# PSeitz/veloci

Measured on AMD Instinct MI355X. Metric: queries/sec, 3-term AND on 100M-doc index (p50 latency and HBM fraction alongside), higher is better.
Workload: dtype u32 doc ids + f16->f32 scores

## Files before the change

### veloci_amd/csrc/capi.cpp

```cpp
#include <chrono>
#include <thread>
#include <cstdio>
#include <cstdlib>
#include <cstring>

#include "../../include/veloci_amd.h"
#include <functional>
#include <future>

#include <dlfcn.h>
#include <unistd.h>

#include "engine.hpp"
#include "text.hpp"

using namespace vq;
using vqreq::Request;
using vqreq::VelociError;

namespace {
thread_local std::string g_err;

int fail(int code, const std::string& msg) {
    g_err = msg;
// ... 64 lines not shown
        s += ']';
    }
    s += '}';
}

static void why_found_info_json(std::string& s, const Result& R) {
    s += '{';
    bool first = true;
    for (auto& [anchor, fields] : R.why_found_info) {
        if (!first) s += ',';
        first = false;
        s += '"' + std::to_string(anchor) + "\":";
        why_found_terms_json(s, fields);
    }
    s += '}';
}

namespace {
void dump_f32(std::string& s, float f) {
    uint32_t b;
    std::memcpy(&b, &f, 4);
    s += std::to_string(b);
}
template <class T, class F>
void dump_opt(std::string& s, const std::optional<T>& v, F f) {
    if (v) f(s, *v);
    else s += "null";
}
void dump_usize(std::string& s, size_t v) { s += std::to_string(v); }
void dump_bool(std::string& s, bool v) { s += v ? "true" : "false"; }
void dump_str(std::string& s, const std::string& v) { vqjson::escape_to(s, v); }
void dump_boost_part(std::string& s, const vqreq::RequestBoostPart& b) {
    static const char* const names[] = {"Log2", "Log10", "Multiply", "Add", "Replace"};
    s += "{\"path\":";
    dump_str(s, b.path);
    s += ",\"boost_fun\":";
    if (b.boost_fun) s += std::string("\"") + names[int(*b.boost_fun)] + "\"";
    else s += "null";
    s += ",\"param\":";
    dump_opt(s, b.param, dump_f32);
    s += ",\"skip_when_score\":";
    if (b.skip_when_score) {
        s += '[';
        for (size_t i = 0; i < b.skip_when_score->size(); ++i) {
            if (i) s += ',';
            dump_f32(s, (*b.skip_when_score)[i]);
        }
        s += ']';
    } else s += "null";
    s += ",\"expression\":";
    dump_opt(s, b.expression, dump_str);
    s += '}';
}
void dump_boost_list(std::string& s, const std::optional<std::vector<vqreq::RequestBoostPart>>& v) {
    if (!v) {
        s += "null";
        return;
    }
    s += '[';
    for (size_t i = 0; i < v->size(); ++i) {
        if (i) s += ',';
        dump_boost_part(s, (*v)[i]);
    }
    s += ']';
}
void dump_options(std::string& s, const std::optional<vqreq::SearchRequestOptions>& o) {
    if (!o) {
        s += "null";
        return;
    }
    s += "{\"explain\":";
    dump_bool(s, o->explain);
    s += ",\"top\":";
    dump_opt(s, o->top, dump_usize);
    s += ",\"skip\":";
    dump_opt(s, o->skip, dump_usize);
    s += ",\"boost\":";
    dump_boost_list(s, o->boost);
    s += '}';
}
void dump_part(std::string& s, const vqreq::RequestSearchPart& p) {
    s += "{\"path\":";
    dump_str(s, p.path);
    s += ",\"terms\":[";
    for (size_t i = 0; i < p.terms.size(); ++i) {
        if (i) s += ',';
        dump_str(s, p.terms[i]);
    }
    s += "],\"levenshtein_distance\":";
    if (p.levenshtein_distance) s += std::to_string(*p.levenshtein_distance);
    else s += "null";
    s += ",\"starts_with\":";
    dump_bool(s, p.starts_with);
    s += ",\"is_regex\":";
    dump_bool(s, p.is_regex);
    s += ",\"token_value\":";
    if (p.token_value) dump_boost_part(s, *p.token_value);
    else s += "null";
    s += ",\"boost\":";
    dump_opt(s, p.boost, dump_f32);
    s += ",\"ignore_case\":";
    dump_opt(s, p.ignore_case, dump_bool);
    s += ",\"snippet\":";
    dump_opt(s, p.snippet, dump_bool);
    s += ",\"snippet_info\":";
    dump_bool(s, p.has_snippet_info);
    s += ",\"top\":";
    dump_opt(s, p.top, dump_usize);
    s += ",\"skip\":";
    dump_opt(s, p.skip, dump_usize);
    s += ",\"options\":";
    dump_options(s, p.options);
    s += '}';
}
void dump_search_request(std::string& s, const vqreq::SearchRequest& r) {
    if (r.kind == vqreq::SearchRequest::Search) {
        s += "{\"search\":";
        dump_part(s, r.part);
        s += '}';
        return;
    }
    s += r.kind == vqreq::SearchRequest::Or ? "{\"or\":{\"queries\":[" : "{\"and\":{\"queries\":[";
    for (size_t i = 0; i < r.tree.queries.size(); ++i) {
        if (i) s += ',';
        dump_search_request(s, r.tree.queries[i]);
    }
    s += "],\"options\":";
    dump_options(s, r.tree.options);
    s += "}}";
}
void dump_parts(std::string& s, const std::optional<std::vector<vqreq::RequestSearchPart>>& v) {
    if (!v) {
        s += "null";
        return;
    }
    s += '[';
    for (size_t i = 0; i < v->size(); ++i) {
        if (i) s += ',';
        dump_part(s, (*v)[i]);
    }
    s += ']';
}
}

extern "C" {

const char* vq_last_error(void) { return g_err.c_str(); }
const char* vq_version(void) { return "veloci_amd 0.3 (gfx950)"; }
uint32_t vq_debug_div100_mismatches(void) { return vq::debug_div100_mismatches(); }
uint32_t vq_debug_probe_occupancy(uint32_t shape, uint32_t nd, uint32_t na, uint32_t arr_slot, uint32_t cand_cap, uint32_t* lds_bytes) {
    const size_t lds = vq::scan_probe_lds_bytes(cand_cap, nd, na, arr_slot);
    if (lds_bytes) *lds_bytes = uint32_t(lds);
    return vq::debug_probe_occupancy(shape, lds);
}
uint64_t vq_index_speculative_reruns(const vq_index* index) { return index ? index->idx->or_reruns.load() : 0; }
int vq_debug_facet_select(const uint32_t* hist, uint32_t num_values, uint32_t top, uint32_t misalign, uint32_t* out_values, uint32_t* out_counts) {
    if (!hist || !out_values || !out_counts) return -1;
    return vq::debug_facet_select(hist, num_values, top, misalign, out_values, out_counts);
}

vq_index_builder* vq_index_builder_new(uint32_t num_anchors, uint32_t doc_lo, uint32_t doc_hi) {
    auto* b = new vq_index_builder();
    b->b.num_anchors = num_anchors;
    b->b.doc_lo = doc_lo;
    b->b.doc_hi = doc_hi;
    return b;
}
void vq_index_builder_free(vq_index_builder* b) { delete b; }

int vq_index_add_fst(vq_index_builder* b, const char* path, uint32_t num_terms, const uint8_t* term_bytes, const uint64_t* term_offsets) {
    return guard([&] {
        if (!b || !path || (num_terms && (!term_bytes || !term_offsets))) throw VelociError(VQ_ERR_INVALID_ARGUMENT, "vq_index_add_fst: null argument");
        HostFst f;
        f.terms.reserve(num_terms);
        for (uint32_t i = 0; i < num_terms; ++i) {
            f.terms.emplace_back(reinterpret_cast<const char*>(term_bytes) + term_offsets[i], size_t(term_offsets[i + 1] - term_offsets[i]));
            if (i && !(f.terms[i - 1] < f.terms[i])) throw VelociError(VQ_ERR_INVALID_ARGUMENT, std::string("terms must be bytewise sorted and unique: ") + path);
        }
        b->b.fst[path] = std::move(f);
    });
}

int vq_index_add_token_to_anchor_score(vq_index_builder* b, const char* path, uint32_t num_tokens, const uint64_t* offsets, const uint32_t* anchors,
                                       const uint32_t* scores, const uint64_t* global_lens) {
    return guard([&] {
        if (!b || !path || !offsets) throw VelociError(VQ_ERR_INVALID_ARGUMENT, "vq_index_add_token_to_anchor_score: null argument");
        HostPostings p;
        p.offsets.assign(offsets, offsets + num_tokens + 1);
        const uint64_t n = offsets[num_tokens];
        if (n && (!anchors || !scores)) throw VelociError(VQ_ERR_INVALID_ARGUMENT, "vq_index_add_token_to_anchor_score: null arrays");
        p.anchors.resize(n);
        p.scores.resize(n);
        const size_t piece = size_t(1) << 24;
        parallel_for((n + piece - 1) / piece, host_threads(), [&](size_t i) {
            const size_t off = i * piece, m = std::min<size_t>(piece, n - off);
            std::memcpy(p.anchors.data() + off, anchors + off, m * 4);
            std::memcpy(p.scores.data() + off, scores + off, m * 4);
        });
        parallel_for(num_tokens, host_threads(), [&](size_t t) {
            for (uint64_t i = offsets[t] + 1; i < offsets[t + 1]; ++i)
                if (!(anchors[i - 1] < anchors[i])) throw VelociError(VQ_ERR_INVALID_ARGUMENT, std::string("posting lists must be ascending and unique: ") + path);
        });
        if (global_lens) p.global_lens.assign(global_lens, global_lens + num_tokens);
        b->b.postings[path] = std::move(p);
    });
}

int vq_index_add_key_value_store(vq_index_builder* b, const char* path, uint32_t key_base, uint32_t num_keys, const uint64_t* offsets,
                                 const uint32_t* values) {
    return guard([&] {
        if (!b || !path || !offsets) throw VelociError(VQ_ERR_INVALID_ARGUMENT, "vq_index_add_key_value_store: null argument");
        HostKV k;
        k.key_base = key_base;
        k.offsets.assign(offsets, offsets + num_keys + 1);
        const uint64_t n = offsets[num_keys];
        if (n && !values) throw VelociError(VQ_ERR_INVALID_ARGUMENT, "vq_index_add_key_value_store: null values");
        k.values.assign(values, values + n);
        b->b.kv[path] = std::move(k);
    });
}

int vq_index_add_phrase_pair_to_anchor(vq_index_builder* b, const char* path, uint64_t num_pairs, const uint32_t* t1, const uint32_t* t2,
                                       const uint64_t* offsets, const uint32_t* anchors) {
    return guard([&] {
        if (!b || !path || !offsets) throw VelociError(VQ_ERR_INVALID_ARGUMENT, "vq_index_add_phrase_pair_to_anchor: null argument");
        HostPhrase p;
        p.t1.assign(t1, t1 + num_pairs);
        p.t2.assign(t2, t2 + num_pairs);
        p.offsets.assign(offsets, offsets + num_pairs + 1);
        p.anchors.assign(anchors, anchors + offsets[num_pairs]);
        b->b.phrase[path] = std::move(p);
    });
}

int vq_index_add_boost(vq_index_builder* b, const char* path, uint32_t key_base, uint32_t num_keys, const uint8_t* present, const uint32_t* value_bits) {
    return guard([&] {
        if (!b || !path || (num_keys && !value_bits)) throw VelociError(VQ_ERR_INVALID_ARGUMENT, "vq_index_add_boost: null argument");
        HostBoost h;
        h.key_base = key_base;
        if (present) h.present.assign(present, present + num_keys);
        h.bits.assign(value_bits, value_bits + num_keys);
        b->b.boost[path] = std::move(h);
    });
}

int vq_index_set_column_meta(vq_index_builder* b, const char* field, int is_anchor_identity_column, int tokenize) {
    return guard([&] {
        if (!b || !field) throw VelociError(VQ_ERR_INVALID_ARGUMENT, "vq_index_set_column_meta: null argument");
        ColumnMeta m;
        m.is_anchor_identity_column = is_anchor_identity_column != 0;
        m.tokenize = tokenize != 0;
        b->b.columns[field] = m;
    });
}

int vq_index_build(vq_index_builder* b, int device, vq_index** out) {
    return guard([&] {
        if (!b || !out) throw VelociError(VQ_ERR_INVALID_ARGUMENT, "vq_index_build: null argument");
        *out = nullptr;
        auto idx = build_index(b->b, device);
        auto* h = new vq_index();
        h->idx = std::move(idx);
        *out = h;
    });
}
void vq_index_free(vq_index* i) { delete i; }

int vq_index_set_stream(vq_index* i, void* hip_stream) {
    return guard([&] {
        if (!i) throw VelociError(VQ_ERR_INVALID_ARGUMENT, "vq_index_set_stream: null index");
        std::vector<std::unique_lock<std::mutex>> quiet;
        for (auto& w : i->idx->ws) quiet.emplace_back(w.mu);
        i->idx->stream = hip_stream ? static_cast<hipStream_t>(hip_stream) : i->idx->own_stream;
        i->idx->fin_stream = hip_stream ? static_cast<hipStream_t>(hip_stream) : i->idx->own_fin_stream;
    });
}
int vq_index_set_streams(vq_index* i, void* scan_stream, void* finish_stream) {
    return guard([&] {
        if (!i) throw VelociError(VQ_ERR_INVALID_ARGUMENT, "vq_index_set_streams: null index");
        if (!scan_stream || !finish_stream) throw VelociError(VQ_ERR_INVALID_ARGUMENT, "vq_index_set_streams: null stream (vq_index_set_stream(index, NULL) restores the index's own)");
        std::vector<std::unique_lock<std::mutex>> quiet;
        for (auto& w : i->idx->ws) quiet.emplace_back(w.mu);
        i->idx->stream = static_cast<hipStream_t>(scan_stream);
        i->idx->fin_stream = static_cast<hipStream_t>(finish_stream);
    });
}
int vq_index_set_allreduce(vq_index* i, vq_allreduce_u64_fn fn, void* ctx) {
    return guard([&] {
        if (!i) throw VelociError(VQ_ERR_INVALID_ARGUMENT, "vq_index_set_allreduce: null index");
        std::vector<std::unique_lock<std::mutex>> quiet;
        for (auto& w : i->idx->ws) quiet.emplace_back(w.mu);
        i->idx->allreduce_fn = fn;
        i->idx->allreduce_ctx = ctx;
    });
}
uint64_t vq_index_device_bytes(const vq_index* i) { return i ? i->idx->device_bytes : 0; }

int vq_request_parse(const char* json, size_t len, vq_request** out) {
    return guard([&] {
        if (!json || !out) throw VelociError(VQ_ERR_INVALID_ARGUMENT, "vq_request_parse: null argument");
        *out = nullptr;
        auto* r = new vq_request();
        try {
            r->req = vqreq::request_from_json_text(json, len);
        } catch (...) {
            delete r;
// ... 957 lines not shown
```

### veloci_amd/csrc/compile.cpp

```cpp
#include <algorithm>
#include <cmath>
#include <cstdlib>
#include <cstring>
#include <regex>
#include <set>

#include "engine.hpp"
#include "text.hpp"

namespace vq {
std::atomic<uint64_t> g_compile_ns[16];

using namespace vqreq;

namespace {

bool ends_with(const std::string& s, const char* suf) {
    size_t n = std::strlen(suf);
    return s.size() >= n && std::memcmp(s.data() + s.size() - n, suf, n) == 0;
}

[[noreturn]] void unsupported(const std::string& what) {
    throw VelociError(ERR_UNSUPPORTED, "unsupported on the MI355X query path: " + what);
}
// ... 532 lines not shown
        for (uint32_t id : l.hits_ids) {
            const uint32_t *b, *e;
            if (t2a.host_row(id, &b, &e)) all.insert(all.end(), b, e);
        }
        std::sort(all.begin(), all.end());
        if (!with_multiplicity) all.erase(std::unique(all.begin(), all.end()), all.end());
        return layered_inline(all);
    }
    std::vector<uint32_t> layered_inline(const std::vector<uint32_t>& sorted_ids) {
        std::vector<std::vector<uint32_t>> layers;
        for (size_t i = 0; i < sorted_ids.size();) {
            size_t j = i;
            while (j < sorted_ids.size() && sorted_ids[j] == sorted_ids[i]) ++j;
            const size_t mult = j - i;
            if (layers.size() < mult) layers.resize(mult);
            for (size_t m = 0; m < mult; ++m) layers[m].push_back(sorted_ids[i]);
            i = j;
        }
        std::vector<uint32_t> out;
        for (auto& l : layers) out.push_back(add_inline_list(std::move(l)));
        return out;
    }

    static size_t union_min() {
        static const size_t v = std::getenv("VQ_UNION_MIN") ? size_t(std::atoi(std::getenv("VQ_UNION_MIN"))) : 4;
        return v;
    }
    static bool has_wide_and(const SearchRequest& r) {
        if (r.kind == SearchRequest::Search) return false;
        if (r.kind == SearchRequest::And && r.tree.queries.size() >= 3) return true;
        for (auto& q : r.tree.queries)
            if (has_wide_and(q)) return true;
        return false;
    }

    void push_op(std::vector<DOp>& ops, const DOp& op, uint32_t& sp) {
        if (ops.size() >= size_t(kMaxOps)) unsupported("query tree with more than " + std::to_string(kMaxOps) + " nodes");
        ops.push_back(op);
        if (op.kind != OP_LEAF) sp -= op.nchild;
        ++sp;
        max_depth = std::max(max_depth, sp);
        if (sp > uint32_t(kStackDepth)) unsupported("query tree deeper than the evaluation stack");
    }

    std::string leaf_union_key(const Leaf& l) {
        const PostingStore& ps = posting_store(l);
        size_t nonempty = 0;
        for (auto& [tid, score] : l.hits_scores)
            if (tid < ps.num_tokens && ps.global_len[tid]) ++nonempty;
        if (!(nonempty > union_min() || (nonempty > 1 && req.search_req && has_wide_and(*req.search_req)))) return std::string();
        return "u|" + l.path + "|" + (l.key.empty() ? l.part->key() : l.key);
    }

    NodeInfo compile_leaf_scores(const SearchRequest& r, Leaf& l, std::vector<DOp>& ops, uint32_t& sp) {
        std::vector<Leaf*> one{&l};
        return compile_leaf_lists(r.part.terms[0], one, ops, sp);
    }

    NodeInfo compile_leaf_lists(const std::string& label, const std::vector<Leaf*>& members, std::vector<DOp>& ops, uint32_t& sp) {
        PhaseTimer pt(3);
        NodeInfo info;
        DOp op{};
        op.kind = OP_LEAF;
        op.list_begin = uint16_t(cq.lists.size());
        info.label = label;
        struct Entry {
            const PostingStore* ps;
            uint32_t tid;
            float score;
        };
        std::vector<Entry> entries;
        entries.reserve(4);
        info.cover.reserve(4);
        for (Leaf* l : members) {
            const PostingStore& ps = posting_store(*l);
            for (auto& [tid, score] : l->hits_scores)
                if (tid < ps.num_tokens) entries.push_back({&ps, tid, score});
        }
        size_t nonempty = 0;
        for (auto& e : entries)
            if (e.ps->global_len[e.tid]) ++nonempty;
        uint32_t count = 0;
        if (nonempty > union_min() || (nonempty > 1 && req.search_req && has_wide_and(*req.search_req))) {
            std::string ukey;
            if (members.size() == 1) ukey = leaf_union_key(*members[0]);
            else {
                ukey = "u|fused";
                for (Leaf* l : members) ukey += "|" + l->path + "|" + (l->key.empty() ? l->part->key() : l->key);
            }
            const UnionJob* done = nullptr;
            if (unions) {
                auto it = unions->find(ukey);
                if (it != unions->end()) done = &it->second;
            }
            info.glen = 0;
            if (!done) {
                UnionJob job;
                job.key = ukey;
                for (auto& e : entries)
                    if (e.ps->global_len[e.tid]) {
                        job.terms.push_back(UnionJob::Term{e.ps, e.tid, e.score});
                        job.input_postings += e.ps->len[e.tid];
                    }
                cq.union_requests.push_back(std::move(job));
                info.len_known = true;
            } else {
                if (done->len) {
                    HList h;
                    h.d_docs = done->d_docs;
                    h.d_scores = reinterpret_cast<const uint16_t*>(done->d_vals);
                    h.len = done->len;
                    h.global_len = done->global_len;
                    h.flags = LIST_HAS_SCORES | LIST_F32;
                    h.term_score = 1.0f;
                    h.max_value = done->max_value;
                    uint32_t li = add_list(h);
                    info.cover.push_back(li);
                    info.cover_len += h.len;
                    count = 1;
                }
                cq.algorithmic_bytes += 6ull * done->input_postings + 8ull * done->len;
                info.glen = done->global_len;
                info.len_known = !req.filter && idx.can_sum_over_shards();
            }
            op.list_count = uint16_t(count);
            push_op(ops, op, sp);
            info.emitted = true;
            return info;
        }
        uint32_t with_entries = 0;
        for (auto& e : entries) {
            const PostingStore& ps = *e.ps;
            if (ps.global_len[e.tid]) ++with_entries;
            if (ps.len[e.tid] == 0) continue;
            HList h;
            h.d_docs = ps.docs.as<uint32_t>() + ps.start[e.tid];
            h.d_scores = ps.scores.as<uint16_t>() + ps.start[e.tid];
            h.len = ps.len[e.tid];
            h.global_len = ps.global_len[e.tid];
            h.flags = LIST_HAS_SCORES;
            h.term_score = e.score;
            h.max_raw = ps.max_raw[e.tid];
            if (!ps.bm_start.empty() && ps.bm_start[e.tid] >= 0) {
                h.flags |= LIST_BITMAP;
                h.d_bitmap = ps.bitmaps.as<uint32_t>() + ps.bm_start[e.tid];
                h.d_rank_dir = ps.rank_dir.as<uint32_t>() + ps.rd_start[e.tid];
            }
            if (!ps.td_start.empty() && ps.td_start[e.tid] >= 0) h.d_tile_dir = ps.tile_dir.as<uint32_t>() + ps.td_start[e.tid];
            if (!ps.pk_start.empty() && ps.pk_start[e.tid] >= 0) {
                h.d_cov32 = ps.cov32.as<uint32_t>() + uint64_t(ps.pk_start[e.tid]) * 8;
                h.d_gdir = ps.gdir.as<uint32_t>() + ps.gd_start[e.tid];
                if (ps.ak_start[e.tid] >= 0) h.d_arr16 = ps.arr16.as<uint16_t>() + uint64_t(ps.ak_start[e.tid]) * 8;
                h.tile_most = ps.tile_most[e.tid];
            }
            uint32_t li = add_list(h);
            info.cover.push_back(li);
            info.cover_len += h.len;
            cq.algorithmic_bytes += 6ull * h.len;
            ++count;
        }
        op.list_count = uint16_t(count);
        info.len_known = with_entries <= 1 && !req.filter;
        info.glen = 0;
        for (auto& e : entries) info.glen += e.ps->global_len[e.tid];
        push_op(ops, op, sp);
        info.emitted = true;
        return info;
    }

    void fill_boost_params(DColBoost& cb, const RequestBoostPart& b) {
        cb.fun = b.boost_fun ? int32_t(*b.boost_fun) : BF_NONE;
        cb.param = b.param.value_or(0.0f);
        if (b.skip_when_score) {
            if (b.skip_when_score->size() > size_t(kMaxSkipWhen)) unsupported("more than 4 skip_when_score values");
            cb.nskip = uint32_t(b.skip_when_score->size());
            for (size_t i = 0; i < b.skip_when_score->size(); ++i) cb.skip[i] = (*b.skip_when_score)[i];
        }
        cb.expr_op = EX_NONE;
        if (b.expression) parse_expression(*b.expression, cb);
    }

    std::vector<uint32_t> boost_1n_text_ids(const RequestSearchPart& part, Leaf& l) {
        std::vector<uint32_t> ids;
        auto cit = idx.columns.find(part.path);
        const bool tokenized = cit != idx.columns.end() && cit->second.tokenize;
        if (tokenized) {
            const KVStore& t2t = kv_store(l.path + TOKENS_TO_TEXT_ID);
            for (auto& h : l.hits_scores) {
                const uint32_t *rb, *re;
                if (t2t.host_row(h.first, &rb, &re)) ids.insert(ids.end(), rb, re);
                else ids.push_back(h.first);
            }
            sort_unique_u32(ids);
        } else ids = l.hits_ids;
        return ids;
    }
    std::vector<std::pair<uint32_t, float>> resolve_boost_1n(const RequestSearchPart& part, Leaf& l, const RequestBoostPart& b) {
        PhaseTimer pt(1);
        std::vector<uint32_t> value_ids;
        {
            PhaseTimer gather(6);
            const std::vector<uint32_t> ids = boost_1n_text_ids(part, l);
            const KVStore& to_parent = kv_store(l.path + VALUE_ID_TO_PARENT);
            for (uint32_t id : ids) {
                const uint32_t *rb, *re;
                if (to_parent.host_row(id, &rb, &re)) value_ids.insert(value_ids.end(), rb, re);
            }
        }
        {
            PhaseTimer sort(7);
            sort_unique_u32(value_ids);
        }
        PhaseTimer pairs_timer(8);
        auto bit = idx.boost.find(b.path + BOOST_VALID_TO_VALUE);
        if (bit == idx.boost.end()) throw VelociError(ERR_INDEX_NOT_FOUND, "Did not found path in indices " + b.path + BOOST_VALID_TO_VALUE);
        const KVStore& to_anchor = kv_store(b.path + VALUE_ID_TO_ANCHOR);
        std::vector<std::pair<uint32_t, float>> pairs;
        pairs.reserve(value_ids.size());
        for (uint32_t vid : value_ids) {
            float v;
            if (!bit->second.host_value(vid, &v)) continue;
            const uint32_t *rb, *re;
            if (to_anchor.host_row(vid, &rb, &re)) pairs.push_back({*rb, v});
        }
        return pairs;
    }

    void emit_boost_1n(const RequestSearchPart& part, Leaf& l, const RequestBoostPart& b, std::vector<DOp>& ops, uint32_t& sp) {
        PhaseTimer pt(2);
        const std::string cache_key = (l.key.empty() ? part.key() : l.key) + "|" + b.path;
        auto emit_layer = [&](const HList& h) {
            const uint32_t li = add_list(h);
            cq.algorithmic_bytes += 8ull * h.len;
            DColBoost cb{};
            fill_boost_params(cb, b);
            cb.nskip = 0;
            cq.leaf_cols.push_back(cb);
            DOp op{};
            op.kind = OP_BOOST1N;
            op.nchild = 1;
            op.list_begin = uint16_t(li);
            op.list_count = 1;
            op.child_slot[0] = uint8_t(cq.leaf_cols.size() - 1);
            push_op(ops, op, sp);
        };
        static const bool device_on = std::getenv("VQ_BOOST1N_DEVICE") != nullptr;
        if (boost_cache && device_on) {
            const std::string to_parent = l.path + VALUE_ID_TO_PARENT, to_anchor = b.path + VALUE_ID_TO_ANCHOR, col = b.path + BOOST_VALID_TO_VALUE;
            auto kp = idx.kv.find(to_parent), ka = idx.kv.find(to_anchor);
            const bool staged = kp != idx.kv.end() && ka != idx.kv.end() && kp->second.value_csr && ka->second.value_csr && idx.boost.count(col);
            if (staged && !boost_cache->device) {
                Boost1nJob job;
                job.key = cache_key;
                job.to_parent_path = to_parent;
                job.to_anchor_path = to_anchor;
                job.boost_path = col;
                job.text_ids = boost_1n_text_ids(part, l);
                cq.boost1n_requests.push_back(std::move(job));
                return;
            }
            if (staged) {
                auto it = boost_cache->device->find(cache_key);
                if (it != boost_cache->device->end() && it->second.done) {
                    const Boost1nJob& job = it->second;
                    if (!job.ascending) unsupported("1:n field boost whose value ids are not in anchor order (" + b.path + ")");
                    if (!job.several) {
                        HList h;
                        h.d_docs = job.d_docs;
                        h.d_scores = reinterpret_cast<const uint16_t*>(job.d_vals);
                        h.len = job.len;
                        h.global_len = job.total;
                        h.flags = LIST_HAS_SCORES | LIST_F32;
                        h.term_score = 1.0f;
                        emit_layer(h);
                        return;
                    }
                }
            }
        }
        std::shared_ptr<Boost1nEntry> entry = boost_cache ? boost_cache->entry(cache_key) : std::make_shared<Boost1nEntry>();
        auto make_layers = [&](const std::vector<std::vector<std::pair<uint32_t, float>>>& layers) {
            auto out = std::make_shared<std::vector<Boost1nEntry::Layer>>();
            for (auto& layer : layers) {
                Boost1nEntry::Layer L;
                L.global_len = layer.size();
                L.docs.reserve(layer.size());
                L.vals.reserve(layer.size());
                for (auto& pr : layer)
                    if (pr.first >= idx.doc_lo && pr.first < idx.doc_hi) {
                        L.docs.push_back(pr.first);
                        L.vals.push_back(pr.second);
                    }
                out->push_back(std::move(L));
            }
            return out;
        };
        std::call_once(entry->resolved, [&] {
            entry->pairs = resolve_boost_1n(part, l, b);
            PhaseTimer order_check(9);
            const auto& pairs = entry->pairs;
            for (size_t i = 1; i < pairs.size(); ++i) {
                if (pairs[i].first < pairs[i - 1].first) entry->ascending = false;
                entry->several = entry->several || pairs[i].first == pairs[i - 1].first;
            }
            if (!entry->ascending) return;
            if (!entry->several) entry->layers = make_layers({pairs});
// ... 1157 lines not shown
                        for (uint32_t e = 0; e < cq.lists.size(); ++e)
                            if (cq.lists[e].d_docs == h.d_docs && cq.lists[e].inline_idx < 0 && cq.lists[e].len == h.len) {
                                li = e;
                                break;
                            }
                        if (li == UINT32_MAX) {
                            li = add_list(h);
                            cq.algorithmic_bytes += 4ull * h.len;
                        }
                        cq.loc_idx.push_back(uint16_t(li));
                        ++count;
                    }
                lf.list_count = uint16_t(count);
                cq.locf.push_back(lf);
            }

        if (req.facets)
            for (auto& fr : *req.facets) {
                std::vector<std::string> steps = get_steps_to_anchor(fr.field);
                std::string store_path;
                if (steps.size() == 1) store_path = steps.front() + PARENT_TO_VALUE_ID;
                else if (idx.kv.count(steps.back() + ANCHOR_TO_TEXT_ID)) store_path = steps.back() + ANCHOR_TO_TEXT_ID;
                const KVStore& kv = store_path.empty() ? idx.composed_facet(steps) : kv_store(store_path);
                if (!kv.facet_csr) unsupported("facet source " + store_path + " is not staged as an anchor-keyed CSR");
                auto dit = idx.dict.find(steps.back());
                if (dit == idx.dict.end()) throw VelociError(ERR_FST_NOT_FOUND, "fst not found loaded in indices " + steps.back() + " ");
                DFacet f{};
                f.offsets = kv.csr_off.as<uint64_t>();
                f.values = kv.csr_values.as<uint32_t>();
                f.direct = kv.csr_direct.p ? kv.csr_direct.as<uint32_t>() : nullptr;
                f.key_base = kv.csr_key_base;
                f.num_keys = kv.csr_num_keys;
                f.num_values = std::max<uint32_t>(uint32_t(dit->second.terms.size()), kv.csr_num_keys ? kv.csr_max_value + 1 : 0);
                const uint64_t want = fr.top ? std::min<uint64_t>(*fr.top, f.num_values) : f.num_values;
                f.top = want > uint64_t(kMaxTopK) ? 0u : uint32_t(want);
                cq.facets.push_back(f);
                FacetOut fo;
                fo.field = fr.field;
                fo.dict_path = steps.back();
                fo.top = f.top;
                fo.host_top = want > uint64_t(kMaxTopK) ? uint32_t(want) : 0u;
                fo.num_values = f.num_values;
                cq.facet_out.push_back(fo);
                cq.algorithmic_bytes += 4ull * f.num_values;
            }
        cq.algorithmic_bytes += 8ull * cq.top_k;

        if (label_wanted) {
            if (maybe_reqs.empty() && count_reqs.empty()) unsupported("OR over an operand whose term label is only known at run time (set_op.rs:143,439)");
            if (!idx.can_sum_over_shards())
                unsupported("OR over an AND whose label follows run-time result sizes, on a sharded index without vq_index_set_allreduce");
            count_reqs.insert(count_reqs.end(), maybe_reqs.begin(), maybe_reqs.end());
        }
        if (2 * count_reqs.size() + 1 > 256) unsupported("more than 127 AND operands whose sizes must be measured first");
        build_presence_program();
        if (!count_reqs.empty())
            for (auto& l : cq.lists) l.flags |= LIST_COVER;
        {
            const size_t n = cq.ops.size();
            auto is_leaf1 = [&](const DOp& o) {
                return o.kind == OP_LEAF && o.list_count == 1 && (cq.lists[o.list_begin].flags & LIST_HAS_SCORES) && !(cq.lists[o.list_begin].flags & LIST_F32);
            };
            if (n == 1 && is_leaf1(cq.ops[0])) cq.simple_n = 1;
            else if (n >= 3 && n <= 5 && cq.ops[n - 1].kind != OP_LEAF && cq.ops[n - 1].nchild == n - 1) {
                bool ok = true;
                for (size_t i = 0; i + 1 < n; ++i) ok = ok && is_leaf1(cq.ops[i]);
                if (ok) cq.simple_n = uint32_t(n - 1);
            }
            if (cq.simple_n > 1 && cq.ops[n - 1].kind == OP_OR && cq.ops[n - 1].nslots == cq.simple_n) {
                DOp& root = cq.ops[n - 1];
                std::vector<std::pair<uint8_t, DOp>> leaves;
                for (uint32_t k = 0; k < cq.simple_n; ++k) leaves.push_back({root.child_slot[k], cq.ops[k]});
                std::stable_sort(leaves.begin(), leaves.end(), [](auto& x, auto& y) { return x.first < y.first; });
                for (uint32_t k = 0; k < cq.simple_n; ++k) {
                    cq.ops[k] = leaves[k].second;
                    root.child_slot[k] = leaves[k].first;
                }
            }
        }

        {
            static const bool force_generic = std::getenv("VQ_FORCE_GENERIC") != nullptr;
            const bool pure = cq.simple_n && count_reqs.empty() && cq.fops.empty() && cq.groups.empty() && cq.tboosts.empty() && cq.cols.empty() && cq.locf.empty() &&
                              cq.facets.empty() && uint64_t(idx.doc_hi) - idx.doc_lo >= 65536;
            if (pure && !force_generic) {
                uint32_t f = 1u << 17;
                static const bool no_probe = std::getenv("VQ_NO_PROBE") != nullptr;
                static const uint64_t probe_min_docs = std::getenv("VQ_PROBE_MIN_DOCS") ? uint64_t(std::atoll(std::getenv("VQ_PROBE_MIN_DOCS"))) : 40'000'000ull;
                bool probe = !no_probe && cq.simple_n >= 2 && cq.ops[cq.simple_n].kind == OP_AND && uint64_t(idx.doc_hi) - idx.doc_lo >= probe_min_docs;
                uint32_t arr_mask = 0;
                if (probe) {
                    static const bool no_arr = std::getenv("VQ_PROBE_NO_ARR") != nullptr;
                    uint32_t covers = 0;
                    for (uint32_t k = 0; k < cq.simple_n; ++k) {
                        const HList& l = cq.lists[cq.ops[k].list_begin];
                        if (l.flags & LIST_COVER) {
                            ++covers;
                            probe = probe && l.d_cov32;
                        } else {
                            const bool arr = l.d_arr16 && !no_arr && (!(l.flags & LIST_BITMAP) || uint64_t(l.len) * 16 < uint64_t(idx.doc_hi) - idx.doc_lo);
                            if (arr) arr_mask |= 1u << k;
                            probe = probe && (arr || (l.flags & LIST_BITMAP));
                        }
                    }
                    probe = probe && covers == 1;
                }
                static const bool no_probe_or = std::getenv("VQ_NO_PROBE_OR") != nullptr;
                uint32_t or_cover = UINT32_MAX;
                if (!probe && !no_probe && !no_probe_or && !req.exact_routes_only && cq.top_k >= 1 && cq.simple_n >= 2 && cq.simple_n <= 3 && cq.ops[cq.simple_n].kind == OP_OR &&
                    cq.ops[cq.simple_n].nslots == cq.simple_n && !idx.sharded() && !(idx.comm && idx.comm->nranks > 1) && uint64_t(idx.doc_hi) - idx.doc_lo >= probe_min_docs) {
                    for (uint32_t k = 0; k < cq.simple_n; ++k) {
                        const HList& l = cq.lists[cq.ops[k].list_begin];
                        if (l.d_cov32 && (or_cover == UINT32_MAX || l.len < cq.lists[cq.ops[or_cover].list_begin].len)) or_cover = k;
                    }
                    double sum = 0.0, cnt = 0.0;
                    for (uint32_t k = 0; k < cq.simple_n && or_cover != UINT32_MAX; ++k) {
                        if (k == or_cover) continue;
                        const HList& l = cq.lists[cq.ops[k].list_begin];
                        if (!(l.flags & LIST_BITMAP) || (l.flags & LIST_F32) || l.max_raw >= 0x7C00 || !(l.term_score >= 0.0f)) {
                            or_cover = UINT32_MAX;
                            break;
                        }
                        const uint16_t h = l.max_raw;
                        const int e = (h >> 10) & 31, m = h & 1023;
                        const double a = e ? std::ldexp(1.0 + m / 1024.0, e - 15) : std::ldexp(m / 1024.0, -14);
                        const double v = double(l.term_score) * (a / 100.0);
                        if (v >= 0.00001 * (1.0 - 1e-5)) cnt += 1.0;
                        sum += v;
                    }
                    if (or_cover != UINT32_MAX) {
                        const HList& c = cq.lists[cq.ops[or_cover].list_begin];
                        if (!(c.term_score > 0.0f) || c.max_raw >= 0x7C00) or_cover = UINT32_MAX;
                        else {
                            const double b = sum * cnt * cnt * (1.0 + 1e-5);
                            cq.or_skip_bound = b < 3.0e38 ? float(b) : std::numeric_limits<float>::infinity();
                            if (cq.or_skip_bound < float(b)) cq.or_skip_bound = std::nextafter(cq.or_skip_bound, std::numeric_limits<float>::infinity());
                            probe = true;
                        }
                    }
                }
                const bool or_probe = or_cover != UINT32_MAX && probe;
                bool seq = false;
                for (uint32_t k = 0; k < cq.simple_n && !probe; ++k) {
                    const HList& l = cq.lists[cq.ops[k].list_begin];
                    if ((l.flags & LIST_COVER) && (l.flags & LIST_BITMAP)) seq = true;
                }
                if (seq) f |= 1u << 16;
                if (probe) {
                    f |= 1u << 25 | arr_mask << 12 | (or_probe ? 1u << 27 : 0u);
                    cq.probe = DProbe{};
                    for (uint32_t k = 0; k < cq.simple_n; ++k) {
                        const HList& l = cq.lists[cq.ops[k].list_begin];
                        cq.probe.leaf[k] = DProbeLeaf{l.d_cov32, l.d_arr16, l.d_gdir};
                        if ((arr_mask >> k) & 1u) cq.probe_arr_gran = std::max(cq.probe_arr_gran, l.tile_most);
                    }
                }
                static const bool ring = std::getenv("VQ_RING") != nullptr && std::atoi(std::getenv("VQ_RING")) != 0;
                if (probe && ring && !arr_mask && !or_probe && cq.top_k >= 1 && cq.top_k <= kPoolMaxK) f |= 1u << 26;
                for (uint32_t k = 0; k < cq.simple_n; ++k) {
                    const HList& l = cq.lists[cq.ops[k].list_begin];
                    const bool cover = or_probe ? k == or_cover : (l.flags & LIST_COVER) != 0;
                    if (cover) f |= 1u << (8 + k);
                    if ((l.flags & LIST_BITMAP) && (seq || !cover) && !((arr_mask >> k) & 1u)) f |= 1u << k;
                    if (uint64_t(l.len) * 8192 >= 200 * (uint64_t(idx.doc_hi) - idx.doc_lo)) f |= 1u << (20 + k);
                }
                static const bool no_union_cov = std::getenv("VQ_NO_UNION_COV") != nullptr;
                if (cq.simple_n == 1 && !no_union_cov) {
                    const HList& l = cq.lists[cq.ops[0].list_begin];
                    if (l.d_cov32 && l.d_gdir && l.d_tile_dir && l.term_score > 0.0f && !(l.flags & LIST_F32) && l.inline_idx < 0) {
                        f |= 1u << 28;
                        cq.probe = DProbe{};
                        cq.probe.leaf[0] = DProbeLeaf{l.d_cov32, l.d_arr16, l.d_gdir};
                    }
                }
                cq.simple_flags = f;
            }
        }

        {
            static const bool off = std::getenv("VQ_FORCE_GENERIC") != nullptr || std::getenv("VQ_NO_LEAF_F32") != nullptr;
            if (!off && !cq.simple_flags && count_reqs.empty() && cq.ops.size() == 1 && cq.ops[0].kind == OP_LEAF && cq.ops[0].list_count == 1 &&
                (cq.lists[cq.ops[0].list_begin].flags & LIST_F32) && cq.fops.empty() && cq.groups.empty() && cq.tboosts.empty() && cq.cols.empty() && cq.locf.empty() &&
                cq.facets.empty())
                cq.simple_flags = 1u << 19;
        }
        if (!cq.simple_flags) detect_rich_simple();
        if (!cq.simple_flags) detect_wide();
        if (!cq.simple_flags || ((cq.simple_flags >> 24) & 1u)) compute_prune_table();
        if (!cq.simple_flags && count_reqs.empty()) {
            bool dense_cover = false;
            for (auto& l : cq.lists) dense_cover = dense_cover || ((l.flags & LIST_COVER) && (l.flags & LIST_BITMAP));
            if (dense_cover) {
                cq.seq_tiles = 1;
                for (auto& l : cq.lists)
                    if (l.flags & LIST_BITMAP) l.flags &= ~uint32_t(LIST_COVER);
            }
        }

        const uint32_t L = std::max<uint32_t>(uint32_t(cq.lists.size()), 1);
        const uint64_t range = uint64_t(idx.doc_hi) - idx.doc_lo;
        static const uint32_t ww_max = [] {
            const char* e = std::getenv("VQ_TILE_WORDS_MAX");
            uint32_t v = e ? uint32_t(std::atoi(e)) : 256u;
            uint32_t p2 = 64;
            while (p2 < v && p2 < 2048) p2 <<= 1;
            return p2;
        }();
        static const size_t var_budget = [] {
            const char* e = std::getenv("VQ_TILE_LDS_KB");
            return size_t(e ? std::atoi(e) : 12) * 1024;
        }();
        static const uint64_t span_env = [] {
            const char* e = std::getenv("VQ_SPAN_POSTINGS");
            return uint64_t(e ? std::atoll(e) : 0);
        }();
        const bool and_like = ((cq.simple_flags >> 18) & 1u) || (cq.simple_flags && cq.simple_n > 1 && cq.ops.back().kind == OP_AND);
        const bool wide_like = (cq.simple_flags >> 24) & 1u;
        const bool probe_like = (cq.simple_flags >> 25) & 1u;
        const uint64_t probe_span = std::min<uint64_t>(std::max<uint64_t>(range / 96, 131072), 1048576);
        const bool or_like = cq.simple_flags && !((cq.simple_flags >> 18) & 1u) && !wide_like && !probe_like && cq.simple_n > 1 && cq.ops.back().kind == OP_OR;
        const uint64_t span_postings = span_env ? span_env : (probe_like ? probe_span : and_like ? 131072 : wide_like ? 589824 : (or_like && range >= 50'000'000ull) ? 524288 : 262144);
        uint32_t ww = ww_max;
        const size_t TL = size_t(L) + cq.n_temps;
        while (ww > 64 && (size_t(ww) + TL * ww + size_t(L) * ww / 2) * 4 > var_budget) ww >>= 1;
        if ((size_t(ww) + TL * ww + size_t(L) * ww / 2) * 4 > 96 * 1024) unsupported("too many lists for the LDS tile");
        const uint64_t cover_len = std::max<uint64_t>(root.cover_len, 1);
        if (cover_len * (uint64_t(ww) << 5) / std::max<uint64_t>(range, 1) < 64) {
            const uint64_t want = std::max<uint64_t>(range / cover_len, 2048);
            while (ww > 64 && (uint64_t(ww) << 5) / 2 >= want) ww >>= 1;
        }
        if (cq.simple_flags) ww = 256;
        cq.tile_words = ww;
        cq.stack_depth = std::max<uint32_t>(max_depth, 1);
        uint64_t spans = (cq.total_len + span_postings - 1) / span_postings;
        static const uint64_t facet_span = [] {
            const char* e = std::getenv("VQ_FACET_SPAN_POSTINGS");
            return uint64_t(e ? std::atoll(e) : 4096);
        }();
        if (!cq.facets.empty()) spans = (cq.total_len + facet_span - 1) / facet_span;
        const uint64_t tiles = std::max<uint64_t>((range + (uint64_t(ww) << 5) - 1) / (uint64_t(ww) << 5), 1);
        {
            uint64_t cover_len = 0;
            for (auto& l : cq.lists)
                if (l.flags & LIST_COVER) cover_len += l.len;
            const uint64_t visited = std::max<uint64_t>(std::min<uint64_t>(cover_len, tiles), 1);
            if (!cq.simple_flags && cq.total_len / visited < 1024) spans = std::max<uint64_t>(spans, visited / 16);
            if (((cq.simple_flags >> 18) & 1u) && cq.total_len / visited < 1024) spans = std::max<uint64_t>(spans, visited / 64);
        }
        if ((cq.simple_flags >> 26) & 1u) {
            static const uint64_t ring_tiles = [] {
                const char* e = std::getenv("VQ_RING_SPAN_TILES");
                return uint64_t(e ? std::max(1, std::atoi(e)) : 64);
            }();
            const uint64_t ptiles = std::max<uint64_t>((range + (1u << kProbeTileShift) - 1) >> kProbeTileShift, 1);
            spans = (ptiles + ring_tiles - 1) / ring_tiles;
        }
        spans = std::min<uint64_t>(spans, tiles);
        spans = std::min<uint64_t>(std::max<uint64_t>(spans, 1), 4096);
        cq.n_spans = uint32_t(spans);
        if ((cq.simple_flags >> 19) & 1u) {
            const uint64_t len = cq.lists[cq.ops[0].list_begin].len;
            cq.n_spans = uint32_t(std::min<uint64_t>(std::max<uint64_t>(len / (cq.facets.empty() ? 16384 : 4096), 1), 4096));
        }
        cq.max_spans = uint32_t(std::min<uint64_t>(std::max<uint64_t>(tiles, 1), 4096));
        if ((cq.simple_flags >> 19) & 1u) cq.max_spans = uint32_t(std::min<uint64_t>(std::max<uint64_t>(cq.lists[cq.ops[0].list_begin].len / 64, 1), 4096));
        compute_layout_bytes(root.cover_len);
    }

    void compute_layout_bytes(uint64_t cover_len) {
        const uint64_t range = uint64_t(idx.doc_hi) - idx.doc_lo;
        const bool simple = cq.simple_flags != 0;
        const bool wide = (cq.simple_flags >> 24) & 1u;
        const uint64_t tile_docs = wide ? 8192 : ((cq.simple_flags >> 25) & 1u) ? (1u << kProbeTileShift) : simple ? 16384 : uint64_t(cq.tile_words) << 5;
        const uint64_t tiles = std::max<uint64_t>((range + tile_docs - 1) / tile_docs, 1);
        const bool seq = wide ? cq.wide.seq != 0 : simple ? ((cq.simple_flags >> 16) & 1u) : cq.seq_tiles != 0;
        const uint64_t visited = seq ? tiles : std::min<uint64_t>(std::max<uint64_t>(cover_len, 1), tiles);
        auto bitmap_cost = [&]() { return visited * (tile_docs / 8 + 4); };
        uint64_t b = 8ull * cq.top_k;
        if ((cq.simple_flags >> 19) & 1u) b += 8ull * cq.lists[cq.ops[0].list_begin].len;
        else if (simple && !((cq.simple_flags >> 18) & 1u) && cq.simple_n == 1 && std::getenv("VQ_NO_UNION") == nullptr)
            b += (((cq.simple_flags >> 28) & 1u) ? 4ull : 6ull) * cq.lists[cq.ops[0].list_begin].len;
        else if (wide) {
            for (uint32_t k = 0; k < cq.wide.n_leaves; ++k) b += ((cq.wide.bitmap_mask >> k) & 1u) ? bitmap_cost() : 4ull * cq.lists[cq.wide.leaf_list[k]].len;
        } else if ((cq.simple_flags >> 25) & 1u) {
            for (uint32_t k = 0; k < cq.simple_n; ++k) {
                const uint64_t len = cq.lists[cq.ops[k].list_begin].len;
                b += ((cq.simple_flags >> k) & 1u) ? visited * (tile_docs / 8 + 4 * (tile_docs >> kRankShift)) : ((cq.simple_flags >> (12 + k)) & 1u) ? 2ull * len : 4ull * len;
            }
        } else if (simple) {
            std::vector<bool> seen(cq.lists.size(), false);
            const bool rich = (cq.simple_flags >> 18) & 1u;
            for (uint32_t k = 0; k < cq.simple_n; ++k) {
                const uint32_t li = rich ? cq.simple2.leaf_list[k] : cq.ops[k].list_begin;
                seen[li] = true;
                b += ((cq.simple_flags >> k) & 1u) ? bitmap_cost() : 4ull * cq.lists[li].len;
            }
            for (uint32_t li = 0; li < cq.lists.size(); ++li)
                if (!seen[li]) b += 4ull * cq.lists[li].len;
        } else {
            for (auto& l : cq.lists) {
                const bool as_bitmap = (l.flags & LIST_BITMAP) && !(l.flags & LIST_COVER);
                b += as_bitmap ? bitmap_cost() : 4ull * l.len;
            }
        }
        for (auto& f : cq.facets) b += 4ull * f.num_values;
        cq.layout_bytes = b;
    }
};

}

float default_score_for_distance_host(uint8_t distance, bool prefix_matches) { return default_score_for_distance(distance, prefix_matches); }
size_t debug_sort_unique(uint32_t* ids, size_t n) {
    std::vector<uint32_t> v(ids, ids + n);
    sort_unique_u32(v);
    std::copy(v.begin(), v.end(), ids);
    return v.size();
}

std::vector<SuggestEntry> suggest_part(const Index& idx, const RequestSearchPart& part, const FuzzyTable* fuzzy) {
    Request dummy;
    Compiler c(idx, dummy, fuzzy);
    Leaf l;
    l.part = &part;
    l.get_scores = true;
    l.return_term = true;
    l.return_term_lowercase = true;
    c.lookup_terms(idx, l, true, false);
    if (part.token_value) c.apply_token_value(*part.token_value, l);
    std::vector<SuggestEntry> out;
    std::map<uint32_t, const std::string*> text;
    for (auto& t : l.terms) text[t.first] = &t.second;
    for (auto& h : l.hits_scores) out.push_back(SuggestEntry{*text.at(h.first), h.second, h.first});
    return out;
}


namespace {
template <class IsHit, class Append>
std::string snippet_of_tokens(size_t n, IsHit is_hit, Append append_text, const vqreq::SnippetInfo& opt, bool* any) {
    const int64_t around = opt.num_words_around_snippet * 2;
    std::string out;
    int64_t first_hit = -1, last_hit = -1, group_first = -1, group_last = -1;
    uint64_t windows = 0;
    auto close_group = [&]() {
        if (group_first < 0) return;
        if (windows < opt.max_snippets) {
            if (windows) out += opt.snippet_connector;
            const size_t lo = size_t(std::max<int64_t>(group_first - around, 0)), hi = size_t(std::min<int64_t>(group_last + around + 1, int64_t(n)));
            for (size_t i = lo; i < hi; ++i) {
                if (is_hit(i)) {
                    out += opt.snippet_start_tag;
                    append_text(out, i);
                    out += opt.snippet_end_tag;
                } else append_text(out, i);
            }
        }
        ++windows;
    };
    for (size_t i = 0; i < n; ++i) {
        if (!is_hit(i)) continue;
        if (first_hit < 0) first_hit = int64_t(i);
        if (group_first < 0 || int64_t(i) - group_last >= around) {
            close_group();
            group_first = int64_t(i);
        }
        group_last = last_hit = int64_t(i);
    }
    close_group();
    *any = first_hit >= 0;
    if (!*any) return out;
    if (first_hit > around) out.insert(0, opt.snippet_connector);
    if (last_hit < int64_t(n) - around) out += opt.snippet_connector;
    return out;
}
std::string snippet_of_text(const Dictionary& dict, const uint32_t* toks, size_t n, const std::vector<uint32_t>& wanted_sorted, const vqreq::SnippetInfo& opt, bool* any) {
    return snippet_of_tokens(
        n, [&](size_t i) { return std::binary_search(wanted_sorted.begin(), wanted_sorted.end(), toks[i]); },
        [&](std::string& out, size_t i) {
            if (toks[i] < dict.terms.size()) out += dict.terms[toks[i]];
        },
        opt, any);
}
void check_snippet_window(const vqreq::SnippetInfo& opt) {
    if (opt.num_words_around_snippet < 0 || opt.num_words_around_snippet > 0x3FFFFFFF)
        throw VelociError(ERR_INVALID_REQUEST, "InvalidRequest: \"snippet_info.num_words_around_snippet out of range\" ");
}
}

std::optional<std::string> highlight_text(const std::string& text, const std::vector<std::string>& terms, const vqreq::SnippetInfo& opt, bool tokenized) {
    check_snippet_window(opt);
    std::vector<std::string> set = terms;
    std::sort(set.begin(), set.end());
    set.erase(std::unique(set.begin(), set.end()), set.end());
    if (set.size() == 1 && set[0] == text) return opt.snippet_start_tag + text + opt.snippet_end_tag;
    if (!tokenized) return std::nullopt;
    const std::vector<vqtext::TokenSpan> tokens = vqtext::tokenize_grouped(text);
    std::vector<char> hit(tokens.size(), 0);
    for (size_t i = 0; i < tokens.size(); ++i) hit[i] = std::binary_search(set.begin(), set.end(), text.substr(tokens[i].begin, tokens[i].end - tokens[i].begin));
    bool any = false;
    std::string out = snippet_of_tokens(
        tokens.size(), [&](size_t i) { return hit[i] != 0; }, [&](std::string& o, size_t i) { o.append(text, tokens[i].begin, tokens[i].end - tokens[i].begin); }, opt, &any);
    if (!any || opt.max_snippets == 0) return std::nullopt;
    return out;
}

std::vector<SuggestEntry> highlight_part(const Index& idx, const RequestSearchPart& part, const FuzzyTable* fuzzy) {
    static const vqreq::SnippetInfo kDefault;
    const vqreq::SnippetInfo& opt = part.has_snippet_info ? part.snippet_info : kDefault;
    check_snippet_window(opt);
    RequestSearchPart lookup = part;
    lookup.snippet.reset();
    lookup.has_snippet_info = false;
    Request dummy;
    Compiler c(idx, dummy, fuzzy);
    Leaf l;
    l.part = &lookup;
    l.get_scores = true;
    c.lookup_terms(idx, l, true, false);
    if (lookup.token_value) c.apply_token_value(*lookup.token_value, l);

    struct TextHit {
        uint32_t text;
        float score;
        uint32_t token, order;
    };
    std::vector<TextHit> hits;
    std::vector<std::pair<uint32_t, float>> ranked;
    const std::string& path = l.path;
    auto cit = idx.columns.find(path.substr(0, path.size() - std::strlen(TEXTINDEX)));
    const bool tokenized = cit != idx.columns.end() && cit->second.tokenize;
    const bool add_snippets = part.snippet.value_or(false);
    std::map<uint32_t, std::string> snippets;
    for (auto& h : l.hits_scores) ranked.push_back(h);
    if (tokenized) {
        auto kit = idx.kv.find(path + TOKENS_TO_TEXT_ID);
        if (kit == idx.kv.end()) throw VelociError(ERR_INDEX_NOT_FOUND, "Did not found path in indices " + path + TOKENS_TO_TEXT_ID);
        uint32_t order = 0;
        for (auto& h : l.hits_scores) {
            const uint32_t *b, *e;
// ... 238 lines not shown
```

### veloci_amd/csrc/device_types.hpp

```cpp
#pragma once
#include <hip/hip_runtime.h>
#include <stdint.h>

namespace vq {

constexpr int kBlock = 64;
constexpr int kCandCap = 2048;
constexpr int kMaxTopK = 1024;
constexpr int kStackDepth = 16;
constexpr int kMaxChildren = 16;
constexpr int kMaxLists = 64;
constexpr int kMaxOps = 160;
constexpr int kMaxSkipWhen = 4;
constexpr uint32_t kTileDirShift = 14;
constexpr uint32_t kProbeTileShift = 15;
constexpr uint32_t kRankShift = 9;

enum ListFlags : uint32_t {
    LIST_HAS_SCORES = 1u,
    LIST_COVER = 2u,
    LIST_BITMAP = 4u,
    LIST_F32 = 8u,
};

struct DList {
    const uint32_t* docs;
    const uint16_t* scores;
    uint32_t len;
    uint32_t flags;
    float term_score;
    uint16_t max_raw;
    uint16_t pad;
    const uint32_t* bitmap;
    const uint32_t* rank_dir;
    const uint32_t* tile_dir;
};

enum OpKind : uint8_t { OP_LEAF = 0, OP_AND = 1, OP_OR = 2, OP_BOOST1N = 3, OP_LEAFMAX = 4 };

struct DOp {
    uint8_t kind;
    uint8_t nchild;
    uint8_t nslots;
    uint8_t pad;
    uint16_t list_begin;
    uint16_t list_count;
    uint8_t child_slot[kMaxChildren];
    uint8_t and_order[kMaxChildren];
};

enum PresKind : uint8_t { PRES_AND = 0, PRES_OR = 1, PRES_ZERO = 2, PRES_COUNT = 3 };
constexpr uint16_t kSlotTemp = 0x8000;
constexpr uint16_t kSlotRoot = 0xFFFF;
struct DPresOp {
    uint8_t kind;
    uint8_t pad;
    uint16_t out;
    uint16_t n_in;
    uint16_t in_begin;
};

struct DGroup {
    uint16_t list_begin, list_count;
    float mult;
};

struct DTermBoost {
    uint16_t list;
    uint16_t pad;
    float mult;
};

enum BoostFun : int32_t { BF_NONE = -1, BF_LOG2 = 0, BF_LOG10 = 1, BF_MULTIPLY = 2, BF_ADD = 3, BF_REPLACE = 4 };
enum ExprOp : int32_t { EX_NONE = -1, EX_DIV = 0, EX_MUL = 1, EX_ADD = 2, EX_SUB = 3 };

struct DColBoost {
    const float* values;
    const uint32_t* present;
    uint32_t key_base, num_keys;
    int32_t fun;
    float param;
    uint32_t nskip;
    float skip[kMaxSkipWhen];
    int32_t expr_op;
    int32_t expr_lkind, expr_rkind;
    float expr_lval, expr_rval;
    uint32_t pad;
};

constexpr uint16_t kLocPrecomputed = 0xFFFF;
struct DLocField {
    uint16_t list_begin, list_count;
};

struct DFacet {
    const uint64_t* offsets;
    const uint32_t* values;
    const uint32_t* direct;
    uint32_t key_base, num_keys;
    uint32_t hist_off;
    uint32_t num_values;
    uint32_t top;
    uint32_t out_off;
};

struct DSimple2 {
    uint8_t ngroups, root_kind, root_nslots, n_side;
    uint8_t g_kind[4], g_mask[4], g_nslots[4];
    uint8_t g_order[4][4];
    uint8_t g_slot[4][4];
    uint8_t r_order[4];
    uint8_t r_slot[4];
    uint8_t n_grp, n_tb, n_loc, has_filter;
    uint8_t filter_mask, f32_mask, pad2, pad3;
    uint8_t grp_mask[4];
    uint8_t tb_side[4];
    uint8_t loc_leaf[2], loc_side[2];
    uint16_t leaf_list[4];
    uint16_t side_list[4];
    float grp_mult[4];
    float tb_mult[4];
    float ub[16];
    uint8_t prune, pad4, pad5, pad6;
};

constexpr int kWideMax = 16;
struct DWide {
    uint8_t n_leaves, n_groups, root_kind, root_nslots;
    uint8_t seq, pad0, pad1, pad2;
    uint16_t bitmap_mask, cover_mask, prefetch_mask, f32_mask;
    uint16_t leaf_list[kWideMax];
    uint8_t leaf_slot[kWideMax];
    uint8_t g_kind[kWideMax], g_begin[kWideMax], g_count[kWideMax];
    uint8_t leaf_and_order[kWideMax];
    uint8_t leaf_slot_order[kWideMax];
    uint8_t r_and_order[kWideMax];
    uint8_t r_slot[kWideMax];
    uint8_t r_slot_order[kWideMax];
};

struct QHeader {
    uint32_t n_lists, n_ops, n_fops, n_groups, n_tboost, n_col, n_locf, n_facets;
    uint32_t off_lists, off_ops, off_fops, off_groups, off_tboost, off_col, off_locf, off_facets;
    uint32_t top_k;
    uint32_t tile_words;
    uint32_t n_spans;
    uint32_t keys_base;
    uint32_t doc_lo, doc_hi;
    uint32_t part_keys_off;
    uint32_t blob_bytes;
    uint32_t desc_bytes;
    uint32_t n_pres, off_pres, off_pres_in, n_temps;
    uint32_t off_loc_idx;
    uint32_t off_simple2;
    uint32_t off_pool;
    uint32_t prune_n;
    uint64_t prune_mask;
    unsigned long long gthr;
    unsigned long long key_upper;
    uint32_t seq_tiles;
    uint32_t stat_off;
    uint32_t prune_gbits[16];
    uint32_t n_counts;
    uint32_t bitmap_base;
    uint32_t simple_n;
    uint32_t simple_flags;
};

// ... 24 lines not shown
```

### veloci_amd/csrc/engine.hpp

```cpp
#pragma once
#include <hip/hip_runtime.h>

#include <atomic>
#include <cmath>
#include <chrono>
#include <cstdint>
#include <map>
#include <limits>
#include <memory>
#include <thread>
#include <functional>
#include <condition_variable>
#include <mutex>
#include <string>
#include <unordered_map>
#include <vector>

#include "device_types.hpp"
#include "kernels.hpp"
#include "request.hpp"
#include "hostpool.hpp"

namespace vq {

// ... 121 lines not shown
};

struct Dictionary {
    std::vector<std::string> terms;
    std::unordered_map<std::string, std::vector<uint32_t>> lower_map;
    uint32_t char_bytes = 2;
    bool low_exact = true;
    DevBuf d_off;
    DevBuf d_raw;
    DevBuf d_low;
};

struct Index;
struct PostingStore;
struct FuzzyProbe {
    std::string key;
    std::string path;
    std::vector<uint32_t> query;
    uint32_t max_d = 0;
    bool transposition = false, prefix = false, ci = true;
    std::vector<uint32_t> matches;
    std::vector<float> scores;
    std::string lower_term;
    uint32_t lev = 0;
    bool check_prefix = false;
    int status = 0;
    std::string error;
};
using FuzzyTable = std::map<std::string, FuzzyProbe>;
std::string fuzzy_key(const vqreq::RequestSearchPart& p);
bool needs_dictionary_scan(const vqreq::RequestSearchPart& p);
void collect_fuzzy_probes(const Index& idx, const vqreq::Request& req, FuzzyTable& table);
struct Workspace;
void run_fuzzy_probes(const Index& idx, Workspace& ws, FuzzyTable& table, hipStream_t st);
void score_fuzzy_probe(const Index& idx, FuzzyProbe& probe);
float default_score_for_distance_host(uint8_t distance, bool prefix_matches);
size_t debug_sort_unique(uint32_t* ids, size_t n);
struct SuggestEntry {
    std::string text;
    float score;
    uint32_t term_id;
};
std::vector<SuggestEntry> suggest_part(const Index& idx, const vqreq::RequestSearchPart& part, const FuzzyTable* fuzzy);
void collect_suggest_probes(const Index& idx, const vqreq::Request& req, FuzzyTable& table);
std::optional<std::string> highlight_text(const std::string& text, const std::vector<std::string>& terms, const vqreq::SnippetInfo& opt, bool tokenized);
vqreq::Request page_request_after(const vqreq::Request& request, float score, uint32_t id);
std::vector<SuggestEntry> highlight_part(const Index& idx, const vqreq::RequestSearchPart& part, const FuzzyTable* fuzzy);
std::vector<SuggestEntry> run_highlight(const Index& idx, vqreq::RequestSearchPart part);
std::vector<SuggestEntry> run_suggest(const Index& idx, const vqreq::Request& req);

struct UnionJob {
    std::string key;
    struct Term {
        const PostingStore* store;
        uint32_t token;
        float score;
    };
    std::vector<Term> terms;
    const uint32_t* d_docs = nullptr;
    const float* d_vals = nullptr;
    float max_value = std::numeric_limits<float>::infinity();
    uint32_t len = 0;
    uint64_t global_len = 0;
    uint64_t input_postings = 0;
};
using UnionTable = std::map<std::string, UnionJob>;
struct RangeJob {
    std::string key;
    std::string store_path;
    std::vector<uint32_t> tokens;
    std::string union_key;
    std::shared_ptr<const std::vector<uint32_t>> anchors;
    std::vector<uint64_t> counts;
};
using RangeTable = std::map<std::string, RangeJob>;
struct Boost1nEntry {
    struct Layer {
        std::vector<uint32_t> docs;
        std::vector<float> vals;
        uint64_t global_len = 0;
    };
    std::once_flag resolved, layered;
    std::vector<std::pair<uint32_t, float>> pairs;
    bool ascending = true, several = false;
    std::vector<uint32_t> anchors;
    std::shared_ptr<const std::vector<Layer>> layers;
};
struct Boost1nCache {
    static constexpr size_t kShards = 64;
    struct Shard {
        std::mutex mu;
        std::unordered_map<std::string, std::shared_ptr<Boost1nEntry>> map;
    } shard[kShards];
    std::shared_ptr<Boost1nEntry> entry(const std::string& key) {
        Shard& sh = shard[std::hash<std::string>{}(key) % kShards];
        std::lock_guard<std::mutex> g(sh.mu);
        auto& slot = sh.map[key];
        if (!slot) slot = std::make_shared<Boost1nEntry>();
        return slot;
    }
    const std::map<std::string, struct Boost1nJob>* device = nullptr;
};
struct LocalityJob {
    std::string key;
    std::string t2t_path, t2a_path;
    std::vector<uint32_t> tokens;
    const uint32_t* d_docs = nullptr;
    const float* d_vals = nullptr;
    uint32_t len = 0;
};
using LocalityTable = std::map<std::string, LocalityJob>;
struct Boost1nJob {
    std::string key;
    std::string to_parent_path, to_anchor_path, boost_path;
    std::vector<uint32_t> text_ids;
    const uint32_t* d_docs = nullptr;
    const float* d_vals = nullptr;
    uint32_t len = 0;
    uint32_t total = 0;
    bool ascending = true;
    bool several = false;
    bool done = false;
};
using Boost1nTable = std::map<std::string, Boost1nJob>;
constexpr int kStatusNeedsUnion = -1;
constexpr int kStatusNeedsCounts = -2;
constexpr int kStatusNeedsRanges = -3;

struct QueryCounts {
    bool has_filter = false;
    uint64_t filter_count = 0;
    std::map<uint32_t, std::pair<uint64_t, uint64_t>> nodes;
};

struct PostingStore {
    uint32_t num_tokens = 0;
    std::vector<uint64_t> start;
    std::vector<uint32_t> len;
    std::vector<uint64_t> global_len;
    std::vector<uint16_t> max_raw;
    DevBuf docs;
    DevBuf scores;
    uint64_t total_padded = 0;
    std::vector<int64_t> bm_start;
    std::vector<int64_t> rd_start;
    DevBuf bitmaps;
    DevBuf rank_dir;
    std::vector<int64_t> td_start;
    DevBuf tile_dir;
    std::vector<int64_t> pk_start;
    std::vector<int64_t> ak_start;
    std::vector<int64_t> gd_start;
    std::vector<uint32_t> tile_most;
    DevBuf cov32, arr16, gdir;
};

struct KVStore {
    uint32_t key_base = 0, num_keys = 0;
    std::vector<uint64_t> host_off;
    std::vector<uint32_t> host_values;
    bool list_rows = false;
    bool rows_sorted_unique = true;
    bool rows_equal_postings = false;
    std::vector<uint64_t> start;
    std::vector<uint32_t> len;
    DevBuf values;
    DevBuf d_row_start, d_row_len;
    bool text_csr = false;
    DevBuf d_text_vals;
    bool value_csr = false;
    DevBuf d_csr_off;
    bool facet_csr = false;
    uint32_t csr_key_base = 0, csr_num_keys = 0;
    uint32_t csr_max_value = 0;
    DevBuf csr_direct;
    DevBuf csr_off;
    DevBuf csr_values;

    bool host_row(uint64_t key, const uint32_t** b, const uint32_t** e) const {
        if (key < key_base) return false;
        uint64_t r = key - key_base;
        if (r >= num_keys || host_off[r] == host_off[r + 1]) return false;
        *b = host_values.data() + host_off[r];
        *e = host_values.data() + host_off[r + 1];
        return true;
    }
};

struct PhraseStore {
    std::vector<std::pair<uint32_t, uint32_t>> keys;
    std::vector<uint64_t> start;
    std::vector<uint32_t> len;
    DevBuf anchors;
};

struct BoostColumn {
    uint32_t key_base = 0, num_keys = 0;
    bool has_present = false;
    float vmin = 0.0f, vmax = 0.0f;
    bool any_value = false, has_nan = false;
    DevBuf values;
    DevBuf present;
    std::vector<uint32_t> host_bits;
    std::vector<uint8_t> host_present;
    bool host_value(uint64_t key, float* out) const {
        if (key < key_base || key - key_base >= host_bits.size()) return false;
        const size_t r = size_t(key - key_base);
        if (!host_present.empty() && !host_present[r]) return false;
        std::memcpy(out, &host_bits[r], 4);
        return true;
    }
};

struct PinnedBuf {
    void* p = nullptr;
    size_t bytes = 0;
    PinnedBuf() = default;
    PinnedBuf(const PinnedBuf&) = delete;
    PinnedBuf& operator=(const PinnedBuf&) = delete;
    ~PinnedBuf();
    void ensure(size_t n);
    template <class T>
    T* as() const { return reinterpret_cast<T*>(p); }
};

constexpr int kWorkspaces = 4;

enum KernelId : int {
    K_DICT_SCAN = 0, K_UNION_COUNT, K_UNION_WRITE, K_UNION_DENSE_SCATTER, K_UNION_DENSE_COUNT, K_UNION_DENSE_WRITE, K_RANGE_HITS, K_COUNT_PREPASS, K_SCAN_LEAF_F32, K_SCAN_RICH, K_SCAN_RING, K_SCAN_PROBE, K_SCAN_AND, K_SCAN_SIMPLE, K_SCAN_UNION,
    K_SCAN_WIDE, K_TILE_SCAN, K_MERGE_SPANS, K_FINALIZE, K_FACET_SELECT, K_LOCALITY, K_BOOST1N, K_COUNT_
};
extern const char* const kKernelNames[K_COUNT_];

struct TimedLaunch {
    int kernel;
    uint32_t ev_begin, ev_end;
    uint64_t layout_bytes, algorithmic_bytes, queries;
};

struct Workspace {
    std::mutex mu;
    std::atomic<bool> pinned{false};
    std::vector<hipEvent_t> ev_pool;
    uint32_t ev_used = 0;
    std::vector<TimedLaunch> timed;
    hipEvent_t ev_done = nullptr;
    PinnedBuf h_up, h_down;
    DevBuf d_up;
    DevBuf d_span_keys;
    DevBuf d_partial;
    DevBuf d_down;
    DevBuf d_union_docs[2], d_union_vals[2], d_union_max, d_union_meta;
    DevBuf d_union_slab, d_union_dense_docs, d_union_dense_vals, d_union_dense_meta;
    DevBuf d_loc_a, d_loc_b, d_loc_pairs_a, d_loc_pairs_b, d_loc_meta, d_loc_tmp, d_loc_docs, d_loc_vals;
    DevBuf d_b1n_a, d_b1n_b, d_b1n_meta, d_b1n_tmp, d_b1n_docs, d_b1n_vals;
    DevBuf d_probe_desc, d_probe_counts, d_probe_ids;
};

struct KernelProfile {
    double ms = 0;
    uint64_t launches = 0;
    uint64_t layout_bytes = 0;
    uint64_t algorithmic_bytes = 0;
    uint64_t gathered_bytes = 0;
    uint64_t queries = 0;
};
struct Profile {
    bool enabled = false;
    KernelProfile k[K_COUNT_];
    uint64_t batches = 0;
};
struct LaunchTimer {
    Workspace* ws = nullptr;
    hipStream_t st = nullptr;
    size_t slot = 0;
    LaunchTimer(bool on, Workspace& w, hipStream_t s, int kernel, uint64_t layout_bytes = 0, uint64_t algorithmic_bytes = 0, uint64_t queries = 0);
    ~LaunchTimer();
    LaunchTimer(const LaunchTimer&) = delete;
    LaunchTimer& operator=(const LaunchTimer&) = delete;
};


struct ShardComm {
    int nranks = 1, rank = 0;
    void* nccl = nullptr;
    int (*allgather)(void* ctx, const void* local, void* gathered, size_t bytes_per_rank, void* stream) = nullptr;
    int (*allreduce_u32)(void* ctx, void* inout, size_t count, void* stream) = nullptr;
    void* ctx = nullptr;
    hipStream_t stream = nullptr;
    hipEvent_t ev_scan[2] = {nullptr, nullptr}, ev_xchg[2] = {nullptr, nullptr}, ev_fin[2] = {nullptr, nullptr};
    void* unmerged = nullptr;
    int live = 0;
    DevBuf gathered[2];
    DevBuf red;
    bool busy[2] = {false, false};
    std::string failed;
    std::mutex mu;
    ~ShardComm();
};

struct Index {
    int device = 0;
    int (*allreduce_fn)(void*, uint64_t*, size_t) = nullptr;
    void* allreduce_ctx = nullptr;
    bool sharded() const { return doc_lo != 0 || doc_hi != num_anchors; }
    bool can_sum_over_shards() const { return !sharded() || allreduce_fn != nullptr; }
    void sum_over_shards(std::vector<uint64_t>& v) const {
        if (!sharded() || v.empty()) return;
        if (!allreduce_fn || allreduce_fn(allreduce_ctx, v.data(), v.size()) != 0) throw vqreq::VelociError(vqreq::ERR_DEVICE, "all-reduce over the shards failed");
    }
    mutable std::atomic<uint64_t> or_reruns{0};
    mutable std::unique_ptr<HostPool> pool;
    mutable std::mutex pool_mu;
    uint32_t num_anchors = 0, doc_lo = 0, doc_hi = 0;
    uint32_t bitmap_base = 0;
    uint64_t bitmap_words = 0;
    std::map<std::string, Dictionary> dict;
    std::map<std::string, PostingStore> postings;
    std::map<std::string, KVStore> kv;
    std::map<std::string, PhraseStore> phrase;
    std::map<std::string, BoostColumn> boost;
    std::map<std::string, ColumnMeta> columns;
    uint64_t device_bytes = 0;
    mutable std::mutex composed_mu;
    mutable std::map<std::string, std::unique_ptr<KVStore>> composed_facets;
    const KVStore& composed_facet(const std::vector<std::string>& steps) const;
    hipStream_t own_stream = nullptr, own_fin_stream = nullptr;
    hipStream_t pre_stream = nullptr;
    hipStream_t stream = nullptr;
    hipStream_t fin_stream = nullptr;
    mutable std::mutex profile_mutex;
    mutable Profile profile;
    mutable Workspace ws[kWorkspaces];
    mutable std::atomic<uint32_t> next_ws{0};
    mutable DevBuf arena;
    static constexpr size_t kArenaBytes = 64ull << 20;
    mutable std::unique_ptr<ShardComm> comm;
    ~Index();
    bool is_anchor_identity(const std::string& textindex_path) const;
};

std::unique_ptr<Index> build_index(const IndexBuilder& b, int device);

struct HList {
    const uint32_t* d_docs = nullptr;
    const uint16_t* d_scores = nullptr;
    uint32_t len = 0;
    uint32_t flags = 0;
    float term_score = 0.f;
    uint16_t max_raw = 0x7C00;
    float max_value = std::numeric_limits<float>::infinity();
    uint64_t global_len = 0;
    const uint32_t* d_bitmap = nullptr;
    const uint32_t* d_rank_dir = nullptr;
    const uint32_t* d_tile_dir = nullptr;
    const uint32_t* d_cov32 = nullptr;
    const uint16_t* d_arr16 = nullptr;
    const uint32_t* d_gdir = nullptr;
    uint32_t tile_most = 0;
    int inline_idx = -1;
    int inline_val_idx = -1;
};

struct FacetOut {
    std::string field;
    std::string dict_path;
    uint32_t top = 10;
    uint32_t num_values = 0;
    uint32_t host_top = 0;
};

struct ExplainRec {
    enum Kind : uint8_t { Boost, MaxTokenToTextId, TermToAnchor, LevenshteinScore, OrSumOverDistinctTerms } kind = Boost;
    float a = 0.0f, b = 0.0f, c = 0.0f;
    uint32_t term_id = 0;
    std::string text;
};
using ExplainRecs = std::vector<ExplainRec>;
struct ExplainNode {
    uint32_t kind = 0;
    int op = -1;
    std::vector<int> children;
    std::vector<uint16_t> order;
    uint32_t list_begin = 0, list_count = 0;
    std::vector<uint32_t> list_term;
    std::map<uint32_t, ExplainRecs> term_records;
};
using WhyFoundPlan = std::map<std::string, std::vector<uint32_t>>;
struct ExplainPlan {
    std::vector<ExplainNode> nodes;
    int root = -1;
    std::vector<ExList> lists;
    std::vector<ExOp> ops;
    std::vector<uint16_t> aux;
    std::vector<DColBoost> cols;
};

struct CompiledQuery {
    size_t blob_bytes = 0, desc_bytes = 0;
    int status = 0;
    std::shared_ptr<const ExplainPlan> explain_plan;
    std::shared_ptr<const WhyFoundPlan> why_found_plan;
    std::string error;
    std::vector<RangeJob> range_requests;
    std::vector<UnionJob> union_requests;
    std::vector<LocalityJob> locality_requests;
    std::vector<Boost1nJob> boost1n_requests;
    std::vector<uint32_t> count_nodes;
    uint32_t n_counts = 0;
    std::vector<HList> lists;
    std::vector<std::vector<uint32_t>> inline_lists;
    std::vector<std::vector<float>> inline_vals;
    std::vector<DColBoost> leaf_cols;
    uint32_t seq_tiles = 0;
    uint32_t prune_n = 0;
    uint64_t prune_mask = 0;
    uint32_t prune_gbits[16] = {};
    uint32_t n_top_cols = 0;
    std::vector<DOp> ops, fops;
    std::vector<DPresOp> pres;
    std::vector<uint16_t> pres_in;
    uint32_t n_temps = 0;
    uint32_t simple_n = 0;
    uint32_t simple_flags = 0;
    std::vector<DGroup> groups;
    std::vector<DTermBoost> tboosts;
    std::vector<DColBoost> cols;
    std::vector<DLocField> locf;
    std::vector<uint16_t> loc_idx;
    DSimple2 simple2{};
    DWide wide{};
    DProbe probe{};
    uint32_t probe_arr_gran = 0;
    std::vector<DFacet> facets;
    std::vector<FacetOut> facet_out;
    std::map<std::string, std::vector<std::string>> why_found_terms;
    uint32_t top = 10, skip = 0, top_k = 10;
    uint64_t total_len = 0;
    uint64_t algorithmic_bytes = 0;
    uint64_t layout_bytes = 0;
    uint64_t key_upper = ~0ull;
    float or_skip_bound = std::numeric_limits<float>::quiet_NaN();
    bool deep = false;
    uint32_t tile_words = 0, n_spans = 1, stack_depth = 1;
    uint32_t max_spans = 1;
};

CompiledQuery compile_query(const Index& idx, const vqreq::Request& req, const FuzzyTable* fuzzy = nullptr, const UnionTable* unions = nullptr,
                            const QueryCounts* counts = nullptr, const RangeTable* ranges = nullptr, Boost1nCache* boost_cache = nullptr,
                            const LocalityTable* localities = nullptr);
void run_locality_jobs(const Index& idx, Workspace& ws, LocalityTable& table, hipStream_t st);
void run_boost1n_jobs(const Index& idx, Workspace& ws, Boost1nTable& table, hipStream_t st);
void run_range_jobs(const Index& idx, Workspace& ws, RangeTable& table, const UnionTable& unions, hipStream_t st);
void run_union_jobs(const Index& idx, Workspace& ws, UnionTable& table, hipStream_t st);
struct Result;
void complete_explain_requests(const Index& idx, std::vector<std::unique_ptr<Result>>& results, std::vector<int>& status, std::vector<std::string>& errors);
void complete_why_found_requests(const Index& idx, std::vector<std::unique_ptr<Result>>& results, std::vector<int>& status, std::vector<std::string>& errors);
bool request_wants_explain(const vqreq::Request& req);
std::string explain_records_json(const ExplainRecs& records);
void complete_deep_requests(const Index& idx, const vqreq::Request* const* reqs, size_t n, std::vector<std::unique_ptr<Result>>& results,
                            std::vector<int>& status, std::vector<std::string>& errors);

struct ResultFacet {
    std::string field;
    std::vector<std::pair<std::string, uint64_t>> entries;
};
struct Result {
    uint64_t num_hits = 0;
    uint64_t execution_time_ns = 0;
    std::vector<uint32_t> ids;
    std::vector<float> scores;
    std::vector<ResultFacet> facets;
    bool has_facets = false;
    std::map<std::string, std::vector<std::string>> why_found_terms;
    std::shared_ptr<const ExplainPlan> explain_plan;
    std::shared_ptr<const WhyFoundPlan> why_found_plan;
    std::map<uint32_t, std::map<std::string, std::vector<std::string>>> why_found_info;
    bool has_explain = false;
    std::vector<std::pair<bool, ExplainRecs>> explain;
    bool deep = false;
    bool rerun_exact = false;
    mutable std::string json;
};

struct PartialBatch {
    const Index* index = nullptr;
    Workspace* ws = nullptr;
    std::unique_lock<std::mutex> lock;
    bool pinned_ws = false;
    std::vector<CompiledQuery> queries;
    std::vector<uint32_t> slot;
    std::vector<uint8_t> qclass;
    std::vector<FacetJob> facet_jobs;
    uint32_t nq_dev = 0;
    PartialLayout layout{};
    const uint8_t* d_blobs = nullptr;
    const uint32_t* d_blob_off = nullptr;
    const uint32_t* d_span_base = nullptr;
    const FacetJob* d_facet_jobs = nullptr;
    uint8_t* d_partial = nullptr;
    uint32_t total_spans = 0;
    uint32_t n_facet_jobs = 0;
    uint32_t total_facet_out = 0;
    bool profiled = false;
    bool launched = false, finished = false;
    bool merge_launched = false;
    std::chrono::steady_clock::time_point t0;
    void release_workspace();
    std::vector<const vqreq::Request*> reqs;
    ~PartialBatch();
};

std::unique_ptr<PartialBatch> run_partial(const Index& idx, const vqreq::Request* const* reqs, size_t n, int slot = -1, int64_t arena_offset = -1);
void finish_batch(const Index& idx, PartialBatch& pb, const void* gathered_device, uint32_t num_shards, std::vector<std::unique_ptr<Result>>& out,
                  std::vector<int>& status, std::vector<std::string>& errors, size_t shard_stride = 0);
void finish_launch(const Index& idx, PartialBatch& pb, const void* gathered_device, uint32_t num_shards, size_t shard_stride = 0);

}
```

### veloci_amd/csrc/exec.cpp

```cpp
#include <algorithm>
#include <cstdio>
#include <cstdlib>
#include <cstring>
#include <thread>

#include "engine.hpp"

#include "text.hpp"

namespace vq {

using namespace vqreq;

void DevBuf::ensure(size_t n) {
    if (n <= bytes) return;
    size_t want = std::max(n, bytes + bytes / 2);
    alloc(want);
}
PinnedBuf::~PinnedBuf() {
    if (p) (void)hipHostFree(p);
}
void PinnedBuf::ensure(size_t n) {
    if (n <= bytes) return;
    if (p) (void)hipHostFree(p);
// ... 1183 lines not shown
                    for (auto& kv : c.nodes) {
                        flat.push_back(kv.second.first);
                        flat.push_back(kv.second.second);
                    }
                }
                idx.sum_over_shards(flat);
                size_t k = 0;
                for (auto& c : counts) {
                    c.filter_count = flat[k++];
                    for (auto& kv : c.nodes) {
                        kv.second.first = flat[k++];
                        kv.second.second = flat[k++];
                    }
                }
            }
            for (size_t k = 0; k < need.size(); ++k) {
                CompiledQuery& q = pb->queries[need[k]];
                q = compile_query(idx, *reqs[need[k]], fuzzy.empty() ? nullptr : &fuzzy, unions.empty() ? nullptr : &unions, &counts[k], rangesp, &boost_cache,
                                  localities.empty() ? nullptr : &localities);
                if (q.status < 0) {
                    q.status = ERR_UNSUPPORTED;
                    q.error = "unsupported on the MI355X query path: query still needs a pre-pass after the count pre-pass (internal)";
                }
            }
        }
    }
    const double t_compiled = now_ms();
    uint32_t nq = 0;
    uint64_t total_keys = 0, total_hist = 0, total_span_keys = 0, total_spans = 0, blob_bytes = 0;
    uint32_t max_lists = 1, max_ww = 32;
    size_t lds_bytes = 0;
    uint32_t stack_depth = 1;
    std::vector<uint32_t> keys_base, part_keys_off, span_base;
    std::vector<std::vector<uint32_t>> hist_offs, fac_out_offs;
    std::vector<FacetJob> jobs;
    uint32_t fac_out_total = 0;
    {
        static const uint64_t target1 = [] {
            const char* e = std::getenv("VQ_SPAN_TARGET");
            return uint64_t(e ? std::atoll(e) : 2048);
        }();
        const uint64_t target = std::min<uint64_t>(target1 + 64 * uint64_t(n - 1), std::max<uint64_t>(target1, 5120));
        uint64_t have = 0;
        for (size_t i = 0; i < n; ++i)
            if (pb->queries[i].status == 0) have += pb->queries[i].n_spans;
        if (have && have * 3 <= target * 2) {
            const uint64_t f = (target + have - 1) / have;
            for (size_t i = 0; i < n; ++i) {
                CompiledQuery& cq = pb->queries[i];
                if (cq.status == 0) cq.n_spans = uint32_t(std::max<uint64_t>(cq.n_spans, std::min<uint64_t>(uint64_t(cq.n_spans) * f, cq.max_spans)));
            }
        }
        static const bool weighted = std::getenv("VQ_NO_WEIGHTED_SPANS") == nullptr;
        uint64_t total_postings = 0;
        for (size_t i = 0; i < n; ++i)
            if (pb->queries[i].status == 0) total_postings += pb->queries[i].total_len;
        if (weighted && n > 1 && total_postings) {
            const uint64_t per_span = std::max<uint64_t>(total_postings / target, 4096);
            for (size_t i = 0; i < n; ++i) {
                CompiledQuery& cq = pb->queries[i];
                if (cq.status != 0) continue;
                const uint64_t want = std::min<uint64_t>((cq.total_len + per_span - 1) / per_span, cq.max_spans);
                cq.n_spans = uint32_t(std::max<uint64_t>(cq.n_spans, want));
            }
        }
    }
    for (size_t i = 0; i < n; ++i) {
        CompiledQuery& cq = pb->queries[i];
        if (cq.status != 0) continue;
        pb->slot[i] = nq++;
        keys_base.push_back(uint32_t(total_span_keys));
        part_keys_off.push_back(uint32_t(total_keys));
        span_base.push_back(uint32_t(total_spans));
        total_span_keys += uint64_t(cq.n_spans) * cq.top_k;
        total_keys += cq.top_k;
        total_spans += cq.n_spans;
        std::vector<uint32_t> ho, fo;
        for (auto& f : cq.facets) {
            ho.push_back(uint32_t(total_hist));
            fo.push_back(fac_out_total);
            jobs.push_back(FacetJob{uint32_t(total_hist), f.num_values, f.top, fac_out_total});
            total_hist += f.num_values;
            fac_out_total += f.top;
        }
        hist_offs.push_back(std::move(ho));
        fac_out_offs.push_back(std::move(fo));
        if (!cq.blob_bytes) size_blob(cq, idx);
        blob_bytes += cq.blob_bytes;
        max_lists = std::max<uint32_t>(max_lists, uint32_t(cq.lists.size()));
        max_ww = std::max(max_ww, cq.tile_words);
        stack_depth = std::max(stack_depth, cq.stack_depth);
    }
    if (total_span_keys > 0xFFFFFFFFull || total_hist > 0xFFFFFFFFull || total_spans > 0x7FFFFFFFull)
        throw VelociError(ERR_UNSUPPORTED, "batch too large for 32-bit workspace offsets: split the batch");
    span_base.push_back(uint32_t(total_spans));
    pb->nq_dev = nq;
    pb->total_spans = uint32_t(total_spans);
    pb->n_facet_jobs = uint32_t(jobs.size());
    pb->total_facet_out = fac_out_total;
    pb->facet_jobs = jobs;
    const double t_layout = now_ms();

    PartialLayout& lay = pb->layout;
    lay.nq = nq;
    lay.total_keys = total_keys;
    lay.total_hist = total_hist;
    lay.off_hits = 0;
    lay.off_stats = align_up(size_t(nq) * 8, 16);
    lay.off_keys = lay.off_stats + align_up(size_t(nq) * 8, 16);
    lay.off_hist = align_up(lay.off_keys + size_t(total_keys) * 8, 256);
    lay.bytes = align_up(lay.off_hist + size_t(total_hist) * 4, 256);

    const size_t up_blob_off = align_up(blob_bytes, 256);
    const size_t tbl = align_up(size_t(nq + 1) * 4, 256);
    const size_t up_span_base = up_blob_off + tbl;
    const size_t up_qmap_g = up_span_base + tbl;
    const size_t up_span_s = up_qmap_g + tbl;
    const size_t up_qmap_s = up_span_s + tbl;
    const size_t up_span_d = up_qmap_s + tbl;
    const size_t up_qmap_d = up_span_d + tbl;
    const size_t up_span_w = up_qmap_d + tbl;
    const size_t up_qmap_w = up_span_w + tbl;
    const size_t up_span_r = up_qmap_w + tbl;
    const size_t up_qmap_r = up_span_r + tbl;
    const size_t up_span_f = up_qmap_r + tbl;
    const size_t up_qmap_f = up_span_f + tbl;
    const size_t up_span_x = up_qmap_f + tbl;
    const size_t up_qmap_x = up_span_x + tbl;
    const size_t tbl_p = align_up(size_t(nq + 1 + kProbeShapes) * 4, 256);
    const size_t up_span_p = up_qmap_x + tbl;
    const size_t up_qmap_p = up_span_p + tbl_p;
    const size_t up_qmap_n = up_qmap_p + tbl_p;
    const size_t up_work_n = up_qmap_n + tbl;
    size_t ring_items_max = 0;
    for (size_t i = 0; i < n; ++i)
        if (pb->queries[i].status == 0 && ((pb->queries[i].simple_flags >> 26) & 1u)) ring_items_max += pb->queries[i].n_spans;
    const size_t up_items_n = up_work_n + 256;
    const size_t up_jobs = up_items_n + align_up(ring_items_max * 4, 256);
    const size_t up_bytes = up_jobs + align_up(jobs.size() * sizeof(FacetJob), 256) + 256;
    ws.h_up.ensure(up_bytes);
    ws.d_up.ensure(up_bytes);
    uint8_t* hup = ws.h_up.as<uint8_t>();
    uint8_t* dup = ws.d_up.as<uint8_t>();
    bool union_has_or = false;
    uint32_t scatter_wide = 0, scatter_simple = 0;
    uint32_t n_simple = 0, n_generic = 0, n_dense = 0, n_wide = 0, n_rich = 0, spans_simple = 0, spans_generic = 0, spans_dense = 0, spans_wide = 0, spans_rich = 0;
    uint32_t scatter_rich = 0;
    bool facets_rich = false;
    uint32_t n_leaf = 0, spans_leaf = 0;
    uint32_t n_xwide = 0, spans_xwide = 0, leaves_xwide = 0, scatter_xwide = 0;
    struct ProbeClass {
        uint32_t first = 0, n = 0, spans = 0;
        uint32_t na_seen = 0, arr_slot = 0;
    } pcls[kProbeShapes];
    auto probe_class = [](const CompiledQuery& cq) -> uint32_t {
        if ((cq.simple_flags >> 27) & 1u) return kProbeOr;
        const uint32_t nd = cq.simple_n - 1, na = uint32_t(__builtin_popcount((cq.simple_flags >> 12) & 0xFu));
        return nd <= 1 ? kProbeAnd1 : nd == 2 ? kProbeAnd2A0 + na : kProbeAnd3A0 + na;
    };
    auto on_probe = [](const CompiledQuery& cq) {
        return cq.status == 0 && ((cq.simple_flags >> 25) & 1u) && !((cq.simple_flags >> 26) & 1u) && !((cq.simple_flags >> 19) & 1u) && !((cq.simple_flags >> 24) & 1u) &&
               !((cq.simple_flags >> 18) & 1u);
    };
    bool any_probe = false;
    uint32_t n_ring = 0, items_ring = 0, nd_ring = 1, ring_spans_each = 0;
    uint64_t cls_layout[K_COUNT_] = {}, cls_algo[K_COUNT_] = {}, cls_q[K_COUNT_] = {};
    {
        size_t off = 0;
        uint32_t* hbo = reinterpret_cast<uint32_t*>(hup + up_blob_off);
        uint32_t qi = 0;
        for (size_t i = 0; i < n; ++i) {
            CompiledQuery& cq = pb->queries[i];
            if (cq.status != 0) continue;
            hbo[qi] = uint32_t(off);
            const size_t packed = pack_blob(cq, idx, hup + off, dup + off, keys_base[qi], part_keys_off[qi], hist_offs[qi], fac_out_offs[qi], nullptr,
                                            pb->profiled ? uint32_t((lay.off_stats - lay.off_hits) / 8 + qi) : 0u);
            if (packed != cq.blob_bytes) throw VelociError(ERR_DEVICE, "query blob changed size between compilation and packing (internal)");
            off += packed;
            ++qi;
        }
        hbo[nq] = uint32_t(off);
        uint32_t* sg = reinterpret_cast<uint32_t*>(hup + up_span_base);
        uint32_t* mg = reinterpret_cast<uint32_t*>(hup + up_qmap_g);
        uint32_t* ss = reinterpret_cast<uint32_t*>(hup + up_span_s);
        uint32_t* ms = reinterpret_cast<uint32_t*>(hup + up_qmap_s);
        uint32_t* sd = reinterpret_cast<uint32_t*>(hup + up_span_d);
        uint32_t* md = reinterpret_cast<uint32_t*>(hup + up_qmap_d);
        uint32_t* sw = reinterpret_cast<uint32_t*>(hup + up_span_w);
        uint32_t* mw = reinterpret_cast<uint32_t*>(hup + up_qmap_w);
        uint32_t* sr = reinterpret_cast<uint32_t*>(hup + up_span_r);
        uint32_t* mr = reinterpret_cast<uint32_t*>(hup + up_qmap_r);
        uint32_t* sf = reinterpret_cast<uint32_t*>(hup + up_span_f);
        uint32_t* mf = reinterpret_cast<uint32_t*>(hup + up_qmap_f);
        uint32_t accf = 0, accx = 0;
        uint32_t* sx = reinterpret_cast<uint32_t*>(hup + up_span_x);
        uint32_t* mx = reinterpret_cast<uint32_t*>(hup + up_qmap_x);
        uint32_t accg = 0, accs = 0, accd = 0, accw = 0, accr = 0;
        uint32_t* sp = reinterpret_cast<uint32_t*>(hup + up_span_p);
        uint32_t* mp = reinterpret_cast<uint32_t*>(hup + up_qmap_p);
        {
            uint32_t cnt[kProbeShapes] = {};
            for (size_t i = 0; i < n; ++i)
                if (on_probe(pb->queries[i])) ++cnt[probe_class(pb->queries[i])];
            uint32_t at = 0;
            for (uint32_t c = 0; c < kProbeShapes; ++c) {
                pcls[c].first = at;
                at += cnt[c] + 1;
            }
        }
        uint32_t* mn = reinterpret_cast<uint32_t*>(hup + up_qmap_n);
        uint32_t ring_max_spans = 0;
        std::vector<uint32_t> ring_ns;
        bool ring_uniform = true;
        std::memset(hup + up_work_n, 0, 256);
        qi = 0;
        for (size_t i = 0; i < n; ++i) {
            const CompiledQuery& cq = pb->queries[i];
            if (cq.status != 0) continue;
            static const bool union_enabled = std::getenv("VQ_NO_UNION") == nullptr;
            static const bool union_or = std::getenv("VQ_UNION_OR") != nullptr;
            const bool rich = (cq.simple_flags >> 18) & 1u;
            const bool dense = !rich && union_enabled && cq.simple_flags && (cq.simple_n == 1 || (union_or && cq.ops.back().kind == OP_OR));
            int kclass;
            if ((cq.simple_flags >> 19) & 1u) {
                kclass = K_SCAN_LEAF_F32;
                sf[n_leaf] = accf;
                mf[n_leaf++] = qi;
                accf += cq.n_spans;
            } else if ((cq.simple_flags >> 24) & 1u) {
                kclass = K_SCAN_WIDE;
                leaves_xwide = std::max<uint32_t>(leaves_xwide, cq.wide.n_leaves);
                scatter_xwide = std::max<uint32_t>(scatter_xwide, cq.wide.n_leaves - uint32_t(__builtin_popcount(cq.wide.bitmap_mask)));
                sx[n_xwide] = accx;
                mx[n_xwide++] = qi;
                accx += cq.n_spans;
            } else if (rich) {
                kclass = K_SCAN_RICH;
                facets_rich = facets_rich || !cq.facets.empty();
                scatter_rich = std::max<uint32_t>(scatter_rich, cq.simple_n - uint32_t(__builtin_popcount(cq.simple_flags & 0xFu)) + cq.simple2.n_side);
                sr[n_rich] = accr;
                mr[n_rich++] = qi;
                accr += cq.n_spans;
            } else if (dense) {
                kclass = K_SCAN_UNION;
                union_has_or = union_has_or || cq.simple_n > 1;
                sd[n_dense] = accd;
                md[n_dense++] = qi;
                accd += cq.n_spans;
            } else if ((cq.simple_flags >> 26) & 1u) {
                kclass = K_SCAN_RING;
                nd_ring = std::max<uint32_t>(nd_ring, cq.simple_n - 1);
                ring_uniform = ring_uniform && (n_ring == 0 || cq.n_spans == ring_max_spans);
                ring_max_spans = std::max(ring_max_spans, cq.n_spans);
                mn[n_ring++] = qi;
                ring_ns.push_back(cq.n_spans);
                items_ring += cq.n_spans;
            } else if ((cq.simple_flags >> 25) & 1u) {
                kclass = K_SCAN_PROBE;
                if (!on_probe(cq)) throw VelociError(ERR_DEVICE, "probe query outside the probe tables (internal)");
                ProbeClass& pc = pcls[probe_class(cq)];
                pc.na_seen |= 1u << uint32_t(__builtin_popcount((cq.simple_flags >> 12) & 0xFu));
                pc.arr_slot = std::max(pc.arr_slot, cq.probe_arr_gran * 4u);
                sp[pc.first + pc.n] = pc.spans;
                mp[pc.first + pc.n++] = qi;
                pc.spans += cq.n_spans;
                any_probe = true;
            } else if (cq.simple_flags && cq.simple_n > 1 && cq.ops.back().kind == OP_AND) {
                kclass = K_SCAN_AND;
                scatter_wide = std::max<uint32_t>(scatter_wide, cq.simple_n - uint32_t(__builtin_popcount(cq.simple_flags & 0xFu)));
                sw[n_wide] = accw;
                mw[n_wide++] = qi;
                accw += cq.n_spans;
            } else if (cq.simple_flags) {
                kclass = K_SCAN_SIMPLE;
                scatter_simple = std::max<uint32_t>(scatter_simple, cq.simple_n - uint32_t(__builtin_popcount(cq.simple_flags & 0xFu)));
                ss[n_simple] = accs;
                ms[n_simple++] = qi;
                accs += cq.n_spans;
            } else {
                kclass = K_TILE_SCAN;
                sg[n_generic] = accg;
                mg[n_generic++] = qi;
                accg += cq.n_spans;
            }
            pb->qclass.push_back(uint8_t(kclass));
            cls_layout[kclass] += cq.layout_bytes;
            cls_algo[kclass] += cq.algorithmic_bytes;
            cls_q[kclass] += 1;
            ++qi;
        }
        sg[n_generic] = accg;
        ss[n_simple] = accs;
        sw[n_wide] = accw;
        spans_wide = accw;
        sr[n_rich] = accr;
        spans_rich = accr;
        sf[n_leaf] = accf;
        spans_leaf = accf;
        sx[n_xwide] = accx;
        spans_xwide = accx;
        for (const ProbeClass& pc : pcls) sp[pc.first + pc.n] = pc.spans;
        if (n_ring) {
            if (ring_uniform) ring_spans_each = ring_max_spans;
            else {
                uint32_t* it = reinterpret_cast<uint32_t*>(hup + up_items_n);
                uint32_t k = 0;
                for (uint32_t r = 0; r < ring_max_spans; ++r)
                    for (uint32_t j = 0; j < n_ring; ++j)
                        if (r < ring_ns[j]) it[k++] = (j << 12) | r;
            }
        }
        sd[n_dense] = accd;
        spans_generic = accg;
        spans_simple = accs;
        spans_dense = accd;
        if (!jobs.empty()) std::memcpy(hup + up_jobs, jobs.data(), jobs.size() * sizeof(FacetJob));
    }
    pb->d_blobs = dup;
    pb->d_blob_off = reinterpret_cast<const uint32_t*>(dup + up_blob_off);
    pb->d_span_base = reinterpret_cast<const uint32_t*>(dup + up_span_base);
    pb->d_facet_jobs = reinterpret_cast<const FacetJob*>(dup + up_jobs);
    if (nq == 0) return pb;

    const double t_packed = now_ms();
    VQ_HIP(hipMemcpyAsync(dup, hup, up_bytes, hipMemcpyHostToDevice, st));
    ws.d_span_keys.ensure(size_t(total_span_keys) * 8 + 16);
    if (arena_offset >= 0) {
        if (size_t(arena_offset) % 256 || size_t(arena_offset) + lay.bytes > Index::kArenaBytes)
            throw VelociError(ERR_UNSUPPORTED, "partial arena: the step's partials do not fit (" + std::to_string(size_t(arena_offset) + lay.bytes) + " bytes)");
        idx.arena.ensure(Index::kArenaBytes);
        pb->d_partial = idx.arena.as<uint8_t>() + arena_offset;
    } else {
        ws.d_partial.ensure(lay.bytes);
        pb->d_partial = ws.d_partial.as<uint8_t>();
    }
    VQ_HIP(hipMemsetAsync(pb->d_partial, 0, lay.bytes, st));

    uint32_t max_top_k = 1;
    for (size_t i = 0; i < n; ++i)
        if (pb->queries[i].status == 0) max_top_k = std::max(max_top_k, pb->queries[i].top_k);
    uint32_t desc_cap = 0;
    for (size_t i = 0; i < n; ++i)
        if (pb->queries[i].status == 0) {
            desc_cap = std::max(desc_cap, uint32_t(pb->queries[i].desc_bytes));
        }
    desc_cap = uint32_t(align_up(desc_cap, 16));
    bool facets_generic = false;
    static const bool no_facet_cache = std::getenv("VQ_NO_FACET_CACHE") != nullptr;
    for (size_t i = 0; i < n; ++i)
        if (pb->queries[i].status == 0 && !pb->queries[i].simple_flags && !pb->queries[i].facets.empty()) facets_generic = !no_facet_cache;
    if (facets_generic) desc_cap += 2 * 1024 * 4;
    static const uint32_t cand_min = [] {
        const char* e = std::getenv("VQ_CAND_CAP");
        return uint32_t(e ? std::max(32, std::atoi(e)) : 32);
    }();
    uint32_t cand_cap = cand_min;
    while (cand_cap < 2 * max_top_k) cand_cap <<= 1;
    const uint32_t list_table = (std::max<uint32_t>(max_lists, 2) + 1u) & ~1u;
    static const bool tile_queue = std::getenv("VQ_NO_QUEUE") == nullptr;
    for (size_t i = 0; i < n; ++i)
        if (pb->queries[i].status == 0 && !pb->queries[i].simple_flags)
            lds_bytes = std::max(lds_bytes, tile_scan_lds_bytes(uint32_t(pb->queries[i].lists.size()) + pb->queries[i].n_temps, uint32_t(pb->queries[i].lists.size()), pb->queries[i].tile_words, stack_depth, cand_cap, desc_cap, tile_queue && !pb->queries[i].simple_n, list_table));
    if (lds_bytes > 160 * 1024) throw VelociError(ERR_UNSUPPORTED, "LDS tile larger than 160 KiB");
    const bool prof = pb->profiled;
    auto hits_ptr = reinterpret_cast<unsigned long long*>(pb->d_partial + lay.off_hits);
    auto hist_ptr = reinterpret_cast<uint32_t*>(pb->d_partial + lay.off_hist);
    auto keys_ptr = ws.d_span_keys.as<unsigned long long>();
    auto tab = [&](size_t o) { return reinterpret_cast<const uint32_t*>(dup + o); };
    if (spans_leaf) {
        LaunchTimer t(prof, ws, st, K_SCAN_LEAF_F32, cls_layout[K_SCAN_LEAF_F32], cls_algo[K_SCAN_LEAF_F32], cls_q[K_SCAN_LEAF_F32]);
        launch_scan_leaf_f32(st, spans_leaf, pb->d_blobs, pb->d_blob_off, tab(up_span_f), tab(up_qmap_f), n_leaf, cand_cap, keys_ptr, hits_ptr, hist_ptr);
    }
    VQ_HIP(hipGetLastError());
    if (spans_rich) {
        LaunchTimer t(prof, ws, st, K_SCAN_RICH, cls_layout[K_SCAN_RICH], cls_algo[K_SCAN_RICH], cls_q[K_SCAN_RICH]);
        launch_scan_simple(st, true, scatter_rich, spans_rich, pb->d_blobs, pb->d_blob_off, tab(up_span_r), tab(up_qmap_r), n_rich, cand_cap, keys_ptr, hits_ptr, hist_ptr, facets_rich);
    }
    VQ_HIP(hipGetLastError());
    if (items_ring) {
        static const uint32_t cus = [] {
            int dev = 0, v = 0;
            if (hipGetDevice(&dev) != hipSuccess || hipDeviceGetAttribute(&v, hipDeviceAttributeMultiprocessorCount, dev) != hipSuccess || v <= 0) v = 256;
            return uint32_t(v);
        }();
        LaunchTimer t(prof, ws, st, K_SCAN_RING, cls_layout[K_SCAN_RING], cls_algo[K_SCAN_RING], cls_q[K_SCAN_RING]);
        launch_scan_ring(st, nd_ring, cus, pb->d_blobs, pb->d_blob_off, tab(up_qmap_n), n_ring, ring_spans_each, tab(up_items_n), items_ring,
                         reinterpret_cast<uint32_t*>(dup + up_work_n), keys_ptr, hits_ptr);
    }
    VQ_HIP(hipGetLastError());
    if (any_probe) {
        LaunchTimer t(prof, ws, st, K_SCAN_PROBE, cls_layout[K_SCAN_PROBE], cls_algo[K_SCAN_PROBE], cls_q[K_SCAN_PROBE]);
        static const bool trace = std::getenv("VQ_PROBE_TRACE") != nullptr;
        for (uint32_t c = 0; c < kProbeShapes; ++c)
            if (pcls[c].spans && trace)
                std::fprintf(stderr, "probe launch: shape %u, %u queries, %u spans, array slot %u words (fullest tile: %u granules), NA seen 0x%x\n", c, pcls[c].n, pcls[c].spans,
                             pcls[c].arr_slot, pcls[c].arr_slot / 4, pcls[c].na_seen);
        for (uint32_t c = 0; c < kProbeShapes; ++c)
            if (pcls[c].spans)
                launch_scan_probe_shape(st, c, pcls[c].na_seen, pcls[c].arr_slot, pcls[c].spans, pb->d_blobs, pb->d_blob_off, tab(up_span_p) + pcls[c].first, tab(up_qmap_p) + pcls[c].first,
                                        pcls[c].n, cand_cap, keys_ptr, hits_ptr);
    }
    VQ_HIP(hipGetLastError());
    if (spans_wide) {
        LaunchTimer t(prof, ws, st, K_SCAN_AND, cls_layout[K_SCAN_AND], cls_algo[K_SCAN_AND], cls_q[K_SCAN_AND]);
        launch_scan_simple(st, false, scatter_wide, spans_wide, pb->d_blobs, pb->d_blob_off, tab(up_span_w), tab(up_qmap_w), n_wide, cand_cap, keys_ptr, hits_ptr, hist_ptr);
    }
    VQ_HIP(hipGetLastError());
    if (spans_simple) {
        LaunchTimer t(prof, ws, st, K_SCAN_SIMPLE, cls_layout[K_SCAN_SIMPLE], cls_algo[K_SCAN_SIMPLE], cls_q[K_SCAN_SIMPLE]);
        launch_scan_simple(st, false, scatter_simple, spans_simple, pb->d_blobs, pb->d_blob_off, tab(up_span_s), tab(up_qmap_s), n_simple, cand_cap, keys_ptr, hits_ptr, hist_ptr);
    }
    VQ_HIP(hipGetLastError());
    if (spans_dense) {
        LaunchTimer t(prof, ws, st, K_SCAN_UNION, cls_layout[K_SCAN_UNION], cls_algo[K_SCAN_UNION], cls_q[K_SCAN_UNION]);
        launch_scan_union(st, union_has_or, spans_dense, pb->d_blobs, pb->d_blob_off, tab(up_span_d), tab(up_qmap_d), n_dense, cand_cap, keys_ptr, hits_ptr);
    }
    VQ_HIP(hipGetLastError());
    if (spans_xwide) {
        LaunchTimer t(prof, ws, st, K_SCAN_WIDE, cls_layout[K_SCAN_WIDE], cls_algo[K_SCAN_WIDE], cls_q[K_SCAN_WIDE]);
        launch_scan_wide(st, leaves_xwide, scatter_xwide, spans_xwide, pb->d_blobs, pb->d_blob_off, tab(up_span_x), tab(up_qmap_x), n_xwide, cand_cap, keys_ptr, hits_ptr);
    }
    VQ_HIP(hipGetLastError());
    if (spans_generic) {
        LaunchTimer t(prof, ws, st, K_TILE_SCAN, cls_layout[K_TILE_SCAN], cls_algo[K_TILE_SCAN], cls_q[K_TILE_SCAN]);
        launch_tile_scan(st, spans_generic, lds_bytes, pb->d_blobs, pb->d_blob_off, pb->d_span_base, tab(up_qmap_g), n_generic, stack_depth, cand_cap, desc_cap, keys_ptr,
                         hits_ptr, hist_ptr, tile_queue, list_table, facets_generic);
    }
    VQ_HIP(hipGetLastError());
    {
        LaunchTimer t(prof, ws, st, K_MERGE_SPANS, total_span_keys * 8 + total_keys * 8, total_span_keys * 8 + total_keys * 8, nq);
        launch_merge_spans(st, nq, pb->d_blobs, pb->d_blob_off, keys_ptr, reinterpret_cast<unsigned long long*>(pb->d_partial + lay.off_keys));
    }
    VQ_HIP(hipGetLastError());
    VQ_HIP(hipEventRecord(ws.ev_done, st));
    pb->launched = true;
    if (timing_enabled())
        std::fprintf(stderr, "[vq timing] n=%zu compile %.3f ms (dictionary scans %.3f [%zu probes], pass 1 %.3f, unions %.3f [%zu jobs], pass 2 %.3f), range jobs %.3f [%zu], spans generic/simple/and/rich/union %u/%u/%u/%u/%u, pack+launch %.3f ms\n", n,
                     t_compiled - t_start, t_probes - t_start, fuzzy.size(), t_pass1 - t_probes, t_unions - t_pass1, unions.size(), t_compiled - t_ranges,
                     t_ranges - t_unions, ranges.size(), spans_generic, spans_simple, spans_wide, spans_rich, spans_dense + spans_leaf, now_ms() - t_compiled);
    if (timing_enabled())
        std::fprintf(stderr, "[vq timing] pack+launch: span sizing + layout %.3f, blobs + tables %.3f, upload + launches %.3f ms\n", t_layout - t_compiled, t_packed - t_layout, now_ms() - t_packed);
    if (timing_enabled()) {
        uint64_t v[16];
        for (int k = 0; k < 16; ++k) v[k] = g_compile_ns[k].exchange(0);
        if (std::getenv("VQ_TIMING_SUB")) {
            std::fprintf(stderr, "[vq timing] inside 1:n resolve (thread-ms; 6 value-id gather, 7 sort, 8 pairs, 9 order check + layers):");
            for (int k = 6; k < 10; ++k) std::fprintf(stderr, " [%d] %.3f", k, v[k] * 1e-6);
            std::fprintf(stderr, "\n");
        }
        std::fprintf(stderr, "[vq timing] compile thread-ms: total %.3f = dictionary lookups %.3f + 1:n resolve %.3f + 1:n layers %.3f + leaf lists %.3f + rest %.3f; longest request %.3f\n", v[5] * 1e-6,
                     v[0] * 1e-6, v[1] * 1e-6, (v[2] - v[1]) * 1e-6, v[3] * 1e-6, (double(v[5]) - double(v[0]) - double(v[2]) - double(v[3])) * 1e-6, v[4] * 1e-6);
    }
    return pb;
}

std::vector<SuggestEntry> run_suggest(const Index& idx, const vqreq::Request& req) {
    if (!req.suggest) throw VelociError(ERR_INVALID_REQUEST, "only suggest allowed in suggest function");
    VQ_HIP(hipSetDevice(idx.device));
    FuzzyTable fuzzy;
    collect_suggest_probes(idx, req, fuzzy);
    if (!fuzzy.empty()) {
        Workspace& ws = idx.ws[idx.next_ws.fetch_add(1) % kWorkspaces];
        std::unique_lock<std::mutex> lock(ws.mu);
        ws.timed.clear();
        ws.ev_used = 0;
        run_fuzzy_probes(idx, ws, fuzzy, idx.pre_stream ? idx.pre_stream : idx.stream);
    }
    std::vector<SuggestEntry> out;
    for (auto& part : *req.suggest) {
        auto one = suggest_part(idx, part, fuzzy.empty() ? nullptr : &fuzzy);
        out.insert(out.end(), one.begin(), one.end());
    }
    std::stable_sort(out.begin(), out.end(), [](const SuggestEntry& a, const SuggestEntry& b) { return a.text > b.text; });
    std::vector<SuggestEntry> merged;
    for (auto& e : out) {
        if (!merged.empty() && merged.back().text == e.text) {
            if (e.score > merged.back().score) merged.back().score = e.score;
        } else merged.push_back(e);
    }
    std::stable_sort(merged.begin(), merged.end(), [](const SuggestEntry& a, const SuggestEntry& b) { return a.score > b.score; });
    const size_t skip = std::min(req.skip.value_or(0), merged.size());
    merged.erase(merged.begin(), merged.begin() + skip);
    if (req.top && merged.size() > *req.top) merged.resize(*req.top);
    return merged;
}

std::vector<SuggestEntry> run_highlight(const Index& idx, vqreq::RequestSearchPart part) {
    for (auto& t : part.terms) t = vqtext::normalize_text(t);
    VQ_HIP(hipSetDevice(idx.device));
    vqreq::Request probe_req;
    probe_req.suggest = std::vector<vqreq::RequestSearchPart>{part};
    FuzzyTable fuzzy;
    collect_suggest_probes(idx, probe_req, fuzzy);
    if (!fuzzy.empty()) {
        Workspace& ws = idx.ws[idx.next_ws.fetch_add(1) % kWorkspaces];
        std::unique_lock<std::mutex> lock(ws.mu);
        ws.timed.clear();
        ws.ev_used = 0;
        run_fuzzy_probes(idx, ws, fuzzy, idx.pre_stream ? idx.pre_stream : idx.stream);
    }
    std::vector<SuggestEntry> out = highlight_part(idx, part, fuzzy.empty() ? nullptr : &fuzzy);
    std::stable_sort(out.begin(), out.end(), [](const SuggestEntry& a, const SuggestEntry& b) { return a.score > b.score; });
    const size_t skip = std::min(part.skip.value_or(0), out.size());
    out.erase(out.begin(), out.begin() + skip);
    if (part.top && out.size() > *part.top) out.resize(*part.top);
    return out;
}

vqreq::Request page_request_after(const vqreq::Request& R, float score, uint32_t id) {
    vqreq::Request page = R;
    page.top = size_t(kMaxTopK);
    page.skip = 0;
    page.facets.reset();
    uint32_t bits;
    std::memcpy(&bits, &score, 4);
    page.key_upper = (uint64_t(order_f32(bits)) << 32) | id;
    return page;
}

void complete_deep_requests(const Index& idx, const vqreq::Request* const* reqs, size_t n, std::vector<std::unique_ptr<Result>>& results,
                            std::vector<int>& status, std::vector<std::string>& errors) {
    constexpr uint64_t kMaxDeep = 65536;
    for (size_t i = 0; i < n; ++i) {
        if (status[i] != 0 || !results[i] || !results[i]->deep) continue;
        const vqreq::Request& R = *reqs[i];
        Result& out = *results[i];
        out.deep = false;
        const uint64_t top = R.top.value_or(10), skip = R.skip.value_or(0);
        const uint64_t want = top + skip < top ? ~0ull : top + skip;
        std::vector<uint32_t> ids = std::move(out.ids);
        std::vector<float> scores = std::move(out.scores);
        out.ids.clear();
        out.scores.clear();
        if (skip >= out.num_hits) continue;
        const uint64_t reach = std::min<uint64_t>(want, out.num_hits);
        if (reach > kMaxDeep) {
            status[i] = ERR_UNSUPPORTED;
            errors[i] = "unsupported on the MI355X query path: top + skip reaches more than " + std::to_string(kMaxDeep) + " ranked hits";
            results[i].reset();
            continue;
        }
        vqreq::Request page = R;
        page.top = size_t(kMaxTopK);
        page.skip = 0;
        page.facets.reset();
        bool failed = false;
        while (ids.size() < reach && ids.size() % size_t(kMaxTopK) == 0 && !ids.empty()) {
            uint32_t bits;
            std::memcpy(&bits, &scores.back(), 4);
            page.key_upper = (uint64_t(order_f32(bits)) << 32) | ids.back();
            const vqreq::Request* arr[1] = {&page};
            std::vector<std::unique_ptr<Result>> r;
// ... 437 lines not shown
```

### veloci_amd/csrc/index.cpp

```cpp
#include <algorithm>
#include <atomic>
#include <chrono>
#include <cstring>
#include <exception>
#include <mutex>
#include <thread>
#include <sys/mman.h>

#include "engine.hpp"
#include "text.hpp"

namespace vq {

const char* const TOKENS_TO_TEXT_ID = ".tokens_to_text_id";
const char* const TO_ANCHOR_ID_SCORE = ".to_anchor_id_score";
const char* const PHRASE_PAIR_TO_ANCHOR = ".phrase_pair_to_anchor";
const char* const VALUE_ID_TO_PARENT = ".value_id_to_parent";
const char* const PARENT_TO_VALUE_ID = ".parent_to_value_id";
const char* const TEXT_ID_TO_ANCHOR = ".text_id_to_anchor";
const char* const ANCHOR_TO_TEXT_ID = ".anchor_to_text_id";
const char* const BOOST_VALID_TO_VALUE = ".boost_valid_to_value";
const char* const TOKEN_VALUES = ".token_values";
const char* const VALUE_ID_TO_ANCHOR = ".value_id_to_anchor";
const char* const TEXTINDEX = ".textindex";
// ... 139 lines not shown

    for (auto& [path, f] : b.fst) {
        Dictionary d;
        d.terms = f.terms;
        d.lower_map.reserve(d.terms.size());
        for (uint32_t i = 0; i < d.terms.size(); ++i) d.lower_map[vqtext::to_lower_utf8(d.terms[i])].push_back(i);
        {
            std::vector<uint32_t> off(d.terms.size() + 1, 0u);
            std::vector<uint32_t> raw, low;
            for (uint32_t i = 0; i < d.terms.size(); ++i) {
                for (uint32_t cp : vqtext::decode_utf8(d.terms[i])) {
                    if (cp > 0xFFFFu) d.char_bytes = 4;
                    if (cp == 0x130u) d.low_exact = false;
                    raw.push_back(cp);
                    low.push_back(vqtext::lower_cp(cp));
                }
                off[i + 1] = uint32_t(raw.size());
            }
            auto image = [&](DevBuf& dst, const std::vector<uint32_t>& cps) {
                if (d.char_bytes == 4) {
                    dst.alloc(cps.size() * 4 + 16);
                    dst.upload(cps.data(), cps.size() * 4);
                } else {
                    const std::vector<uint16_t> narrow(cps.begin(), cps.end());
                    dst.alloc(narrow.size() * 2 + 16);
                    dst.upload(narrow.data(), narrow.size() * 2);
                }
            };
            d.d_off.alloc(off.size() * 4 + 16);
            d.d_off.upload(off.data(), off.size() * 4);
            image(d.d_raw, raw);
            image(d.d_low, low);
            idx->device_bytes += d.d_off.bytes + d.d_raw.bytes + d.d_low.bytes;
        }
        idx->dict.emplace(path, std::move(d));
    }

    const size_t nthreads = host_threads();
    auto upload = [&](DevBuf& dst, const void* src, size_t n) {
        const size_t piece = size_t(256) << 20;
        parallel_for((n + piece - 1) / piece, nthreads, [&](size_t i) {
            VQ_HIP(hipSetDevice(device));
            const size_t off = i * piece;
            VQ_HIP(hipMemcpy(dst.as<uint8_t>() + off, static_cast<const uint8_t*>(src) + off, std::min(piece, n - off), hipMemcpyHostToDevice));
        });
    };
    for (const auto& kv : b.postings) {
        const std::string& path = kv.first;
        const HostPostings& p = kv.second;
        PostingStore ps;
        ps.num_tokens = uint32_t(p.offsets.size() - 1);
        ps.start.resize(ps.num_tokens);
        ps.len.resize(ps.num_tokens);
        ps.global_len.resize(ps.num_tokens);
        ps.max_raw.assign(ps.num_tokens, 0);
        std::vector<uint64_t> src_at(ps.num_tokens);
        uint64_t total = 0;
        for (uint32_t t = 0; t < ps.num_tokens; ++t) {
            const uint32_t* rb = p.anchors.data() + p.offsets[t];
            const uint32_t* re = p.anchors.data() + p.offsets[t + 1];
            const uint32_t *sb, *se;
            shard_subrange(rb, re, lo, hi, &sb, &se);
            src_at[t] = uint64_t(sb - p.anchors.data());
            ps.start[t] = total;
            ps.len[t] = uint32_t(se - sb);
            ps.global_len[t] = p.global_lens.empty() ? uint64_t(re - rb) : p.global_lens[t];
            total += (uint64_t(ps.len[t]) + 3u) & ~uint64_t(3);
        }
        uninit_vector<uint32_t> docs(total);
        uninit_vector<uint16_t> scores(total);
        parallel_for(ps.num_tokens, nthreads, [&](size_t t) {
            const uint64_t s0 = ps.start[t], n = ps.len[t], padded = (n + 3u) & ~uint64_t(3);
            std::memcpy(docs.data() + s0, p.anchors.data() + src_at[t], n * 4);
            const uint32_t* sc = p.scores.data() + src_at[t];
            uint16_t most = 0;
            for (uint64_t i = 0; i < n; ++i) {
                const uint16_t h = f32_to_f16_rne(float(sc[i]));
                scores[s0 + i] = h;
                most = std::max(most, h);
            }
            for (uint64_t i = n; i < padded; ++i) {
                docs[s0 + i] = 0xFFFFFFFFu;
                scores[s0 + i] = 0;
            }
            ps.max_raw[t] = most;
        });
        ps.total_padded = total;
        ps.bm_start.assign(ps.num_tokens, -1);
        ps.rd_start.assign(ps.num_tokens, -1);
        {
            const uint64_t range = uint64_t(hi) - lo;
            const uint64_t words = idx->bitmap_words, blocks = words >> (kRankShift - 5);
            std::vector<uint32_t> dense;
            for (uint32_t t = 0; t < ps.num_tokens; ++t)
                if (range >= 65536 && uint64_t(ps.len[t]) * 64 >= range) dense.push_back(t);
            if (!dense.empty()) {
                uninit_vector<uint32_t> bits(words * dense.size());
                uninit_vector<uint32_t> rdir((blocks + 1) * dense.size());
                parallel_for(dense.size(), nthreads, [&](size_t k) {
                    const uint32_t t = dense[k];
                    uint32_t* bw = bits.data() + words * k;
                    uint32_t* rd = rdir.data() + (blocks + 1) * k;
                    std::memset(bw, 0, words * 4);
                    std::memset(rd, 0, (blocks + 1) * 4);
                    const uint32_t* d = docs.data() + ps.start[t];
                    for (uint32_t i = 0; i < ps.len[t]; ++i) {
                        const uint32_t rel = d[i] - idx->bitmap_base;
                        bw[rel >> 5] |= 1u << (rel & 31u);
                        rd[(rel >> kRankShift) + 1] += 1;
                    }
                    for (uint64_t bl = 1; bl <= blocks; ++bl) rd[bl] += rd[bl - 1];
                    ps.bm_start[t] = int64_t(words * k);
                    ps.rd_start[t] = int64_t((blocks + 1) * k);
                });
                ps.bitmaps.alloc(bits.size() * 4 + 16);
                upload(ps.bitmaps, bits.data(), bits.size() * 4);
                ps.rank_dir.alloc(rdir.size() * 4 + 16);
                upload(ps.rank_dir, rdir.data(), rdir.size() * 4);
                idx->device_bytes += ps.bitmaps.bytes + ps.rank_dir.bytes;
            }
        }
        ps.td_start.assign(ps.num_tokens, -1);
        std::vector<uint32_t> tiled;
        {
            const uint64_t range = uint64_t(hi) - lo;
            const uint64_t tiles = (idx->bitmap_words >> (kTileDirShift - 5)) + 3;
            for (uint32_t t = 0; t < ps.num_tokens; ++t) {
                if (range < 65536 || uint64_t(ps.len[t]) * 4096 < range) continue;
                ps.td_start[t] = int64_t(tiled.size() * (tiles + 1));
                tiled.push_back(t);
            }
            std::vector<uint32_t> tdir(tiled.size() * (tiles + 1));
            parallel_for(tiled.size(), nthreads, [&](size_t j) {
                const uint32_t t = tiled[j];
                const uint32_t* d = docs.data() + ps.start[t];
                uint32_t* out = tdir.data() + j * (tiles + 1);
                uint32_t i = 0;
                for (uint64_t k = 0; k <= tiles; ++k) {
                    const uint64_t bound = uint64_t(idx->bitmap_base) + (k << kTileDirShift);
                    while (i < ps.len[t] && d[i] < bound) ++i;
                    out[k] = i;
                }
            });
            if (!tdir.empty()) {
                ps.tile_dir.alloc(tdir.size() * 4 + 16);
                ps.tile_dir.upload(tdir.data(), tdir.size() * 4);
                idx->device_bytes += ps.tile_dir.bytes;
            }
        }
        ps.pk_start.assign(ps.num_tokens, -1);
        ps.ak_start.assign(ps.num_tokens, -1);
        ps.gd_start.assign(ps.num_tokens, -1);
        ps.tile_most.assign(ps.num_tokens, 0);
        {
            const uint64_t ptiles = (idx->bitmap_words >> (kProbeTileShift - 5)) + 2;
            uint64_t cov_gran = 0, arr_gran = 0;
            std::vector<uint32_t> gd(tiled.size() * (ptiles + 1));
            std::vector<uint64_t> gran_of(tiled.size());
            std::vector<uint32_t> most_of(tiled.size());
            parallel_for(tiled.size(), nthreads, [&](size_t j) {
                const uint32_t t = tiled[j];
                const uint32_t* d = docs.data() + ps.start[t];
                uint32_t* g = gd.data() + j * (ptiles + 1);
                uint64_t gran = 0;
                uint32_t i = 0, most = 0;
                for (uint64_t k = 0; k <= ptiles; ++k) {
                    g[k] = uint32_t(gran);
                    const uint64_t thi = uint64_t(idx->bitmap_base) + ((k + 1) << kProbeTileShift);
                    const uint32_t i0 = i;
                    while (i < ps.len[t] && d[i] < thi) ++i;
                    const uint32_t n8 = (i - i0 + 7u) / 8u;
                    most = std::max(most, n8);
                    gran += n8;
                }
                gran_of[j] = gran;
                most_of[j] = most;
            });
            for (size_t j = 0; j < tiled.size(); ++j) {
                const uint32_t t = tiled[j];
                ps.gd_start[t] = int64_t(j * (ptiles + 1));
                if (gran_of[j] >= (1ull << 28)) throw VelociError(vqreq::ERR_INVALID_ARGUMENT, "posting list too long for its tile-packed image");
                ps.pk_start[t] = int64_t(cov_gran);
                ps.tile_most[t] = most_of[j];
                cov_gran += gran_of[j];
                if (most_of[j] <= 256) {
                    ps.ak_start[t] = int64_t(arr_gran);
                    arr_gran += gran_of[j];
                }
            }
            if (cov_gran) {
                ps.cov32.alloc(cov_gran * 32 + 4096);
                ps.arr16.alloc(arr_gran * 16 + 4096);
                ps.gdir.alloc(gd.size() * 4 + 16);
                ps.gdir.upload(gd.data(), gd.size() * 4);
                idx->device_bytes += ps.cov32.bytes + ps.arr16.bytes + ps.gdir.bytes;
                uninit_vector<uint32_t> cov(cov_gran * 8);
                uninit_vector<uint16_t> arr(arr_gran * 8);
                parallel_for(tiled.size(), nthreads, [&](size_t j) {
                    const uint32_t t = tiled[j];
                    const bool as_array = ps.ak_start[t] >= 0;
                    const uint32_t* d = docs.data() + ps.start[t];
                    const uint16_t* sc = scores.data() + ps.start[t];
                    uint32_t* c = cov.data() + uint64_t(ps.pk_start[t]) * 8;
                    uint16_t* a = as_array ? arr.data() + uint64_t(ps.ak_start[t]) * 8 : nullptr;
                    uint64_t w = 0;
                    uint32_t i = 0;
                    for (uint64_t k = 0; k <= ptiles; ++k) {
                        const uint64_t tlo = uint64_t(idx->bitmap_base) + (k << kProbeTileShift), thi = tlo + (1u << kProbeTileShift);
                        for (; i < ps.len[t] && d[i] < thi; ++i, ++w) {
                            const uint32_t rel = uint32_t(d[i] - tlo);
                            c[w] = rel << 16 | sc[i];
                            if (a) a[w] = uint16_t(rel);
                        }
                        for (; w % 8; ++w) {
                            c[w] = 0xFFFFFFFFu;
                            if (a) a[w] = 0xFFFFu;
                        }
                    }
                });
                upload(ps.cov32, cov.data(), cov.size() * 4);
                upload(ps.arr16, arr.data(), arr.size() * 2);
            }
        }
        ps.docs.alloc(docs.size() * 4 + 16);
        upload(ps.docs, docs.data(), docs.size() * 4);
        ps.scores.alloc(scores.size() * 2 + 16);
        upload(ps.scores, scores.data(), scores.size() * 2);
        idx->device_bytes += ps.docs.bytes + ps.scores.bytes;
        idx->postings.emplace(path, std::move(ps));
    }

    for (auto& [path, k] : b.kv) {
        KVStore s;
        s.key_base = k.key_base;
        s.num_keys = uint32_t(k.offsets.size() - 1);
        s.host_off = k.offsets;
        s.host_values = k.values;
        bool identity_t2t = false;
        if (ends_with(path, TOKENS_TO_TEXT_ID)) {
            std::string ti = path.substr(0, path.size() - std::strlen(TOKENS_TO_TEXT_ID));
            identity_t2t = idx->is_anchor_identity(ti);
        }
        s.list_rows = ends_with(path, TEXT_ID_TO_ANCHOR) || identity_t2t;
        if (identity_t2t) {
            std::string pp = path.substr(0, path.size() - std::strlen(TOKENS_TO_TEXT_ID)) + TO_ANCHOR_ID_SCORE;
            auto bit = b.postings.find(pp);
            if (bit != b.postings.end() && bit->second.offsets.size() == k.offsets.size() && k.key_base == 0) {
                const auto& po = bit->second;
                bool same = po.offsets == k.offsets && po.anchors.size() == k.values.size() &&
                            std::memcmp(po.anchors.data(), k.values.data(), k.values.size() * 4) == 0;
                s.rows_equal_postings = same;
            }
        }
        if (s.list_rows) {
            s.start.resize(s.num_keys);
            s.len.resize(s.num_keys);
            std::vector<uint32_t> vals;
            vals.reserve(k.values.size() + 4);
            std::vector<uint32_t> tmp;
            for (uint32_t r = 0; r < s.num_keys; ++r) {
                const uint32_t* rb = k.values.data() + k.offsets[r];
                const uint32_t* re = k.values.data() + k.offsets[r + 1];
                if (!std::is_sorted(rb, re) || std::adjacent_find(rb, re) != re) {
                    tmp.assign(rb, re);
                    std::sort(tmp.begin(), tmp.end());
                    tmp.erase(std::unique(tmp.begin(), tmp.end()), tmp.end());
                    rb = tmp.data();
                    re = tmp.data() + tmp.size();
                    s.rows_sorted_unique = false;
                }
                const uint32_t *sb, *se;
                shard_subrange(rb, re, lo, hi, &sb, &se);
                s.start[r] = vals.size();
                s.len[r] = uint32_t(se - sb);
                append_padded(vals, sb, se);
            }
            s.values.alloc(vals.size() * 4 + 16);
            s.values.upload(vals.data(), vals.size() * 4);
            idx->device_bytes += s.values.bytes;
            if (ends_with(path, TEXT_ID_TO_ANCHOR)) {
                s.d_row_start.alloc(s.start.size() * 8 + 16);
                s.d_row_start.upload(s.start.data(), s.start.size() * 8);
                s.d_row_len.alloc(s.len.size() * 4 + 16);
                s.d_row_len.upload(s.len.data(), s.len.size() * 4);
                idx->device_bytes += s.d_row_start.bytes + s.d_row_len.bytes;
            }
        }
        if (ends_with(path, TOKENS_TO_TEXT_ID) && !identity_t2t) {
            s.text_csr = true;
            s.d_text_vals.alloc(k.values.size() * 4 + 16);
            s.d_text_vals.upload(k.values.data(), k.values.size() * 4);
            idx->device_bytes += s.d_text_vals.bytes;
        }
        if (ends_with(path, VALUE_ID_TO_PARENT) || ends_with(path, VALUE_ID_TO_ANCHOR)) {
            s.value_csr = true;
            s.d_text_vals.alloc(k.values.size() * 4 + 16);
            s.d_text_vals.upload(k.values.data(), k.values.size() * 4);
            s.d_csr_off.alloc(k.offsets.size() * 8 + 16);
            s.d_csr_off.upload(k.offsets.data(), k.offsets.size() * 8);
            idx->device_bytes += s.d_text_vals.bytes + s.d_csr_off.bytes;
        }
        s.facet_csr = ends_with(path, ANCHOR_TO_TEXT_ID) || (ends_with(path, PARENT_TO_VALUE_ID) && path.find("[]") == std::string::npos);
        if (s.facet_csr) {
            const uint64_t kb = k.key_base, ke = uint64_t(k.key_base) + s.num_keys;
            const uint64_t nb = std::min<uint64_t>(std::max<uint64_t>(kb, lo), ke);
            const uint64_t ne = std::max<uint64_t>(nb, std::min<uint64_t>(ke, hi));
            std::vector<uint64_t> off(ne - nb + 1);
            const uint64_t first = k.offsets[nb - kb];
            for (uint64_t r = nb; r <= ne; ++r) off[r - nb] = k.offsets[r - kb] - first;
            s.csr_off.alloc(off.size() * 8);
            s.csr_off.upload(off.data(), off.size() * 8);
            const uint64_t nvals = k.offsets[ne - kb] - first;
            s.csr_values.alloc(nvals * 4 + 16);
            s.csr_values.upload(k.values.data() + first, nvals * 4);
            idx->device_bytes += s.csr_off.bytes + s.csr_values.bytes;
            s.csr_key_base = uint32_t(nb);
            s.csr_num_keys = uint32_t(ne - nb);
            for (uint64_t e = first; e < first + nvals; ++e) s.csr_max_value = std::max(s.csr_max_value, k.values[e]);
            bool single = true;
            for (size_t r = 0; r + 1 < off.size() && single; ++r) single = off[r + 1] - off[r] <= 1;
            if (single && s.csr_num_keys) {
                std::vector<uint32_t> direct(s.csr_num_keys, 0xFFFFFFFFu);
                for (size_t r = 0; r + 1 < off.size(); ++r)
                    if (off[r + 1] > off[r]) direct[r] = k.values[first + off[r]];
                s.csr_direct.alloc(direct.size() * 4 + 16);
                s.csr_direct.upload(direct.data(), direct.size() * 4);
                idx->device_bytes += s.csr_direct.bytes;
            }
        }
        idx->kv.emplace(path, std::move(s));
    }

    for (auto& [path, p] : b.phrase) {
        PhraseStore s;
        const size_t n = p.t1.size();
        s.keys.reserve(n);
        s.start.resize(n);
        s.len.resize(n);
        std::vector<uint32_t> vals;
        for (size_t i = 0; i < n; ++i) {
            s.keys.push_back({p.t1[i], p.t2[i]});
            const uint32_t* rb = p.anchors.data() + p.offsets[i];
            const uint32_t* re = p.anchors.data() + p.offsets[i + 1];
            const uint32_t *sb, *se;
            shard_subrange(rb, re, lo, hi, &sb, &se);
            s.start[i] = vals.size();
            s.len[i] = uint32_t(se - sb);
            append_padded(vals, sb, se);
        }
        if (!std::is_sorted(s.keys.begin(), s.keys.end())) throw VelociError(vqreq::ERR_INVALID_ARGUMENT, "phrase pair keys must be sorted by (t1, t2): " + path);
        s.anchors.alloc(vals.size() * 4 + 16);
        s.anchors.upload(vals.data(), vals.size() * 4);
        idx->device_bytes += s.anchors.bytes;
        idx->phrase.emplace(path, std::move(s));
    }

    for (auto& [path, bc] : b.boost) {
        BoostColumn c;
        c.key_base = bc.key_base;
        c.num_keys = uint32_t(bc.bits.size());
        for (size_t i = 0; i < bc.bits.size(); ++i) {
            if (!bc.present.empty() && !bc.present[i]) continue;
            float v;
            std::memcpy(&v, &bc.bits[i], 4);
            if (v != v) {
                c.has_nan = true;
                continue;
            }
            c.vmin = c.any_value ? std::min(c.vmin, v) : v;
            c.vmax = c.any_value ? std::max(c.vmax, v) : v;
// ... 69 lines not shown
```

### veloci_amd/csrc/kernels.hpp

```cpp
#pragma once
#include <hip/hip_runtime.h>
#include <stddef.h>
#include <stdint.h>

#include "device_types.hpp"

namespace vq {

struct DictProbe {
    uint32_t m, max_d, flags, lm;
    uint16_t query[64];
    uint16_t lquery[64];
};
struct DictProbeW {
    uint32_t m, max_d, flags, lm;
    uint32_t q_off;
    uint32_t lq_off;
    uint32_t pad[2];
};
constexpr uint32_t kDictMaxPattern = 1u << 20;
struct DictMatch {
    uint32_t probe, term;
    uint32_t info;
};

struct UList {
    const uint32_t* docs;
    const void* scores;
    uint32_t len;
    float term_score;
    uint32_t flags, pad;
};
struct RangeJobD {
    uint32_t list_begin, n_lists, anchor_begin, n_anchors, block_begin, pad;
};
struct UTask {
    uint32_t list_begin, n_lists;
    uint32_t span_begin, n_spans;
    uint32_t pivot, pad;
};

struct FacetJob {
    uint32_t hist_off, num_values, top, out_off;
};

size_t tile_scan_lds_bytes(uint32_t n_bitmaps, uint32_t n_lists, uint32_t tile_words, uint32_t stack_depth, uint32_t cand_cap, uint32_t desc_cap, bool queue, uint32_t ml);

void launch_tile_scan(hipStream_t st, uint32_t total_spans, size_t lds_bytes, const uint8_t* blobs, const uint32_t* blob_off, const uint32_t* span_base,
                      const uint32_t* qmap, uint32_t nq, uint32_t stack_depth, uint32_t cand_cap, uint32_t desc_cap, unsigned long long* span_keys, unsigned long long* num_hits, uint32_t* hist, bool queue, uint32_t ml,
                      bool facet_cache = false);
void launch_scan_leaf_f32(hipStream_t st, uint32_t total_spans, const uint8_t* blobs, const uint32_t* blob_off, const uint32_t* span_base, const uint32_t* qmap,
                          uint32_t nq, uint32_t cand_cap, unsigned long long* span_keys, unsigned long long* num_hits, uint32_t* hist);
size_t scan_simple_lds_bytes(uint32_t cand_cap, uint32_t nv, uint32_t n_scatter, bool facet_cache);
uint32_t debug_div100_mismatches();
int debug_facet_select(const uint32_t* hist_host, uint32_t num_values, uint32_t top, uint32_t misalign, uint32_t* out_vals_host, uint32_t* out_counts_host);
void launch_scan_simple(hipStream_t st, bool wide, uint32_t n_scatter, uint32_t total_spans, const uint8_t* blobs, const uint32_t* blob_off, const uint32_t* span_base,
                        const uint32_t* qmap, uint32_t nq, uint32_t cand_cap, unsigned long long* span_keys, unsigned long long* num_hits, uint32_t* hist, bool facet_cache = false);
enum : uint32_t { kProbeAnd1 = 0, kProbeAnd2A0, kProbeAnd2A1, kProbeAnd2A2, kProbeAnd3A0, kProbeAnd3A1, kProbeAnd3A2, kProbeAnd3A3, kProbeOr, kProbeShapes };
size_t scan_probe_lds_bytes(uint32_t cand_cap, uint32_t nd, uint32_t na, uint32_t arr_slot);
uint32_t debug_probe_occupancy(uint32_t shape, size_t lds_bytes);
void launch_scan_probe_shape(hipStream_t st, uint32_t shape, uint32_t na_seen, uint32_t arr_slot, uint32_t total_spans, const uint8_t* blobs, const uint32_t* blob_off,
                             const uint32_t* span_base, const uint32_t* qmap, uint32_t nq, uint32_t cand_cap, unsigned long long* span_keys, unsigned long long* num_hits);
uint32_t scan_ring_consumers(uint32_t max_nd);
uint32_t scan_ring_slots(uint32_t maxnd, uint32_t consumers);
size_t scan_ring_lds_bytes(uint32_t maxnd, uint32_t consumers, uint32_t slots);
void launch_scan_ring(hipStream_t st, uint32_t max_nd, uint32_t grid, const uint8_t* blobs, const uint32_t* blob_off, const uint32_t* qmap, uint32_t nq, uint32_t spans_each,
                      const uint32_t* items, uint32_t total_items, uint32_t* work, unsigned long long* span_keys, unsigned long long* num_hits);
size_t scan_wide_lds_bytes(uint32_t cand_cap, uint32_t n_leaves, uint32_t n_scatter);
void launch_scan_wide(hipStream_t st, uint32_t max_leaves, uint32_t max_scatter, uint32_t total_spans, const uint8_t* blobs, const uint32_t* blob_off, const uint32_t* span_base,
                      const uint32_t* qmap, uint32_t nq, uint32_t cand_cap, unsigned long long* span_keys, unsigned long long* num_hits);
void launch_merge_spans(hipStream_t st, uint32_t nq, const uint8_t* blobs, const uint32_t* blob_off, const unsigned long long* span_keys,
                        unsigned long long* part_keys);
void launch_finalize(hipStream_t st, uint32_t nq, const uint8_t* blobs, const uint32_t* blob_off, const uint8_t* gathered, uint32_t num_shards,
                     size_t shard_stride, const PartialLayout& lay, uint32_t* res_ids, float* res_scores, uint32_t* res_n, unsigned long long* res_hits);
void launch_facet_select(hipStream_t st, uint32_t n_jobs, const FacetJob* jobs, const uint32_t* hist, uint32_t* out_vals, uint32_t* out_counts,
                         uint32_t* out_n);

void launch_range_hits(hipStream_t st, uint32_t n_blocks, uint32_t n_jobs, const UList* ulists, const RangeJobD* jobs, const uint32_t* anchors, unsigned long long* counts);
void launch_union(hipStream_t st, bool write, uint32_t total_spans, const UList* ulists, const UTask* tasks, const uint32_t* span_task, uint32_t* span_cnt,
                  const uint64_t* span_off, uint32_t* out_docs, float* out_vals, uint32_t* task_min);
constexpr uint32_t kDenseBlockDocs = 2048;
struct UDenseList {
    const uint32_t* docs;
    const uint16_t* scores;
    uint64_t first;
    float term_score;
    uint32_t job;
};
struct UDenseJob {
    uint64_t slab_off;
    uint64_t out_off;
    uint32_t block_begin, n_blocks;
    uint32_t result, pad;
};
struct UDenseResult {
    uint32_t len, max_key;
};
void launch_union_dense_scatter(hipStream_t st, const UDenseList* lists, uint32_t n_lists, uint64_t total_postings, const UDenseJob* jobs, uint32_t* slab, uint32_t lo_doc,
                                uint32_t range);
void launch_union_dense_count(hipStream_t st, const UDenseJob* jobs, uint32_t n_jobs, uint32_t n_blocks, const uint32_t* slab, uint32_t* block_cnt, uint32_t* block_max,
                              UDenseResult* results);
void launch_union_dense_write(hipStream_t st, const UDenseJob* jobs, uint32_t n_jobs, uint32_t n_blocks, const uint32_t* slab, const uint32_t* block_off, uint32_t lo_doc,
                              uint32_t* out_docs, float* out_vals);
void launch_scan_union(hipStream_t st, bool with_or, uint32_t total_spans, const uint8_t* blobs, const uint32_t* blob_off, const uint32_t* span_base, const uint32_t* qmap,
                       uint32_t nq, uint32_t cand_cap, unsigned long long* span_keys, unsigned long long* num_hits);
void launch_dict_scan(hipStream_t st, const DictProbe* d_probes, uint32_t probe_base, uint32_t n_probes, const uint32_t* off, const uint16_t* chars, const uint16_t* low_chars,
                      uint32_t num_terms, uint32_t* out_count, uint32_t out_cap, DictMatch* out);
void launch_dict_scan_wide(hipStream_t st, uint32_t char_bytes, const DictProbeW* d_probes, const uint32_t* pool, uint32_t probe_base, uint32_t n_probes, const uint32_t* off,
                           const void* chars, const void* low_chars, uint32_t num_terms, uint32_t* out_count, uint32_t out_cap, DictMatch* out);

struct LocRow {
    uint64_t src, dst;
    uint32_t len, pad;
};
struct LocJob {
    const uint32_t* t2a_vals;
    const uint64_t* t2a_start;
    const uint32_t* t2a_len;
    uint32_t t2a_key_base, t2a_num_keys;
    uint32_t seg_begin, seg_end;
    uint32_t pair_begin, pair_end;
    uint32_t out_off, pad;
};
void launch_loc_gather(hipStream_t st, const LocRow* rows, uint32_t n_rows, const uint32_t* table, uint32_t* gathered);
void launch_loc_expand(hipStream_t st, bool write, const LocJob* jobs, uint32_t n_jobs, const uint32_t* sorted_text_ids, uint32_t n, uint32_t* totals_or_cursors,
                       unsigned long long* pairs);
void launch_loc_compact(hipStream_t st, const LocJob* jobs, uint32_t n_jobs, const unsigned long long* sorted_pairs, uint32_t* out_docs, float* out_vals, uint32_t* out_len);
size_t seg_sort_u32(void* tmp, size_t tmp_bytes, const uint32_t* in, uint32_t* out, uint32_t n, uint32_t nseg, const uint32_t* seg_begin, const uint32_t* seg_end,
                    hipStream_t st);
size_t seg_sort_u64(void* tmp, size_t tmp_bytes, const unsigned long long* in, unsigned long long* out, uint32_t n, uint32_t nseg, const uint32_t* seg_begin,
                    const uint32_t* seg_end, hipStream_t st);

struct B1nJob {
    const uint32_t* boost_present;
    const float* boost_values;
    const uint64_t* to_anchor_off;
    const uint32_t* to_anchor_vals;
    uint32_t boost_key_base, boost_num_keys, to_anchor_key_base, to_anchor_num_keys;
    uint32_t seg_begin, seg_end, out_off, doc_lo, doc_hi, pad;
};
struct B1nResult {
    uint32_t len, total, flags, pad;
};
void launch_b1n_map(hipStream_t st, const B1nJob* jobs, uint32_t n_jobs, const uint32_t* sorted_value_ids, uint32_t* out_docs, float* out_vals, B1nResult* results);

struct ExList {
    const uint32_t* docs;
    const uint16_t* scores;
    uint32_t len;
    float term_score;
};
constexpr uint32_t XP_LEAF = 0, XP_AND = 1, XP_OR = 2;
struct ExOp {
    uint32_t kind, nchild;
    uint32_t a;
    uint32_t b;
};
struct ExQuery {
    uint32_t op_begin, n_ops, list_begin, n_lists, col_begin, n_col;
    uint32_t doc_begin, trace_begin;
};
constexpr uint32_t kExStack = 256;
__host__ __device__ inline uint32_t explain_trace_words(uint32_t n_lists, uint32_t n_ops, uint32_t n_col) { return 3u * (n_lists + n_ops + n_col + 1u); }
void launch_explain(hipStream_t st, uint32_t n_docs, const ExQuery* queries, const uint32_t* doc_query, const uint32_t* docs, const ExOp* ops, const uint16_t* aux,
                    const ExList* lists, const DColBoost* cols, uint32_t* trace);

#ifdef VQ_STAMP
void debug_read_stamps(unsigned long long* out, int reset);
void debug_read_probe_stamps(unsigned long long* out, int reset);
void debug_read_ring_stamps(unsigned long long* out, int reset);
#endif

}
```

### veloci_amd/csrc/scan_probe.hip

```cpp
#include <hip/hip_runtime.h>
#include <hip/hip_fp16.h>

#include "device_types.hpp"
#include "kernel_common.hpp"
#include "kernels.hpp"
#include "probe_common.hpp"

namespace vq {

#ifdef VQ_STAMP
__device__ unsigned long long g_probe_stamp[16];
#define PS_INIT                                                      \
    unsigned long long _st0 = __builtin_amdgcn_s_memtime();          \
    const unsigned long long _t0 = _st0;                             \
    const unsigned long long _r0 = __builtin_amdgcn_s_memrealtime(); \
    unsigned long long _acc[16] = {0};
#define PS_AT(k)                                                \
    {                                                           \
        unsigned long long _st1 = __builtin_amdgcn_s_memtime(); \
        _acc[k] += _st1 - _st0;                                 \
        _st0 = _st1;                                            \
    }
#define PS_COUNT(k) _acc[k] += 1ull;
#define PS_FLUSH                                                                                             \
    _acc[14] = __builtin_amdgcn_s_memtime() - _t0;                        \
    _acc[15] = __builtin_amdgcn_s_memrealtime() - _r0;                \
    if (threadIdx.x == 0) {                                                                                  \
        _Pragma("unroll") for (int _k = 0; _k < 16; ++_k) if (_acc[_k]) atomicAdd(&g_probe_stamp[_k], _acc[_k]); \
    }
void debug_read_probe_stamps(unsigned long long* out, int reset) {
    (void)hipMemcpyFromSymbol(out, HIP_SYMBOL(g_probe_stamp), sizeof(unsigned long long) * 16);
    if (reset) {
        unsigned long long z[16] = {0};
        (void)hipMemcpyToSymbol(HIP_SYMBOL(g_probe_stamp), z, sizeof z);
    }
}
#else
#define PS_INIT
#define PS_AT(k)
#define PS_COUNT(k)
#define PS_FLUSH
#endif

constexpr uint32_t kPMaxR = 2;
constexpr uint32_t kPU = 256;
static_assert(kPU >= 256, "a round of 256 postings must fit the empty queue");
constexpr uint32_t kPR = 128;
constexpr uint32_t kPLdsShape = 8;
constexpr uint32_t kPLdsU = kPLdsShape + 24;
constexpr uint32_t kPLdsR = kPLdsU + kPU;
__host__ __device__ constexpr uint32_t probe_lds_tile(uint32_t nd) { return kPLdsR + (2 + nd) * kPR; }
__host__ __device__ constexpr uint32_t probe_lds_arr(uint32_t nd, uint32_t nb) { return probe_lds_tile(nd) + nb * (kPTW + kPRk); }
size_t scan_probe_lds_bytes(uint32_t cand_cap, uint32_t nd, uint32_t na, uint32_t arr_slot) {
    return (size_t)(probe_lds_arr(nd, nd - na) + na * arr_slot + 2 * cand_cap) * 4 + 16;
}

template <uint32_t ND, uint32_t NA, bool OR = false>
__device__ __forceinline__ void probe_body(const uint8_t* __restrict__ blob, const uint32_t span, const uint32_t q, const uint32_t cand_cap, const uint32_t arr_slot,
                                           unsigned long long* __restrict__ span_keys, unsigned long long* __restrict__ num_hits) {
    extern __shared__ __attribute__((aligned(16))) uint32_t lds[];
    const uint32_t lane = threadIdx.x;
    const VQ_CONST QHeader* H = as_const<QHeader>(blob);
    const VQ_CONST DList* gl = as_const<DList>(blob + H->off_lists);
    const VQ_CONST DOp* gops = as_const<DOp>(blob + H->off_ops);
    const VQ_CONST DProbe* P = as_const<DProbe>(blob + H->off_simple2);
    const uint32_t sflags = H->simple_flags;
    const uint32_t top_k = H->top_k;
    constexpr uint32_t n = ND + 1u;
    constexpr uint32_t NB = ND - NA;
    constexpr uint32_t NB1 = NB ? NB : 1u, NA1 = NA ? NA : 1u;
    PS_INIT

    unsigned long long* thr = reinterpret_cast<unsigned long long*>(lds);
    uint32_t* cand_n = lds + 2;
    uint32_t* sh = lds + kPLdsShape;
    uint32_t* uq = lds + kPLdsU;
    uint32_t* rq = lds + kPLdsR;
    uint32_t* tile = lds + probe_lds_tile(ND);
    uint32_t* rank = tile + NB * kPTW;
    uint32_t* arr = lds + probe_lds_arr(ND, NB);
    unsigned long long* cand = reinterpret_cast<unsigned long long*>(arr + NA * arr_slot);
    unsigned long long* const gthr = reinterpret_cast<unsigned long long*>(const_cast<uint8_t*>(blob) + offsetof(QHeader, gthr));
    CandState cs{cand, cand_n, thr, cand_cap, gthr};
    cs.upper = H->key_upper;
    uint32_t* const stat = H->stat_off ? lds + 4 : nullptr;
    uint8_t* const pool = H->off_pool ? const_cast<uint8_t*>(blob) + H->off_pool : nullptr;

    const uint32_t* ccov = nullptr;
    const uint32_t* cgdir = nullptr;
    const uint32_t* d_bitmap[NB1];
    const uint32_t* d_rank[NB1];
    const uint16_t* d_arr[NA1];
    const uint32_t* d_agd[NA1];
    {
        const uint32_t ck = (uint32_t)__ffs((int)((sflags >> 8) & 0xFu)) - 1u;
        const uint32_t am = (sflags >> 12) & 0xFu;
        uint32_t role_of[4] = {0u, 0u, 0u, 0u};
        uint32_t ib = 0, ia = NB;
#pragma unroll
        for (uint32_t k = 0; k < n; ++k) {
            const VQ_CONST DList& d = gl[gops[k].list_begin];
            if (k == ck) {
                ccov = P->leaf[k].cov32;
                cgdir = P->leaf[k].gdir;
                if (lane == 0) {
                    sh[kShCts] = __float_as_uint(d.term_score);
                    sh[kShPrunable] = (d.term_score > 0.0f && d.max_raw < 0x7C00u) ? 1u : 0u;
                }
            } else {
                const bool is_arr = ((am >> k) & 1u) != 0u;
                const uint32_t role = is_arr ? ia : ib;
#pragma unroll
                for (uint32_t j = 0; j < NB; ++j)
                    if (!is_arr && j == role) {
                        d_bitmap[j] = d.bitmap;
                        d_rank[j] = d.rank_dir;
                    }
#pragma unroll
                for (uint32_t a = 0; a < NA; ++a)
                    if (is_arr && NB + a == role) {
                        d_arr[a] = P->leaf[k].arr16;
                        d_agd[a] = P->leaf[k].gdir;
                    }
                if (lane == 0) {
                    const uint16_t mr = d.max_raw;
                    sh[kShTs + role] = __float_as_uint(d.term_score);
                    sh[kShVmax + role] = (d.term_score > 0.0f && mr < 0x7C00u) ? __float_as_uint(posting_value(d.term_score, mr)) : 0x7F800000u;
                    reinterpret_cast<unsigned long long*>(sh + kShScores)[role] = is_arr ? (unsigned long long)(uintptr_t)P->leaf[k].cov32 : (unsigned long long)(uintptr_t)d.scores;
                }
                role_of[k] = 1u + role;
                if (is_arr) ++ia;
                else ++ib;
            }
        }
        const KOp root(gops + n);
#pragma unroll
        for (uint32_t j = 0; j < n; ++j) {
            const uint32_t k = OR ? j : root.and_order(j);
            if (lane == 0) sh[kShSrc + j] = k == 0u ? role_of[0] : k == 1u ? role_of[1] : k == 2u ? role_of[2] : role_of[3];
        }
    }

    const uint32_t n_spans = H->n_spans;
    const unsigned long long range = (unsigned long long)(H->doc_hi - H->doc_lo);
    const uint32_t span_lo = span == 0 ? H->doc_lo : ((H->doc_lo + (uint32_t)(range * span / n_spans)) & ~(kPT - 1u));
    const uint32_t span_hi = span + 1 == n_spans ? H->doc_hi : ((H->doc_lo + (uint32_t)(range * (span + 1) / n_spans)) & ~(kPT - 1u));
    const uint32_t bitmap_base = H->bitmap_base;
    const uint32_t keys_base = H->keys_base;

    if (lane == 0) {
        *thr = __hip_atomic_load(gthr, __ATOMIC_RELAXED, __HIP_MEMORY_SCOPE_AGENT);
        *cand_n = 0;
        lds[4] = 0u;
    }
    __syncthreads();
    unsigned long long thr_seen = *thr;
    uint32_t raw_min = 0u;
    constexpr uint32_t kMasks = OR ? (1u << ND) : 1u;
    uint32_t rmin[kMasks];
    auto take_raw_min = [&](const float thr_f) {
        if (OR) {
#pragma unroll
            for (uint32_t m = 0; m < kMasks; ++m) rmin[m] = probe_raw_min<ND>(sh, thr_f, lane, m);
        } else raw_min = probe_raw_min<ND>(sh, thr_f, lane);
    };
    take_raw_min(__uint_as_float(unorder_f32((uint32_t)(thr_seen >> 32))));

    const u32x4 kSent = u32x4{0xFFFFFFFFu, 0xFFFFFFFFu, 0xFFFFFFFFu, 0xFFFFFFFFu};
    const VQ_GLOBAL u32x4* cc4 = as_global(reinterpret_cast<const u32x4*>(ccov));

    uint32_t un = 0, rn = 0;
    uint32_t ucnt = 0;
    unsigned long long hits = 0;
    unsigned long long g_prev = 0ull;

    const uint32_t t_first = (span_lo - bitmap_base) >> kProbeTileShift;
    const uint32_t t_end = span_hi > span_lo ? ((span_hi - 1u - bitmap_base) >> kProbeTileShift) + 1u : t_first;
    uint32_t dir_base = t_first;
    auto load_dir = [&](const uint32_t* g) { return as_global(g)[dir_base + lane < t_end ? dir_base + lane : t_end]; };
    uint32_t dirv = load_dir(cgdir);
    uint32_t adv[NA1];
#pragma unroll
    for (uint32_t a = 0; a < NA; ++a) adv[a] = load_dir(d_agd[a]);
    auto dir_at = [&](const uint32_t v, const uint32_t tt) { return (uint32_t)__builtin_amdgcn_readlane((int)v, (int)(tt - dir_base)); };

    u32x4 wk[ND][kPNV];
    uint32_t rk[NB1];
    u32x4 nid[kPMaxR], cid[kPMaxR];
#pragma unroll
    for (uint32_t r = 0; r < kPMaxR; ++r) nid[r] = cid[r] = kSent;
    uint32_t pf_rounds = 0, pf_v0 = 0, pf_v1 = 0;
    uint32_t na_g0[NA1], na_nv[NA1];
    uint32_t a_g0[NA1], a_cnt[NA1];
#pragma unroll
    for (uint32_t a = 0; a < NA1; ++a) na_g0[a] = na_nv[a] = a_g0[a] = a_cnt[a] = 0u;
    auto issue_tile = [&](const uint32_t tt, const uint32_t g0, const uint32_t g1) {
        pf_rounds = (g1 - g0 + 31u) >> 5;
        pf_v0 = g0 * 2u;
        pf_v1 = g1 * 2u;
        if (OR || pf_rounds) {
#pragma unroll
            for (uint32_t i = 0; i < NB; ++i) {
                const VQ_GLOBAL u32x4* gb = as_global(reinterpret_cast<const u32x4*>(d_bitmap[i] + (size_t)tt * kPTW));
#pragma unroll
                for (uint32_t h = 0; h < kPNV; ++h) wk[i][h] = gb[h * 64u + lane];
                rk[i] = as_global(d_rank[i])[tt * kPRk + lane];
            }
#pragma unroll
            for (uint32_t a = 0; a < NA; ++a) {
                const VQ_GLOBAL u32x4* ga = as_global(reinterpret_cast<const u32x4*>(d_arr[a]) + na_g0[a]);
#pragma unroll
                for (uint32_t h = 0; h < kPNV; ++h)
                    if (h * 64u + lane < na_nv[a]) wk[NB + a][h] = ga[h * 64u + lane];
            }
#pragma unroll
            for (uint32_t r = 0; r < kPMaxR; ++r) {
                const uint32_t v = pf_v0 + r * 64u + lane;
                nid[r] = kSent;
                if (r < pf_rounds && v < pf_v1) nid[r] = cc4[v];
            }
        }
    };

    uint32_t tile_lo = 0;
    uint32_t f_stage = 0;
    uint32_t f_doc = 0, f_idx[ND];
    float f_vc = 0.0f, f_vd[ND];
    uint16_t f_r = 0;
    bool f_alive = false;
#pragma unroll
    for (uint32_t i = 0; i < ND; ++i) {
        f_idx[i] = 0u;
        f_vd[i] = 0.0f;
    }
    uint32_t rhead = 0;
    uint32_t tiles_since_merge = 8;
    auto push_keys = [&](const unsigned long long key, bool pending, const bool final) {
        if (wballot(pending)) {
            while (true) {
                if (pending) {
                    if (key > *thr) {
                        uint32_t pos = atomicAdd(cs.n, 1u);
                        if (pos < cs.cap) {
                            cs.cand[pos] = key;
                            pending = false;
                        }
                    } else pending = false;
                }
                probe_lds_fence();
                if (!wballot(pending)) break;
                cand_prune(cs, top_k);
            }
            if (pool && (tiles_since_merge >= 8u || final)) {
                PS_COUNT(13)
                tiles_since_merge = 0;
                probe_pool_merge<true>(cs, top_k, pool, lane);
            }
            const unsigned long long tn = *thr;
            if ((uint32_t)(tn >> 32) != (uint32_t)(thr_seen >> 32)) take_raw_min(__uint_as_float(unorder_f32((uint32_t)(tn >> 32))));
            thr_seen = tn;
        }
    };
    uint32_t f_mask = 0;
    auto sum_of = [&](const ProbeShape<ND>& S, const float vc, const float (&vd)[ND], const uint32_t mask) { return OR ? probe_or_sum<ND>(S, vc, vd, mask) : probe_sum<ND>(S, vc, vd); };
    auto flush_final = [&](const ProbeShape<ND>& S, const bool final) {
        const float score = sum_of(S, f_vc, f_vd, f_mask);
        const unsigned long long key = ((unsigned long long)order_f32(__float_as_uint(score)) << 32) | (unsigned long long)f_doc;
        f_stage = 0;
        PS_COUNT(12)
        push_keys(key, f_alive && key > *thr && key < cs.upper, final);
    };
    auto flush_service = [&](const bool final) {
        const unsigned long long* sptr = reinterpret_cast<const unsigned long long*>(sh + kShScores);
        unsigned long long gp = sptr[0];
        uint32_t gidx = 0u;
        if (f_stage) {
            const ProbeShape<ND> S = probe_shape<ND>(sh);
            const float thr_f = __uint_as_float(unorder_f32((uint32_t)(*thr >> 32)));
            bool last = true;
#pragma unroll
            for (uint32_t i = 0; i < ND; ++i)
                if (f_stage == i + 1u) {
                    f_vd[i] = posting_value(S.ts[i], f_r);
                    if (i + 1u < ND) {
                        constexpr uint32_t zero = 0;
                        f_alive = f_alive && !(sum_of(S, f_vc, f_vd, f_mask) < thr_f);
                        if (stat && lane == 0) *stat += 2u * (uint32_t)__popcll(wballot(f_alive));
                        gp = sptr[i + 1u < ND ? i + 1u : zero];
                        gidx = (f_alive && (!OR || ((f_mask >> (i + 1u < ND ? i + 1u : zero)) & 1u))) ? f_idx[i + 1u < ND ? i + 1u : zero] : 0u;
                        last = false;
                    }
                }
            if (last) flush_final(S, final);
            else ++f_stage;
        } else if (rn >= 64u || (final && rn)) {
            const uint32_t count = rn < 64u ? rn : 64u;
            probe_lds_fence();
            f_alive = lane < count;
            uint32_t raw = 0;
            const uint32_t slot = (rhead + lane) & (kPR - 1u);
            if (f_alive) {
                f_doc = rq[slot];
                raw = rq[kPR + slot];
#pragma unroll
                for (uint32_t i = 0; i < ND; ++i) f_idx[i] = rq[(2u + i) * kPR + slot];
            }
            if (OR) {
                f_mask = 0u;
#pragma unroll
                for (uint32_t i = 0; i < ND; ++i) f_mask |= f_idx[i] != 0xFFFFFFFFu ? 1u << i : 0u;
            }
            f_vc = posting_value(__uint_as_float(sh[kShCts]), (uint16_t)raw);
#pragma unroll
            for (uint32_t i = 0; i < ND; ++i) f_vd[i] = __uint_as_float(sh[kShVmax + i]);
            if (stat && lane == 0) *stat += 2u * count;
            gidx = (f_alive && (!OR || (f_mask & 1u))) ? f_idx[0] : 0u;
            f_stage = 1u;
            rhead = (rhead + count) & (kPR - 1u);
            rn -= count;
        }
        f_r = as_global(reinterpret_cast<const uint16_t*>((uintptr_t)gp))[gidx];
    };
    auto flush_sync = [&]() {
        const ProbeShape<ND> S = probe_shape<ND>(sh);
        probe_lds_fence();
        const uint32_t slot = (rhead + lane) & (kPR - 1u);
        const uint32_t doc = rq[slot];
        const float vc = posting_value(S.cts, (uint16_t)rq[kPR + slot]);
        float vd[ND];
        uint32_t mask = 0;
#pragma unroll
        for (uint32_t i = 0; i < ND; ++i) {
            const uint16_t* sp = reinterpret_cast<const uint16_t*>((uintptr_t) reinterpret_cast<const unsigned long long*>(sh + kShScores)[i]);
            const uint32_t ix = rq[(2u + i) * kPR + slot];
            if (ix != 0xFFFFFFFFu) mask |= 1u << i;
            vd[i] = posting_value(S.ts[i], as_global(sp)[(OR && ix == 0xFFFFFFFFu) ? 0u : ix]);
        }
        if (stat && lane == 0) *stat += 2u * ND * 64u;
        const float score = sum_of(S, vc, vd, mask);
        const unsigned long long key = ((unsigned long long)order_f32(__float_as_uint(score)) << 32) | (unsigned long long)doc;
        rhead = (rhead + 64u) & (kPR - 1u);
        rn -= 64u;
        push_keys(key, key > *thr && key < cs.upper, false);
    };
    auto bitmap_rank = [&](const uint32_t i, const uint32_t rel) {
        const uint32_t g = rel >> kRankShift, wi = (rel >> 5) & 15u, below = (1u << (rel & 31u)) - 1u;
        const int full = (int)((1u << wi) - 1u);
        const uint32_t* tl = tile + i * kPTW;
        uint32_t acc = rank[i * kPRk + g] + (uint32_t)__popc(tl[rel >> 5] & below);
        const u32x4* gw = reinterpret_cast<const u32x4*>(tl + g * 16u);
#pragma unroll
        for (uint32_t v4 = 0; v4 < 4; ++v4) {
            const u32x4 x = gw[v4];
            acc += (uint32_t)__popc(x.x & (uint32_t)__builtin_amdgcn_sbfe(full, v4 * 4u + 0u, 1u));
            acc += (uint32_t)__popc(x.y & (uint32_t)__builtin_amdgcn_sbfe(full, v4 * 4u + 1u, 1u));
            acc += (uint32_t)__popc(x.z & (uint32_t)__builtin_amdgcn_sbfe(full, v4 * 4u + 2u, 1u));
            acc += (uint32_t)__popc(x.w & (uint32_t)__builtin_amdgcn_sbfe(full, v4 * 4u + 3u, 1u));
        }
        return acc;
    };
    auto rank_some = [&](const uint32_t cnt) {
        while (rn + cnt > kPR) flush_sync();
        probe_lds_fence();
        const uint32_t* const uqe = uq + (un - cnt);
        un -= cnt;
        if (NA == 0u && ND == 2u && cnt <= 32u) {
            const uint32_t el = lane & 31u, role = lane >> 5;
            if (el < cnt) {
                const uint32_t e = uqe[el];
                const uint32_t rel = e >> 16;
                const uint32_t slot = (rhead + rn + el) & (kPR - 1u);
                if (role == 0u) {
                    rq[slot] = tile_lo + rel;
                    rq[kPR + slot] = e & 0xFFFFu;
                }
                const bool here = !OR || ((tile[role * kPTW + (rel >> 5)] >> (rel & 31u)) & 1u) != 0u;
                rq[(2u + role) * kPR + slot] = here ? bitmap_rank(role, rel) : 0xFFFFFFFFu;
            }
            rn += cnt;
        } else if (NA == 0u) {
            if (lane < cnt) {
                const uint32_t e = uqe[lane];
                const uint32_t rel = e >> 16;
                const uint32_t slot = (rhead + rn + lane) & (kPR - 1u);
                rq[slot] = tile_lo + rel;
                rq[kPR + slot] = e & 0xFFFFu;
#pragma unroll
                for (uint32_t i = 0; i < NB; ++i) {
                    const bool here = !OR || ((tile[i * kPTW + (rel >> 5)] >> (rel & 31u)) & 1u) != 0u;
                    rq[(2u + i) * kPR + slot] = here ? bitmap_rank(i, rel) : 0xFFFFFFFFu;
                }
            }
            rn += cnt;
        } else {
            uint32_t e = 0xFFFFFFFFu, pos[NA1];
            bool found = lane < cnt;
            if (found) e = uqe[lane];
            const uint32_t rel = e >> 16;
#pragma unroll
            for (uint32_t a = 0; a < NA; ++a) {
                const uint16_t* A = reinterpret_cast<const uint16_t*>(arr + a * arr_slot);
                uint32_t lo = 0u, len = a_cnt[a];
#ifdef VQ_PROBE_NO_SEARCH
                lo = rel & 7u;
                len = 0u;
#endif
                while (len > 1u) {
                    const uint32_t half = len >> 1;
                    lo = (uint32_t)A[lo + half] <= rel ? lo + half : lo;
                    len -= half;
                }
#ifdef VQ_PROBE_NO_SEARCH
                found = found && a_cnt[a] != 0u && ((uint32_t)A[lo] ^ rel) < 0x2000u;
#else
                found = found && a_cnt[a] != 0u && (uint32_t)A[lo] == rel;
#endif
                pos[a] = lo;
            }
            const unsigned long long fm = wballot(found);
            hits += (unsigned long long)__popcll(fm);
            const bool live = found && (e & 0xFFFFu) >= raw_min;
            const unsigned long long lm = wballot(live);
            if (lm) {
                if (live) {
                    const uint32_t slot = (rhead + rn + (uint32_t)__popcll(lm & ((1ull << lane) - 1ull))) & (kPR - 1u);
                    rq[slot] = tile_lo + rel;
                    rq[kPR + slot] = e & 0xFFFFu;
#pragma unroll
                    for (uint32_t i = 0; i < NB; ++i) rq[(2u + i) * kPR + slot] = bitmap_rank(i, rel);
#pragma unroll
                    for (uint32_t a = 0; a < NA; ++a) rq[(2u + NB + a) * kPR + slot] = (a_g0[a] * 8u + pos[a]) * 2u;
                }
                rn += (uint32_t)__popcll(lm);
            }
        }
    };
    uint32_t lo_rel = 0, width = 0;
    struct ProbeWords {
        uint32_t w[OR ? ND : 1u][4];
    };
    auto probe_read = [&](const u32x4 e4) {
        const uint32_t ee[4] = {e4.x, e4.y, e4.z, e4.w};
        ProbeWords pw;
#pragma unroll
        for (uint32_t c = 0; c < 4; ++c) {
            const uint32_t a = (ee[c] >> 21) & (kPTW - 1u);
            if (OR) {
#pragma unroll
                for (uint32_t i = 0; i < ND; ++i) pw.w[OR ? i : 0u][c] = tile[i * kPTW + a];
            } else {
                pw.w[0][c] = 0xFFFFFFFFu;
                if (NB) {
                    pw.w[0][c] = tile[a];
#pragma unroll
                    for (uint32_t i = 1; i < NB; ++i) pw.w[0][c] &= tile[i * kPTW + a];
                }
            }
        }
        return pw;
    };
    auto probe_eval = [&](const u32x4 e4, const ProbeWords& pw, const bool may_overflow) {
        const uint32_t ee[4] = {e4.x, e4.y, e4.z, e4.w};
        unsigned long long lm[4];
        bool live[4];
#pragma unroll
        for (uint32_t c = 0; c < 4; ++c) {
            const uint32_t rel = ee[c] >> 16;
            const bool in = (rel - lo_rel) < width;
            if (OR) {
                uint32_t mask = 0;
#pragma unroll
                for (uint32_t i = 0; i < ND; ++i) mask |= ((pw.w[OR ? i : 0u][c] >> (rel & 31u)) & 1u) << i;
                uint32_t need = rmin[0];
#pragma unroll
                for (uint32_t m = 1; m < kMasks; ++m) need = mask == m ? rmin[OR ? m : 0u] : need;
                hits += (unsigned long long)__popcll(wballot(in && mask == 0u));
                live[c] = in && (ee[c] & 0xFFFFu) >= need;
                lm[c] = wballot(live[c]);
                continue;
            }
            const bool bit = ((pw.w[0][c] >> (rel & 31u)) & 1u) != 0u;
            const unsigned long long sm = NB ? (wballot(in) & wballot(bit)) : wballot(in);
            if (NA == 0u) {
                const bool strong = (ee[c] & 0xFFFFu) >= raw_min;
                hits += (unsigned long long)__popcll(sm);
                lm[c] = sm & wballot(strong);
                live[c] = in && bit && strong;
            } else {
                lm[c] = sm;
                live[c] = in && bit;
            }
        }
        if (lm[0] | lm[1] | lm[2] | lm[3]) {
            if (may_overflow) {
                const uint32_t add = (uint32_t)__popcll(lm[0]) + (uint32_t)__popcll(lm[1]) + (uint32_t)__popcll(lm[2]) + (uint32_t)__popcll(lm[3]);
                while (un + add > kPU) rank_some(un < 64u ? un : 64u);
            }
#pragma unroll
            for (uint32_t c = 0; c < 4; ++c) {
                if (live[c]) uq[un + (uint32_t)__popcll(lm[c] & ((1ull << lane) - 1ull))] = ee[c];
                un += (uint32_t)__popcll(lm[c]);
            }
        }
    };

    uint32_t t = t_first;
    tile_lo = bitmap_base + (t_first << kProbeTileShift);
    auto next_arrays = [&](const uint32_t tt) {
#pragma unroll
        for (uint32_t a = 0; a < NA; ++a) {
            na_g0[a] = dir_at(adv[a], tt);
            na_nv[a] = dir_at(adv[a], tt + 1u) - na_g0[a];
        }
    };
    if (t < t_end) {
        next_arrays(t);
        issue_tile(t, dir_at(dirv, t), dir_at(dirv, t + 1u));
    }
    PS_AT(0)
    while (t < t_end) {
        PS_COUNT(8)
        __builtin_amdgcn_s_waitcnt(0x0F70);
        __builtin_amdgcn_s_setprio(3);
        const uint32_t rounds = pf_rounds, v0 = pf_v0, v1 = pf_v1;
        if (OR || rounds) {
            if (OR) {
#pragma unroll
                for (uint32_t h = 0; h < kPNV; ++h) {
                    u32x4 u = wk[0][h];
#pragma unroll
                    for (uint32_t i = 1; i < NB; ++i) u |= wk[i][h];
                    ucnt += (uint32_t)__popc(u.x) + (uint32_t)__popc(u.y) + (uint32_t)__popc(u.z) + (uint32_t)__popc(u.w);
                }
            }
#pragma unroll
            for (uint32_t i = 0; i < NB; ++i) {
#pragma unroll
                for (uint32_t h = 0; h < kPNV; ++h) reinterpret_cast<u32x4*>(tile + i * kPTW)[h * 64u + lane] = wk[i][h];
                rank[i * kPRk + lane] = rk[i];
            }
#pragma unroll
            for (uint32_t a = 0; a < NA; ++a) {
#pragma unroll
                for (uint32_t h = 0; h < kPNV; ++h)
                    if (h * 64u + lane < na_nv[a]) reinterpret_cast<u32x4*>(arr + a * arr_slot)[h * 64u + lane] = wk[NB + a][h];
                a_g0[a] = na_g0[a];
                a_cnt[a] = na_nv[a] * 8u;
            }
#pragma unroll
            for (uint32_t r = 0; r < kPMaxR; ++r) {
                cid[r] = nid[r];
                asm volatile("" : "+v"(cid[r]));
            }
        }
        {
            uint32_t fr = f_r, glo = (uint32_t)g_prev, ghi = (uint32_t)(g_prev >> 32);
            asm volatile("" : "+v"(fr), "+v"(glo), "+v"(ghi), "+v"(dirv));
#pragma unroll
            for (uint32_t a = 0; a < NA; ++a) asm volatile("" : "+v"(adv[a]));
            f_r = (uint16_t)fr;
            g_prev = ((unsigned long long)ghi << 32) | glo;
        }
        PS_AT(1)
        if (lane == 0 && g_prev > *thr) *thr = g_prev;
        const bool more = t + 1u < t_end;
        uint32_t ng0 = 0, ng1 = 0;
        if (more) {
            if (t + 2u - dir_base >= 64u) {
                dir_base = t + 1u;
                dirv = load_dir(cgdir);
#pragma unroll
                for (uint32_t a = 0; a < NA; ++a) adv[a] = load_dir(d_agd[a]);
            }
            ng0 = dir_at(dirv, t + 1u);
            ng1 = dir_at(dirv, t + 2u);
            next_arrays(t + 1u);
        }
        if (f_stage || rn >= 64u) PS_COUNT(11)
        flush_service(false);
        PS_AT(4)
        if (more) issue_tile(t + 1u, ng0, ng1);
        else pf_rounds = 0;
        if (lane == 0) g_prev = __hip_atomic_load(gthr, __ATOMIC_RELAXED, __HIP_MEMORY_SCOPE_AGENT);
        __builtin_amdgcn_s_setprio(0);
        probe_lds_fence();
        {
            const unsigned long long tn = *thr;
            if ((uint32_t)(tn >> 32) != (uint32_t)(thr_seen >> 32)) take_raw_min(__uint_as_float(unorder_f32((uint32_t)(tn >> 32))));
            thr_seen = tn;
            ++tiles_since_merge;
        }
        PS_AT(5)
#ifdef VQ_PROBE_STREAM_ONLY
        hits += (unsigned long long)__popcll(wballot((cid[0].x ^ cid[1].y) == 0x12345u));
        if (rounds && span == 0xFFFFFFFFu) {
#else
        if (rounds) {
#endif
            const uint32_t tile_end = tile_lo + kPT;
            const uint32_t tile_hi = (tile_end > tile_lo && tile_end < span_hi) ? tile_end : span_hi;
            const uint32_t lo_bound = tile_lo > span_lo ? tile_lo : span_lo;
            lo_rel = lo_bound - tile_lo;
            width = tile_hi - lo_bound;
            {
                ProbeWords pw[kPMaxR];
#pragma unroll
                for (uint32_t r = 0; r < kPMaxR; ++r)
                    if (r < rounds) pw[r] = probe_read(cid[r]);
#pragma unroll
                for (uint32_t r = 0; r < kPMaxR; ++r)
                    if (r < rounds) {
                        PS_COUNT(9)
                        probe_eval(cid[r], pw[r], r > 0u);
                    }
            }
            for (uint32_t r = kPMaxR; r < rounds; ++r) {
                const uint32_t v = v0 + r * 64u + lane;
                u32x4 e4 = kSent;
                if (v < v1) e4 = cc4[v];
                PS_COUNT(9)
                const ProbeWords pw = probe_read(e4);
                probe_eval(e4, pw, true);
            }
            PS_AT(2)
            while (un) {
                PS_COUNT(10)
                rank_some(un < 64u ? un : 64u);
            }
            PS_AT(3)
        }
        ++t;
        tile_lo += kPT;
    }
    while (f_stage || rn) flush_service(true);
    __syncthreads();
    cand_prune(cs, top_k);
    {
        const uint32_t cn = *cand_n;
        unsigned long long* out = span_keys + (size_t)keys_base + (size_t)span * top_k;
        for (uint32_t i = lane; i < top_k; i += 64u) out[i] = i < cn ? cand[i] : 0ull;
    }
    if (OR) {
        uint32_t total;
        (void)wave_excl_scan_u32(ucnt, &total);
        hits += (unsigned long long)total;
    }
    if (lane == 0 && hits) atomicAdd(&num_hits[q], hits);
    if (lane == 0 && H->stat_off && lds[4]) atomicAdd(&num_hits[H->stat_off], (unsigned long long)lds[4]);
    PS_AT(6)
    PS_FLUSH
}

__device__ __forceinline__ void probe_item(const uint32_t* __restrict__ span_base, const uint32_t* __restrict__ qmap, uint32_t nq, uint32_t* q, uint32_t* span) {
    uint32_t lo = 0, hi = nq;
    const uint32_t wg = blockIdx.x;
    while (hi - lo > 1) {
        uint32_t mid = (lo + hi) >> 1;
        if (span_base[mid] <= wg) lo = mid;
        else hi = mid;
    }
    *span = blockIdx.x - span_base[lo];
    *q = qmap[lo];
}

#define VQ_PROBE_PARAMS                                                                                                                                       \
    const uint8_t *__restrict__ blobs, const uint32_t *__restrict__ blob_off, const uint32_t *__restrict__ span_base, const uint32_t *__restrict__ qmap, uint32_t nq, \
        uint32_t cand_cap, uint32_t arr_slot, unsigned long long *__restrict__ span_keys, unsigned long long *__restrict__ num_hits
#define VQ_PROBE_ITEM                           \
    uint32_t q, span;                           \
    probe_item(span_base, qmap, nq, &q, &span); \
    const uint8_t* blob = blobs + blob_off[q];
#ifndef VQ_PROBE_WAVES
#define VQ_PROBE_WAVES 4
#endif
#define VQ_PROBE_KERNEL(waves) __global__ __launch_bounds__(64) __attribute__((amdgpu_waves_per_eu(waves, 8))) void

VQ_PROBE_KERNEL(VQ_PROBE_WAVES) k_scan_probe_1(VQ_PROBE_PARAMS) {
    VQ_PROBE_ITEM
    if (((as_const<QHeader>(blob)->simple_flags >> 12) & 0xFu) == 0u) probe_body<1, 0>(blob, span, q, cand_cap, arr_slot, span_keys, num_hits);
    else probe_body<1, 1>(blob, span, q, cand_cap, arr_slot, span_keys, num_hits);
}
VQ_PROBE_KERNEL(VQ_PROBE_WAVES) k_scan_probe_2_0(VQ_PROBE_PARAMS) {
    VQ_PROBE_ITEM
    probe_body<2, 0>(blob, span, q, cand_cap, arr_slot, span_keys, num_hits);
}
VQ_PROBE_KERNEL(VQ_PROBE_WAVES) k_scan_probe_2_1(VQ_PROBE_PARAMS) {
    VQ_PROBE_ITEM
    probe_body<2, 1>(blob, span, q, cand_cap, arr_slot, span_keys, num_hits);
}
VQ_PROBE_KERNEL(VQ_PROBE_WAVES) k_scan_probe_2_2(VQ_PROBE_PARAMS) {
    VQ_PROBE_ITEM
    probe_body<2, 2>(blob, span, q, cand_cap, arr_slot, span_keys, num_hits);
}
VQ_PROBE_KERNEL(3) k_scan_probe_3_0(VQ_PROBE_PARAMS) {
    VQ_PROBE_ITEM
    probe_body<3, 0>(blob, span, q, cand_cap, arr_slot, span_keys, num_hits);
}
VQ_PROBE_KERNEL(3) k_scan_probe_3_1(VQ_PROBE_PARAMS) {
    VQ_PROBE_ITEM
    probe_body<3, 1>(blob, span, q, cand_cap, arr_slot, span_keys, num_hits);
}
VQ_PROBE_KERNEL(3) k_scan_probe_3_2(VQ_PROBE_PARAMS) {
    VQ_PROBE_ITEM
    probe_body<3, 2>(blob, span, q, cand_cap, arr_slot, span_keys, num_hits);
}
VQ_PROBE_KERNEL(3) k_scan_probe_3_3(VQ_PROBE_PARAMS) {
    VQ_PROBE_ITEM
    probe_body<3, 3>(blob, span, q, cand_cap, arr_slot, span_keys, num_hits);
}

VQ_PROBE_KERNEL(3) k_scan_probe_or(VQ_PROBE_PARAMS) {
    VQ_PROBE_ITEM
    if (as_const<QHeader>(blob)->simple_n == 2u) probe_body<1, 0, true>(blob, span, q, cand_cap, arr_slot, span_keys, num_hits);
    else probe_body<2, 0, true>(blob, span, q, cand_cap, arr_slot, span_keys, num_hits);
}

static auto* probe_kernel(uint32_t shape) {
    return shape == kProbeAnd1 ? k_scan_probe_1 : shape == kProbeAnd2A0 ? k_scan_probe_2_0 : shape == kProbeAnd2A1 ? k_scan_probe_2_1 : shape == kProbeAnd2A2 ? k_scan_probe_2_2 :
           shape == kProbeAnd3A0 ? k_scan_probe_3_0 : shape == kProbeAnd3A1 ? k_scan_probe_3_1 : shape == kProbeAnd3A2 ? k_scan_probe_3_2 : shape == kProbeAnd3A3 ? k_scan_probe_3_3 :
                                                                                                                                                                    k_scan_probe_or;
}

uint32_t debug_probe_occupancy(uint32_t shape, size_t lds_bytes) {
    int n = 0;
    if (shape >= kProbeShapes || hipOccupancyMaxActiveBlocksPerMultiprocessor(&n, probe_kernel(shape), 64, lds_bytes) != hipSuccess || n < 0) return 0;
    return (uint32_t)n;
}

void launch_scan_probe_shape(hipStream_t st, uint32_t shape, uint32_t na_seen, uint32_t arr_slot, uint32_t total_spans, const uint8_t* blobs, const uint32_t* blob_off,
                             const uint32_t* span_base, const uint32_t* qmap, uint32_t nq, uint32_t cand_cap, unsigned long long* span_keys, unsigned long long* num_hits) {
    if (!total_spans) return;
    const uint32_t nd = shape == kProbeAnd1 ? 1u : (shape >= kProbeAnd3A0 && shape <= kProbeAnd3A3) ? 3u : 2u;
    size_t lds = 0;
    for (uint32_t na = 0; na <= nd; ++na)
        if ((na_seen >> na) & 1u) lds = std::max(lds, scan_probe_lds_bytes(cand_cap, nd, na, arr_slot));
    hipLaunchKernelGGL(probe_kernel(shape), dim3(total_spans), dim3(64), lds, st, blobs, blob_off, span_base, qmap, nq, cand_cap, arr_slot, span_keys, num_hits);
}

}
```

Before: 161,400.

## Add per-tile group directory to arr16 images to shorten LDS binary search

Each 32K-doc tile in the arr16 image now gets a prefix directory of 64 u16 group offsets (512-doc groups), built at index time and loaded into LDS along with the tile's array. The probe kernel jumps to the group start and runs a fixed-depth branchless search whose depth comes from the largest group size, passed in the upper bits of the launch argument. This replaces the full log2(tile) binary search per candidate. The cost is extra HBM bytes per visited tile for the directory, larger LDS slots that may lower occupancy, and a small debug API.

```diff
diff --git a/veloci_amd/csrc/capi.cpp b/veloci_amd/csrc/capi.cpp
--- a/veloci_amd/csrc/capi.cpp
+++ b/veloci_amd/csrc/capi.cpp
@@ -240,6 +240,28 @@
     const size_t lds = vq::scan_probe_lds_bytes(cand_cap, nd, na, arr_slot);
     if (lds_bytes) *lds_bytes = uint32_t(lds);
     return vq::debug_probe_occupancy(shape, lds);
+}
+int vq_debug_arr16_image(const vq_index* index, const char* path, uint32_t token, uint32_t* info, uint32_t* gdir_out, uint64_t gdir_cap, uint16_t* image_out, uint64_t image_cap) {
+    if (!index || !path || !info) return -1;
+    const auto it = index->idx->postings.find(path);
+    if (it == index->idx->postings.end() || token >= it->second.num_tokens) return -1;
+    const PostingStore& ps = it->second;
+    const uint64_t entries = (index->idx->bitmap_words >> (vq::kProbeTileShift - 5)) + 3;
+    const bool has = !ps.ak_start.empty() && ps.ak_start[token] >= 0;
+    info[0] = ps.tile_most.empty() ? 0 : ps.tile_most[token];
+    info[1] = ps.group_most.empty() ? 0 : ps.group_most[token];
+    info[2] = has ? uint32_t(entries) : 0;
+    info[3] = 0;
+    if (!has) return 0;
+    std::vector<uint32_t> gd(entries);
+    if (hipMemcpy(gd.data(), ps.gdir.as<uint32_t>() + ps.gd_start[token], entries * 4, hipMemcpyDeviceToHost) != hipSuccess) return -1;
+    const uint64_t gran = uint64_t(gd[entries - 1]) + uint64_t(vq::kArrDirGran) * entries;
+    info[3] = uint32_t(gran);
+    if (gdir_out) std::copy_n(gd.data(), std::min<uint64_t>(entries, gdir_cap), gdir_out);
+    if (image_out && image_cap &&
+        hipMemcpy(image_out, ps.arr16.as<uint16_t>() + uint64_t(ps.ak_start[token]) * 8, std::min<uint64_t>(gran * 8, image_cap) * 2, hipMemcpyDeviceToHost) != hipSuccess)
+        return -1;
+    return 0;
 }
 uint64_t vq_index_speculative_reruns(const vq_index* index) { return index ? index->idx->or_reruns.load() : 0; }
 int vq_debug_facet_select(const uint32_t* hist, uint32_t num_values, uint32_t top, uint32_t misalign, uint32_t* out_values, uint32_t* out_counts) {
diff --git a/veloci_amd/csrc/compile.cpp b/veloci_amd/csrc/compile.cpp
--- a/veloci_amd/csrc/compile.cpp
+++ b/veloci_amd/csrc/compile.cpp
@@ -708,6 +708,7 @@
                 h.d_gdir = ps.gdir.as<uint32_t>() + ps.gd_start[e.tid];
                 if (ps.ak_start[e.tid] >= 0) h.d_arr16 = ps.arr16.as<uint16_t>() + uint64_t(ps.ak_start[e.tid]) * 8;
                 h.tile_most = ps.tile_most[e.tid];
+                h.group_most = ps.group_most[e.tid];
             }
             uint32_t li = add_list(h);
             info.cover.push_back(li);
@@ -2171,7 +2172,10 @@
                     for (uint32_t k = 0; k < cq.simple_n; ++k) {
                         const HList& l = cq.lists[cq.ops[k].list_begin];
                         cq.probe.leaf[k] = DProbeLeaf{l.d_cov32, l.d_arr16, l.d_gdir};
-                        if ((arr_mask >> k) & 1u) cq.probe_arr_gran = std::max(cq.probe_arr_gran, l.tile_most);
+                        if ((arr_mask >> k) & 1u) {
+                            cq.probe_arr_gran = std::max(cq.probe_arr_gran, l.tile_most + kArrDirGran);
+                            cq.probe_arr_group = std::max(cq.probe_arr_group, l.group_most);
+                        }
                     }
                 }
                 static const bool ring = std::getenv("VQ_RING") != nullptr && std::atoi(std::getenv("VQ_RING")) != 0;
@@ -2304,7 +2308,7 @@
         } else if ((cq.simple_flags >> 25) & 1u) {
             for (uint32_t k = 0; k < cq.simple_n; ++k) {
                 const uint64_t len = cq.lists[cq.ops[k].list_begin].len;
-                b += ((cq.simple_flags >> k) & 1u) ? visited * (tile_docs / 8 + 4 * (tile_docs >> kRankShift)) : ((cq.simple_flags >> (12 + k)) & 1u) ? 2ull * len : 4ull * len;
+                b += ((cq.simple_flags >> k) & 1u) ? visited * (tile_docs / 8 + 4 * (tile_docs >> kRankShift)) : ((cq.simple_flags >> (12 + k)) & 1u) ? 2ull * len + 16ull * kArrDirGran * visited : 4ull * len;
             }
         } else if (simple) {
             std::vector<bool> seen(cq.lists.size(), false);
diff --git a/veloci_amd/csrc/device_types.hpp b/veloci_amd/csrc/device_types.hpp
--- a/veloci_amd/csrc/device_types.hpp
+++ b/veloci_amd/csrc/device_types.hpp
@@ -14,6 +14,7 @@
 constexpr int kMaxSkipWhen = 4;
 constexpr uint32_t kTileDirShift = 14;
 constexpr uint32_t kProbeTileShift = 15;
+constexpr uint32_t kArrGroupShift = 9, kArrGroups = 1u << (kProbeTileShift - kArrGroupShift), kArrDirGran = kArrGroups / 8, kArrMaxGran = 256 - kArrDirGran;
 constexpr uint32_t kRankShift = 9;
 
 enum ListFlags : uint32_t {
diff --git a/veloci_amd/csrc/engine.hpp b/veloci_amd/csrc/engine.hpp
--- a/veloci_amd/csrc/engine.hpp
+++ b/veloci_amd/csrc/engine.hpp
@@ -297,6 +297,7 @@
     std::vector<int64_t> ak_start;
     std::vector<int64_t> gd_start;
     std::vector<uint32_t> tile_most;
+    std::vector<uint32_t> group_most;
     DevBuf cov32, arr16, gdir;
 };
 
@@ -503,6 +504,7 @@
     const uint16_t* d_arr16 = nullptr;
     const uint32_t* d_gdir = nullptr;
     uint32_t tile_most = 0;
+    uint32_t group_most = 0;
     int inline_idx = -1;
     int inline_val_idx = -1;
 };
@@ -576,6 +578,7 @@
     DSimple2 simple2{};
     DWide wide{};
     DProbe probe{};
+    uint32_t probe_arr_group = 0;
     uint32_t probe_arr_gran = 0;
     std::vector<DFacet> facets;
     std::vector<FacetOut> facet_out;
diff --git a/veloci_amd/csrc/exec.cpp b/veloci_amd/csrc/exec.cpp
--- a/veloci_amd/csrc/exec.cpp
+++ b/veloci_amd/csrc/exec.cpp
@@ -1359,6 +1359,7 @@
     struct ProbeClass {
         uint32_t first = 0, n = 0, spans = 0;
         uint32_t na_seen = 0, arr_slot = 0;
+        uint32_t arr_group = 0;
     } pcls[kProbeShapes];
     auto probe_class = [](const CompiledQuery& cq) -> uint32_t {
         if ((cq.simple_flags >> 27) & 1u) return kProbeOr;
@@ -1468,6 +1469,7 @@
                 ProbeClass& pc = pcls[probe_class(cq)];
                 pc.na_seen |= 1u << uint32_t(__builtin_popcount((cq.simple_flags >> 12) & 0xFu));
                 pc.arr_slot = std::max(pc.arr_slot, cq.probe_arr_gran * 4u);
+                pc.arr_group = std::max(pc.arr_group, cq.probe_arr_group);
                 sp[pc.first + pc.n] = pc.spans;
                 mp[pc.first + pc.n++] = qi;
                 pc.spans += cq.n_spans;
@@ -1600,11 +1602,16 @@
         static const bool trace = std::getenv("VQ_PROBE_TRACE") != nullptr;
         for (uint32_t c = 0; c < kProbeShapes; ++c)
             if (pcls[c].spans && trace)
-                std::fprintf(stderr, "probe launch: shape %u, %u queries, %u spans, array slot %u words (fullest tile: %u granules), NA seen 0x%x\n", c, pcls[c].n, pcls[c].spans,
-                             pcls[c].arr_slot, pcls[c].arr_slot / 4, pcls[c].na_seen);
+                std::fprintf(stderr, "probe launch: shape %u, %u queries, %u spans, array slot %u words (directory + fullest tile: %u granules), fullest group %u entries, NA seen 0x%x\n", c,
+                             pcls[c].n, pcls[c].spans, pcls[c].arr_slot, pcls[c].arr_slot / 4, pcls[c].arr_group, pcls[c].na_seen);
+        auto depth_of = [](uint32_t group_most) {
+            uint32_t d = 0;
+            while ((1u << d) < group_most + 1u) ++d;
+            return d;
+        };
         for (uint32_t c = 0; c < kProbeShapes; ++c)
             if (pcls[c].spans)
-                launch_scan_probe_shape(st, c, pcls[c].na_seen, pcls[c].arr_slot, pcls[c].spans, pb->d_blobs, pb->d_blob_off, tab(up_span_p) + pcls[c].first, tab(up_qmap_p) + pcls[c].first,
+                launch_scan_probe_shape(st, c, pcls[c].na_seen, pcls[c].arr_slot | depth_of(pcls[c].arr_group) << 16, pcls[c].spans, pb->d_blobs, pb->d_blob_off, tab(up_span_p) + pcls[c].first, tab(up_qmap_p) + pcls[c].first,
                                         pcls[c].n, cand_cap, keys_ptr, hits_ptr);
     }
     VQ_HIP(hipGetLastError());
diff --git a/veloci_amd/csrc/index.cpp b/veloci_amd/csrc/index.cpp
--- a/veloci_amd/csrc/index.cpp
+++ b/veloci_amd/csrc/index.cpp
@@ -315,29 +315,35 @@
         ps.ak_start.assign(ps.num_tokens, -1);
         ps.gd_start.assign(ps.num_tokens, -1);
         ps.tile_most.assign(ps.num_tokens, 0);
+        ps.group_most.assign(ps.num_tokens, 0);
         {
             const uint64_t ptiles = (idx->bitmap_words >> (kProbeTileShift - 5)) + 2;
             uint64_t cov_gran = 0, arr_gran = 0;
             std::vector<uint32_t> gd(tiled.size() * (ptiles + 1));
             std::vector<uint64_t> gran_of(tiled.size());
-            std::vector<uint32_t> most_of(tiled.size());
+            std::vector<uint32_t> most_of(tiled.size()), group_of(tiled.size());
             parallel_for(tiled.size(), nthreads, [&](size_t j) {
                 const uint32_t t = tiled[j];
                 const uint32_t* d = docs.data() + ps.start[t];
                 uint32_t* g = gd.data() + j * (ptiles + 1);
                 uint64_t gran = 0;
-                uint32_t i = 0, most = 0;
+                uint32_t i = 0, most = 0, gmost = 0;
                 for (uint64_t k = 0; k <= ptiles; ++k) {
                     g[k] = uint32_t(gran);
-                    const uint64_t thi = uint64_t(idx->bitmap_base) + ((k + 1) << kProbeTileShift);
+                    const uint64_t tlo = uint64_t(idx->bitmap_base) + (k << kProbeTileShift);
                     const uint32_t i0 = i;
-                    while (i < ps.len[t] && d[i] < thi) ++i;
+                    for (uint32_t grp = 1; grp <= kArrGroups; ++grp) {
+                        const uint32_t ig = i;
+                        while (i < ps.len[t] && d[i] < tlo + (uint64_t(grp) << kArrGroupShift)) ++i;
+                        gmost = std::max(gmost, i - ig);
+                    }
                     const uint32_t n8 = (i - i0 + 7u) / 8u;
                     most = std::max(most, n8);
                     gran += n8;
                 }
                 gran_of[j] = gran;
                 most_of[j] = most;
+                group_of[j] = gmost;
             });
             for (size_t j = 0; j < tiled.size(); ++j) {
                 const uint32_t t = tiled[j];
@@ -346,9 +352,10 @@
                 ps.pk_start[t] = int64_t(cov_gran);
                 ps.tile_most[t] = most_of[j];
                 cov_gran += gran_of[j];
-                if (most_of[j] <= 256) {
+                if (most_of[j] <= kArrMaxGran) {
                     ps.ak_start[t] = int64_t(arr_gran);
-                    arr_gran += gran_of[j];
+                    ps.group_most[t] = group_of[j];
+                    arr_gran += gran_of[j] + kArrDirGran * (ptiles + 1);
                 }
             }
             if (cov_gran) {
@@ -370,15 +377,24 @@
                     uint32_t i = 0;
                     for (uint64_t k = 0; k <= ptiles; ++k) {
                         const uint64_t tlo = uint64_t(idx->bitmap_base) + (k << kProbeTileShift), thi = tlo + (1u << kProbeTileShift);
+                        uint16_t* const ak = a ? a + (w + (k + 1) * kArrDirGran * 8) : nullptr;
+                        const uint64_t w0 = w;
+                        uint16_t* const dir = a ? ak - kArrGroups : nullptr;
+                        if (a) std::fill(dir, ak, uint16_t(0));
                         for (; i < ps.len[t] && d[i] < thi; ++i, ++w) {
                             const uint32_t rel = uint32_t(d[i] - tlo);
                             c[w] = rel << 16 | sc[i];
-                            if (a) a[w] = uint16_t(rel);
+                            if (a) {
+                                ak[w - w0] = uint16_t(rel);
+                                if ((rel >> kArrGroupShift) + 1 < kArrGroups) ++dir[(rel >> kArrGroupShift) + 1];
+                            }
                         }
                         for (; w % 8; ++w) {
                             c[w] = 0xFFFFFFFFu;
-                            if (a) a[w] = 0xFFFFu;
+                            if (a) ak[w - w0] = 0xFFFFu;
                         }
+                        if (a)
+                            for (uint32_t grp = 1; grp < kArrGroups; ++grp) dir[grp] += dir[grp - 1];
                     }
                 });
                 upload(ps.cov32, cov.data(), cov.size() * 4);
diff --git a/veloci_amd/csrc/kernels.hpp b/veloci_amd/csrc/kernels.hpp
--- a/veloci_amd/csrc/kernels.hpp
+++ b/veloci_amd/csrc/kernels.hpp
@@ -59,7 +59,7 @@
 enum : uint32_t { kProbeAnd1 = 0, kProbeAnd2A0, kProbeAnd2A1, kProbeAnd2A2, kProbeAnd3A0, kProbeAnd3A1, kProbeAnd3A2, kProbeAnd3A3, kProbeOr, kProbeShapes };
 size_t scan_probe_lds_bytes(uint32_t cand_cap, uint32_t nd, uint32_t na, uint32_t arr_slot);
 uint32_t debug_probe_occupancy(uint32_t shape, size_t lds_bytes);
-void launch_scan_probe_shape(hipStream_t st, uint32_t shape, uint32_t na_seen, uint32_t arr_slot, uint32_t total_spans, const uint8_t* blobs, const uint32_t* blob_off,
+void launch_scan_probe_shape(hipStream_t st, uint32_t shape, uint32_t na_seen, uint32_t arr_geom, uint32_t total_spans, const uint8_t* blobs, const uint32_t* blob_off,
                              const uint32_t* span_base, const uint32_t* qmap, uint32_t nq, uint32_t cand_cap, unsigned long long* span_keys, unsigned long long* num_hits);
 uint32_t scan_ring_consumers(uint32_t max_nd);
 uint32_t scan_ring_slots(uint32_t maxnd, uint32_t consumers);
diff --git a/veloci_amd/csrc/scan_probe.hip b/veloci_amd/csrc/scan_probe.hip
--- a/veloci_amd/csrc/scan_probe.hip
+++ b/veloci_amd/csrc/scan_probe.hip
@@ -55,10 +55,14 @@
     return (size_t)(probe_lds_arr(nd, nd - na) + na * arr_slot + 2 * cand_cap) * 4 + 16;
 }
 
+__device__ __forceinline__ uint16_t lds_u16(const uint32_t addr) { return *reinterpret_cast<const __attribute__((address_space(3))) uint16_t*>((uintptr_t)addr); }
+
 template <uint32_t ND, uint32_t NA, bool OR = false>
-__device__ __forceinline__ void probe_body(const uint8_t* __restrict__ blob, const uint32_t span, const uint32_t q, const uint32_t cand_cap, const uint32_t arr_slot,
+__device__ __forceinline__ void probe_body(const uint8_t* __restrict__ blob, const uint32_t span, const uint32_t q, const uint32_t cand_cap, const uint32_t arr_geom,
                                            unsigned long long* __restrict__ span_keys, unsigned long long* __restrict__ num_hits) {
     extern __shared__ __attribute__((aligned(16))) uint32_t lds[];
+    const uint32_t lds_addr = (uint32_t)(uintptr_t)(__attribute__((address_space(3))) uint32_t*)lds;
+    const uint32_t arr_slot = arr_geom & 0xFFFFu;
     const uint32_t lane = threadIdx.x;
     const VQ_CONST QHeader* H = as_const<QHeader>(blob);
     const VQ_CONST DList* gl = as_const<DList>(blob + H->off_lists);
@@ -208,7 +212,7 @@
             }
 #pragma unroll
             for (uint32_t a = 0; a < NA; ++a) {
-                const VQ_GLOBAL u32x4* ga = as_global(reinterpret_cast<const u32x4*>(d_arr[a]) + na_g0[a]);
+                const VQ_GLOBAL u32x4* ga = as_global(reinterpret_cast<const u32x4*>(d_arr[a]) + na_g0[a] + kArrDirGran * tt);
 #pragma unroll
                 for (uint32_t h = 0; h < kPNV; ++h)
                     if (h * 64u + lane < na_nv[a]) wk[NB + a][h] = ga[h * 64u + lane];
@@ -399,23 +403,37 @@
             const uint32_t rel = e >> 16;
 #pragma unroll
             for (uint32_t a = 0; a < NA; ++a) {
-                const uint16_t* A = reinterpret_cast<const uint16_t*>(arr + a * arr_slot);
-                uint32_t lo = 0u, len = a_cnt[a];
+                const uint32_t ebase = lds_addr + (probe_lds_arr(ND, NB) + a * arr_slot) * 4u + kArrGroups * 2u;
+                uint32_t last = ebase + (a_cnt[a] ? a_cnt[a] * 2u - 2u : 0u);
+                asm volatile("" : "+v"(last));
+                uint32_t lo = min(ebase + (uint32_t)lds_u16(ebase - kArrGroups * 2u + ((e >> (16u + kArrGroupShift - 1u)) & (kArrGroups * 2u - 2u))) * 2u, last);
 #ifdef VQ_PROBE_NO_SEARCH
-                lo = rel & 7u;
-                len = 0u;
+                lo = ebase + (rel & 7u) * 2u;
+                found = found && a_cnt[a] != 0u && ((uint32_t)lds_u16(lo) ^ rel) < 0x2000u;
+#else
+#define VQ_ARR_STEP(w)                                                      \
+    {                                                                       \
+        const uint32_t p = min(lo + 2u * (w), last);                        \
+        lo = (uint32_t)lds_u16(p) <= rel ? p : lo;  \
+    }
+#define VQ_ARR_STEPS4 VQ_ARR_STEP(8u) VQ_ARR_STEP(4u) VQ_ARR_STEP(2u) VQ_ARR_STEP(1u)
+                const uint32_t depth = arr_geom >> 16;
+                if (depth <= 6u) {
+                    if (depth > 4u) {
+                        VQ_ARR_STEP(32u) VQ_ARR_STEP(16u)
+                    }
+                    VQ_ARR_STEPS4
+                } else {
+                    if (depth > 8u) {
+                        VQ_ARR_STEP(512u) VQ_ARR_STEP(256u)
+                    }
+                    VQ_ARR_STEP(128u) VQ_ARR_STEP(64u) VQ_ARR_STEP(32u) VQ_ARR_STEP(16u) VQ_ARR_STEPS4
+                }
+#undef VQ_ARR_STEPS4
+#undef VQ_ARR_STEP
+                found = found && a_cnt[a] != 0u && (uint32_t)lds_u16(lo) == rel;
 #endif
-                while (len > 1u) {
-                    const uint32_t half = len >> 1;
-                    lo = (uint32_t)A[lo + half] <= rel ? lo + half : lo;
-                    len -= half;
-                }
-#ifdef VQ_PROBE_NO_SEARCH
-                found = found && a_cnt[a] != 0u && ((uint32_t)A[lo] ^ rel) < 0x2000u;
-#else
-                found = found && a_cnt[a] != 0u && (uint32_t)A[lo] == rel;
-#endif
-                pos[a] = lo;
+                pos[a] = lo - ebase;
             }
             const unsigned long long fm = wballot(found);
             hits += (unsigned long long)__popcll(fm);
@@ -429,7 +447,7 @@
 #pragma unroll
                     for (uint32_t i = 0; i < NB; ++i) rq[(2u + i) * kPR + slot] = bitmap_rank(i, rel);
 #pragma unroll
-                    for (uint32_t a = 0; a < NA; ++a) rq[(2u + NB + a) * kPR + slot] = (a_g0[a] * 8u + pos[a]) * 2u;
+                    for (uint32_t a = 0; a < NA; ++a) rq[(2u + NB + a) * kPR + slot] = a_g0[a] * 16u + pos[a];
                 }
                 rn += (uint32_t)__popcll(lm);
             }
@@ -510,7 +528,7 @@
 #pragma unroll
         for (uint32_t a = 0; a < NA; ++a) {
             na_g0[a] = dir_at(adv[a], tt);
-            na_nv[a] = dir_at(adv[a], tt + 1u) - na_g0[a];
+            na_nv[a] = dir_at(adv[a], tt + 1u) - na_g0[a] + kArrDirGran;
         }
     };
     if (t < t_end) {
@@ -545,7 +563,7 @@
                 for (uint32_t h = 0; h < kPNV; ++h)
                     if (h * 64u + lane < na_nv[a]) reinterpret_cast<u32x4*>(arr + a * arr_slot)[h * 64u + lane] = wk[NB + a][h];
                 a_g0[a] = na_g0[a];
-                a_cnt[a] = na_nv[a] * 8u;
+                a_cnt[a] = (na_nv[a] - kArrDirGran) * 8u;
             }
 #pragma unroll
             for (uint32_t r = 0; r < kPMaxR; ++r) {
@@ -665,7 +683,7 @@
 
 #define VQ_PROBE_PARAMS                                                                                                                                       \
     const uint8_t *__restrict__ blobs, const uint32_t *__restrict__ blob_off, const uint32_t *__restrict__ span_base, const uint32_t *__restrict__ qmap, uint32_t nq, \
-        uint32_t cand_cap, uint32_t arr_slot, unsigned long long *__restrict__ span_keys, unsigned long long *__restrict__ num_hits
+        uint32_t cand_cap, uint32_t arr_geom, unsigned long long *__restrict__ span_keys, unsigned long long *__restrict__ num_hits
 #define VQ_PROBE_ITEM                           \
     uint32_t q, span;                           \
     probe_item(span_base, qmap, nq, &q, &span); \
@@ -677,42 +695,42 @@
 
 VQ_PROBE_KERNEL(VQ_PROBE_WAVES) k_scan_probe_1(VQ_PROBE_PARAMS) {
     VQ_PROBE_ITEM
-    if (((as_const<QHeader>(blob)->simple_flags >> 12) & 0xFu) == 0u) probe_body<1, 0>(blob, span, q, cand_cap, arr_slot, span_keys, num_hits);
-    else probe_body<1, 1>(blob, span, q, cand_cap, arr_slot, span_keys, num_hits);
+    if (((as_const<QHeader>(blob)->simple_flags >> 12) & 0xFu) == 0u) probe_body<1, 0>(blob, span, q, cand_cap, arr_geom, span_keys, num_hits);
+    else probe_body<1, 1>(blob, span, q, cand_cap, arr_geom, span_keys, num_hits);
 }
 VQ_PROBE_KERNEL(VQ_PROBE_WAVES) k_scan_probe_2_0(VQ_PROBE_PARAMS) {
     VQ_PROBE_ITEM
-    probe_body<2, 0>(blob, span, q, cand_cap, arr_slot, span_keys, num_hits);
+    probe_body<2, 0>(blob, span, q, cand_cap, arr_geom, span_keys, num_hits);
 }
 VQ_PROBE_KERNEL(VQ_PROBE_WAVES) k_scan_probe_2_1(VQ_PROBE_PARAMS) {
     VQ_PROBE_ITEM
-    probe_body<2, 1>(blob, span, q, cand_cap, arr_slot, span_keys, num_hits);
+    probe_body<2, 1>(blob, span, q, cand_cap, arr_geom, span_keys, num_hits);
 }
 VQ_PROBE_KERNEL(VQ_PROBE_WAVES) k_scan_probe_2_2(VQ_PROBE_PARAMS) {
     VQ_PROBE_ITEM
-    probe_body<2, 2>(blob, span, q, cand_cap, arr_slot, span_keys, num_hits);
+    probe_body<2, 2>(blob, span, q, cand_cap, arr_geom, span_keys, num_hits);
 }
 VQ_PROBE_KERNEL(3) k_scan_probe_3_0(VQ_PROBE_PARAMS) {
     VQ_PROBE_ITEM
-    probe_body<3, 0>(blob, span, q, cand_cap, arr_slot, span_keys, num_hits);
+    probe_body<3, 0>(blob, span, q, cand_cap, arr_geom, span_keys, num_hits);
 }
 VQ_PROBE_KERNEL(3) k_scan_probe_3_1(VQ_PROBE_PARAMS) {
     VQ_PROBE_ITEM
-    probe_body<3, 1>(blob, span, q, cand_cap, arr_slot, span_keys, num_hits);
+    probe_body<3, 1>(blob, span, q, cand_cap, arr_geom, span_keys, num_hits);
 }
 VQ_PROBE_KERNEL(3) k_scan_probe_3_2(VQ_PROBE_PARAMS) {
     VQ_PROBE_ITEM
-    probe_body<3, 2>(blob, span, q, cand_cap, arr_slot, span_keys, num_hits);
+    probe_body<3, 2>(blob, span, q, cand_cap, arr_geom, span_keys, num_hits);
 }
 VQ_PROBE_KERNEL(3) k_scan_probe_3_3(VQ_PROBE_PARAMS) {
     VQ_PROBE_ITEM
-    probe_body<3, 3>(blob, span, q, cand_cap, arr_slot, span_keys, num_hits);
+    probe_body<3, 3>(blob, span, q, cand_cap, arr_geom, span_keys, num_hits);
 }
 
 VQ_PROBE_KERNEL(3) k_scan_probe_or(VQ_PROBE_PARAMS) {
     VQ_PROBE_ITEM
-    if (as_const<QHeader>(blob)->simple_n == 2u) probe_body<1, 0, true>(blob, span, q, cand_cap, arr_slot, span_keys, num_hits);
-    else probe_body<2, 0, true>(blob, span, q, cand_cap, arr_slot, span_keys, num_hits);
+    if (as_const<QHeader>(blob)->simple_n == 2u) probe_body<1, 0, true>(blob, span, q, cand_cap, arr_geom, span_keys, num_hits);
+    else probe_body<2, 0, true>(blob, span, q, cand_cap, arr_geom, span_keys, num_hits);
 }
 
 static auto* probe_kernel(uint32_t shape) {
@@ -727,14 +745,14 @@
     return (uint32_t)n;
 }
 
-void launch_scan_probe_shape(hipStream_t st, uint32_t shape, uint32_t na_seen, uint32_t arr_slot, uint32_t total_spans, const uint8_t* blobs, const uint32_t* blob_off,
+void launch_scan_probe_shape(hipStream_t st, uint32_t shape, uint32_t na_seen, uint32_t arr_geom, uint32_t total_spans, const uint8_t* blobs, const uint32_t* blob_off,
                              const uint32_t* span_base, const uint32_t* qmap, uint32_t nq, uint32_t cand_cap, unsigned long long* span_keys, unsigned long long* num_hits) {
     if (!total_spans) return;
     const uint32_t nd = shape == kProbeAnd1 ? 1u : (shape >= kProbeAnd3A0 && shape <= kProbeAnd3A3) ? 3u : 2u;
     size_t lds = 0;
     for (uint32_t na = 0; na <= nd; ++na)
-        if ((na_seen >> na) & 1u) lds = std::max(lds, scan_probe_lds_bytes(cand_cap, nd, na, arr_slot));
-    hipLaunchKernelGGL(probe_kernel(shape), dim3(total_spans), dim3(64), lds, st, blobs, blob_off, span_base, qmap, nq, cand_cap, arr_slot, span_keys, num_hits);
-}
-
-}
+        if ((na_seen >> na) & 1u) lds = std::max(lds, scan_probe_lds_bytes(cand_cap, nd, na, arr_geom & 0xFFFFu));
+    hipLaunchKernelGGL(probe_kernel(shape), dim3(total_spans), dim3(64), lds, st, blobs, blob_off, span_base, qmap, nq, cand_cap, arr_geom, span_keys, num_hits);
+}
+
+}
```

After: 161,700 (median of 6 runs). No clear change (+0.2%).
